# ddrakard/tensorflow-distributed-on-gke

Hardware: AMD Instinct MI355X
Metric: tokens/sec (whole node), Transformer-base en-pt at 1/2/4/8 MI355X (higher is better)
Workload: dtype bf16; 1 GPU; model=transformer-base (6L, d_model=512, heads=8, d_ff=2048, vocab 7765/7010), global_batch=64, local_batch=64, seq_len=128, parallelism=dp1, hip_graph=single, grad_comm=fp32, defer_wgrad=True

## Files before the change

csrc/bindings/embedding.cpp:

```cpp
#include "common.h"

namespace {

bool check_tok(const Tensor& tok) {
  TORCH_CHECK(tok.is_contiguous() && tok.is_cuda(), "tok must be a contiguous GPU tensor");
  const bool t64 = tok.scalar_type() == at::kLong;
  TORCH_CHECK(t64 || tok.scalar_type() == at::kInt, "tok must be int32/int64");
  return t64;
}
void check_grads(const Tensor& dout, const Tensor& dtable, int64_t M) {
  check_bf16(dout, "dout");
  check_contig(dout, "dout");
  check_f32(dtable, "dtable");
  check_contig(dtable, "dtable");
  TORCH_CHECK(dout.numel() == M * dtable.size(1), "dout shape");
}
void check_kbits(const optional<Tensor>& kbits, int64_t M, int64_t D) {
  if (!kbits.has_value()) return;
  TORCH_CHECK(kbits->is_cuda() && kbits->scalar_type() == at::kByte && kbits->is_contiguous() &&
                  kbits->numel() == M * D / 8,
              "kbits: uint8 [M, D / 8]");
  check_aligned(*kbits, 4, "kbits");
}

void embed_fwd(const Tensor& tok, const Tensor& table, const Tensor& pe, const Tensor& out,
               double scale, double p, int64_t seed, const optional<Tensor>& ctr, int64_t site,
               const optional<Tensor>& kbits) {
  TORCH_CHECK(tok.dim() == 2, "tok must be [B,L]");
  const bool t64 = check_tok(tok);
  check_bf16(table, "table");
  check_contig(table, "table");
  check_f32(pe, "pe");
  check_contig(pe, "pe");
  check_bf16(out, "out");
  check_contig(out, "out");
  const int64_t D = table.size(1), L = tok.size(1), M = tok.numel();
  TORCH_CHECK(pe.dim() == 2 && pe.size(1) == D && pe.size(0) >= L, "pe table too short");
  TORCH_CHECK(out.numel() == M * D, "out shape");
  check_kbits(kbits, M, D);
  c10::DeviceGuard g(tok.device());
  const int rc = tdg_embed_fwd(tok.data_ptr(), t64, table.data_ptr(), pe.data_ptr<float>(),
                               out.data_ptr(), (int)M, (int)L, (int)D, (float)scale, (float)p,
                               (uint64_t)seed, ctr_ptr(ctr), (uint64_t)site, opt_ptr(kbits),
                               stream_of(tok));
  check_err(rc, "tdg embed_fwd");
}

void embed_bwd(const Tensor& tok, const Tensor& dout, const Tensor& dtable, double scale,
               double p, int64_t seed, const optional<Tensor>& ctr, int64_t site) {
  const bool t64 = check_tok(tok);
  const int64_t D = dtable.size(1), M = tok.numel();
  check_grads(dout, dtable, M);
  c10::DeviceGuard g(tok.device());
  const int rc = tdg_embed_bwd(tok.data_ptr(), t64, dout.data_ptr(), dtable.data_ptr<float>(),
                               (int)M, (int)D, (float)scale, (float)p, (uint64_t)seed,
                               ctr_ptr(ctr), (uint64_t)site, stream_of(tok));
  check_err(rc, "tdg embed_bwd");
}

void embed_bwd_det(const Tensor& tok, const Tensor& dout, const Tensor& dtable, const Tensor& acc,
                   double scale, double p, int64_t seed, const optional<Tensor>& ctr, int64_t site,
                   bool accumulate) {
  const bool t64 = check_tok(tok);
  const int64_t D = dtable.size(1), M = tok.numel(), V = dtable.size(0);
  check_grads(dout, dtable, M);
  TORCH_CHECK(acc.scalar_type() == at::kLong && acc.is_cuda() && acc.is_contiguous(), "acc int64");
  TORCH_CHECK(acc.numel() >= dtable.numel(), "acc too small");
  c10::DeviceGuard g(tok.device());
  const int rc = tdg_embed_bwd_det(tok.data_ptr(), t64, dout.data_ptr(), dtable.data_ptr<float>(),
                                   reinterpret_cast<long long*>(acc.data_ptr<int64_t>()), (int)M,
                                   (int)D, (long long)V, (float)scale, (float)p, (uint64_t)seed,
                                   ctr_ptr(ctr), (uint64_t)site, accumulate ? 1.f : 0.f,
                                   stream_of(tok));
  check_err(rc, "tdg embed_bwd_det");
}

std::vector<int64_t> embed_csr_ws(int64_t M, int64_t V, int64_t D) {
  long long n32 = 0, n64 = 0;
  tdg_embed_csr_ws((int)M, (int)V, (int)D, &n32, &n64);
  return {n32, n64};
}

bool embed_csr_ok(int64_t M, int64_t V) { return tdg_embed_csr_ok((int)M, (int)V) != 0; }

void check_csr_ws(const Tensor& ws32, int64_t M, int64_t V, int64_t D, const char* n) {
  const int64_t n32 = embed_csr_ws(M, V, D)[0];
  TORCH_CHECK(ws32.scalar_type() == at::kInt && ws32.is_cuda() && ws32.is_contiguous() &&
                  ws32.numel() >= n32,
              n, ": int32 workspace of ", n32, " words");
  check_aligned(ws32, 16, n);
}

void embed_csr_sort(const std::vector<Tensor>& toks, const std::vector<int64_t>& V,
                    const std::vector<Tensor>& ws32, const optional<Tensor>& stamps) {
  const int n = (int)toks.size();
  TORCH_CHECK(n >= 1 && n <= 2 && (int)V.size() == n && (int)ws32.size() == n, "embed_csr_sort: 1-2 tables");
  const void* tp[2];
  int t64[2], M[2], VV[2];
  int* wp[2];
  for (int i = 0; i < n; ++i) {
    const Tensor& t = toks[i];
    t64[i] = check_tok(t);
    TORCH_CHECK(tdg_embed_csr_ok((int)t.numel(), (int)V[i]), "embed_csr_sort: shape past the sort");
    check_csr_ws(ws32[i], t.numel(), V[i], 128, "embed_csr_sort");
    tp[i] = t.data_ptr();
    M[i] = (int)t.numel();
    VV[i] = (int)V[i];
    wp[i] = ws32[i].data_ptr<int>();
  }
  c10::DeviceGuard g(toks[0].device());
  long long* sp = nullptr;
  if (stamps.has_value()) {
    TORCH_CHECK(stamps->scalar_type() == at::kLong && stamps->is_cuda() && stamps->numel() >= 1024,
                "stamps");
    sp = reinterpret_cast<long long*>(stamps->data_ptr<int64_t>());
  }
  check_err(tdg_embed_csr_sort(n, tp, t64, M, VV, wp, sp, stream_of(toks[0])), "tdg embed_csr_sort");
}

void embed_csr_apply(const Tensor& dout, const Tensor& dtable, const Tensor& ws32,
                     const Tensor& ws64, int64_t M, double scale, double p, int64_t seed,
                     const optional<Tensor>& ctr, int64_t site, bool accumulate,
                     const optional<Tensor>& kbits) {
  check_grads(dout, dtable, M);
  check_aligned(dtable, 16, "dtable");
  const int64_t D = dtable.size(1), V = dtable.size(0);
  TORCH_CHECK(tdg_embed_csr_ok((int)M, (int)V), "embed_csr_apply: shape past the sort");
  check_kbits(kbits, M, D);
  check_csr_ws(ws32, M, V, D, "embed_csr_apply");
  const int64_t n64 = embed_csr_ws(M, V, D)[1];
  TORCH_CHECK(ws64.scalar_type() == at::kLong && ws64.is_cuda() && ws64.is_contiguous() &&
                  ws64.numel() >= n64,
              "embed_csr_apply: int64 workspace of ", n64, " words");
  c10::DeviceGuard g(dout.device());
  check_err(tdg_embed_csr_apply(dout.data_ptr(), opt_ptr(kbits), dtable.data_ptr<float>(),
                                ws32.data_ptr<int>(),
                                reinterpret_cast<long long*>(ws64.data_ptr<int64_t>()), (int)M,
                                (int)D, (int)V, (float)scale, (float)p, (uint64_t)seed,
                                ctr_ptr(ctr), (uint64_t)site, accumulate ? 1.f : 0.f,
                                stream_of(dout)),
            "tdg embed_csr_apply");
}

}

void def_embedding(py::module_& m) {
  m.def("embed_fwd", &embed_fwd);
  m.def("embed_bwd", &embed_bwd);
  m.def("embed_bwd_det", &embed_bwd_det);
  m.def("embed_csr_ws", &embed_csr_ws);
  m.def("embed_csr_ok", &embed_csr_ok);
  m.def("embed_csr_sort", &embed_csr_sort);
  m.def("embed_csr_apply", &embed_csr_apply);
}
```

csrc/bindings/gemm.cpp:

```cpp
#include "common.h"

namespace {

void check_operand(const Tensor& t, bool kc, int64_t mn, int64_t K, int64_t ld, const char* n) {
  check_bf16(t, n);
  check_aligned(t, 16, n);
  if (kc) check_extent(t, mn, ld, round8(K), n);
  else check_extent(t, K, ld, round8(mn), n);
}
void check_group_c(const Tensor& C, bool f32, int64_t M, int64_t N, int64_t ldc) {
  TORCH_CHECK(C.is_cuda() && (C.scalar_type() == at::kFloat) == f32 &&
                  (f32 || C.scalar_type() == at::kBFloat16),
              "grouped gemm: C dtypes must match (f32 or bf16)");
  check_extent(C, M, ldc, N, "C");
}

void gemm(const Tensor& A, const Tensor& B, const Tensor& C, const optional<Tensor>& bias,
          const optional<Tensor>& aux, int64_t M, int64_t N, int64_t K, int64_t lda, int64_t ldb,
          int64_t ldc, int64_t ldaux, bool a_kc, bool b_kc, int64_t epi, double alpha,
          double beta, int64_t tile_cfg, int64_t splits, const optional<Tensor>& ws,
          const optional<Tensor>& relu_bits, int64_t ldbits) {
  TORCH_CHECK(C.is_cuda(), "C must be a GPU tensor");
  const bool f32 = C.scalar_type() == at::kFloat;
  TORCH_CHECK(f32 || C.scalar_type() == at::kBFloat16, "C must be f32 or bf16");
  TORCH_CHECK(M > 0 && N > 0 && K > 0, "gemm: empty problem");
  TORCH_CHECK(lda % 8 == 0 && ldb % 8 == 0, "gemm: lda/ldb must be multiples of 8");
  TORCH_CHECK(lda >= round8(a_kc ? K : M), "gemm: lda < round8(", a_kc ? "K)" : "M)");
  TORCH_CHECK(ldb >= round8(b_kc ? K : N), "gemm: ldb < round8(", b_kc ? "K)" : "N)");
  check_operand(A, a_kc, M, K, lda, "A");
  check_operand(B, b_kc, N, K, ldb, "B");
  TORCH_CHECK(ldc >= N, "gemm: ldc < N");
  check_extent(C, M, ldc, N, "C");
  const float* bptr = nullptr;
  if (epi == 1 || epi == 2) {
    TORCH_CHECK(bias.has_value(), "gemm: bias epilogue needs bias");
    check_f32(*bias, "bias");
    TORCH_CHECK(bias->numel() >= N, "gemm: bias too short");
    bptr = bias->data_ptr<float>();
  }
  const void* xptr = nullptr;
  void* bits = nullptr;
  if (relu_bits.has_value()) {
    TORCH_CHECK(epi == 2 || epi == 3, "gemm: relu_bits needs the bias+ReLU or ReLU-backward epilogue");
    TORCH_CHECK(relu_bits->is_cuda() && relu_bits->scalar_type() == at::kByte,
                "relu_bits must be a uint8 GPU tensor");
    TORCH_CHECK(N % 8 == 0, "gemm: relu_bits needs N % 8 == 0");
    TORCH_CHECK(ldbits >= N / 8, "gemm: ldbits < N / 8");
    check_extent(*relu_bits, M, ldbits, N / 8, "relu_bits");
    bits = relu_bits->data_ptr();
  }
  if (epi == 3 && bits == nullptr) {
    TORCH_CHECK(aux.has_value(), "gemm: DRELU epilogue needs aux");
    check_bf16(*aux, "aux");
    check_extent(*aux, M, ldaux, N, "aux");
    xptr = aux->data_ptr();
  }
  float* wptr = nullptr;
  if (splits > 1) {
    TORCH_CHECK(ws.has_value(), "gemm: split-K needs a workspace");
    check_f32(*ws, "ws");
    TORCH_CHECK(ws->numel() >= splits * M * ldc, "gemm: workspace too small");
    wptr = ws->data_ptr<float>();
  }
  c10::DeviceGuard g(A.device());
  const int rc = tdg_gemm(A.data_ptr(), B.data_ptr(), C.data_ptr(), bptr, xptr, (int)M, (int)N,
                          (int)K, (int)lda, (int)ldb, (int)ldc, (int)ldaux, a_kc, b_kc, (int)epi,
                          f32, (float)alpha, (float)beta, (int)tile_cfg, (int)splits, wptr,
                          stream_of(A), bits, (int)ldbits);
  check_err(rc, "tdg gemm");
}

void gemm_grouped(const std::vector<Tensor>& As, const std::vector<Tensor>& Bs,
                  const std::vector<Tensor>& Cs, int64_t M, int64_t N, int64_t K, int64_t lda,
                  int64_t ldb, int64_t ldc, bool a_kc, bool b_kc, double alpha, double beta,
                  int64_t tile_cfg) {
  const size_t G = As.size();
  TORCH_CHECK(G >= 1 && G <= 32 && Bs.size() == G && Cs.size() == G, "gemm_grouped: 1..32 problems");
  TORCH_CHECK(M > 0 && N > 0 && K > 0 && lda % 8 == 0 && ldb % 8 == 0 && ldc >= N, "gemm_grouped: shape");
  const bool f32 = Cs[0].scalar_type() == at::kFloat;
  std::vector<const void*> a(G), b(G);
  std::vector<void*> c(G);
  for (size_t i = 0; i < G; ++i) {
    check_operand(As[i], a_kc, M, K, lda, "A");
    check_operand(Bs[i], b_kc, N, K, ldb, "B");
    check_group_c(Cs[i], f32, M, N, ldc);
    a[i] = As[i].data_ptr();
    b[i] = Bs[i].data_ptr();
    c[i] = Cs[i].data_ptr();
  }
  c10::DeviceGuard g(As[0].device());
  const int rc = tdg_gemm_grouped(a.data(), b.data(), c.data(), (int)G, (int)M, (int)N, (int)K,
                                  (int)lda, (int)ldb, (int)ldc, a_kc, b_kc, f32, (float)alpha,
                                  (float)beta, (int)tile_cfg, stream_of(As[0]));
  check_err(rc, "tdg gemm_grouped");
}

void gemm_ragged(const std::vector<Tensor>& As, const std::vector<Tensor>& Bs,
                 const std::vector<Tensor>& Cs, const std::vector<int64_t>& shapes, int64_t K,
                 bool a_kc, bool b_kc, double alpha, double beta,
                 const std::vector<c10::optional<Tensor>>& bias_out) {
  const size_t P = As.size();
  TORCH_CHECK(P >= 1 && P <= 64 && Bs.size() == P && Cs.size() == P && shapes.size() == 7 * P,
              "gemm_ragged: 1..64 problems, 7 shape values each (M, N, lda, ldb, ldc, t_first, "
              "t_count)");
  TORCH_CHECK(K > 0 && K % 64 == 0, "gemm_ragged: K must be a multiple of 64");
  const bool f32 = Cs[0].scalar_type() == at::kFloat;
  std::vector<const void*> a(P), b(P);
  std::vector<void*> c(P);
  std::vector<int> sh(7 * P);
  for (size_t i = 0; i < P; ++i) {
    const int64_t M = shapes[7 * i], N = shapes[7 * i + 1], lda = shapes[7 * i + 2],
                  ldb = shapes[7 * i + 3], ldc = shapes[7 * i + 4];
    TORCH_CHECK(M > 0 && N > 0 && lda % 8 == 0 && ldb % 8 == 0 && ldc >= N, "gemm_ragged: shape");
    check_operand(As[i], a_kc, M, K, lda, "A");
    check_operand(Bs[i], b_kc, N, K, ldb, "B");
    check_group_c(Cs[i], f32, M, N, ldc);
    a[i] = As[i].data_ptr();
    b[i] = Bs[i].data_ptr();
    c[i] = Cs[i].data_ptr();
    for (int j = 0; j < 7; ++j) sh[7 * i + j] = (int)shapes[7 * i + j];
  }
// ... 12 lines not shown
  }
  c10::DeviceGuard g(As[0].device());
  const int rc = tdg_gemm_ragged(a.data(), b.data(), c.data(), (int)P, sh.data(), (int)K, a_kc,
                                 b_kc, f32, (float)alpha, (float)beta,
                                 any_bias ? bo.data() : nullptr, stream_of(As[0]));
  check_err(rc, "tdg gemm_ragged");
}

void colsum(const Tensor& X, const Tensor& out, const Tensor& part, int64_t M, int64_t N,
            int64_t ld, int64_t rows_per_block, double beta) {
  check_bf16(X, "X");
  check_f32(out, "out");
  check_f32(part, "part");
  check_extent(X, M, ld, N, "X");
  TORCH_CHECK(out.numel() >= N, "colsum: out too short");
  TORCH_CHECK(part.numel() >= ((M + rows_per_block - 1) / rows_per_block) * N,
              "colsum: partial buffer too small");
  c10::DeviceGuard g(X.device());
  tdg_colsum(X.data_ptr(), out.data_ptr<float>(), part.data_ptr<float>(), (int)M, (int)N, (int)ld,
             (int)rows_per_block, (float)beta, stream_of(X));
  check_err(0, "tdg colsum");
}

void colsum_grouped(const std::vector<Tensor>& Xs, const std::vector<Tensor>& outs,
                    const Tensor& part, int64_t M, int64_t N, int64_t ld, int64_t rows_per_block,
                    double beta) {
  const size_t G = Xs.size();
  TORCH_CHECK(G >= 1 && G <= 32 && outs.size() == G, "colsum_grouped: 1..32 problems");
  check_f32(part, "part");
  const int64_t nparts = (M + rows_per_block - 1) / rows_per_block;
  TORCH_CHECK(part.numel() >= (int64_t)G * nparts * N, "colsum_grouped: partials too small");
  std::vector<const void*> x(G);
  std::vector<float*> o(G);
  for (size_t i = 0; i < G; ++i) {
    check_bf16(Xs[i], "X");
    check_extent(Xs[i], M, ld, N, "X");
    check_f32(outs[i], "out");
    TORCH_CHECK(outs[i].numel() >= N, "colsum_grouped: out too short");
    x[i] = Xs[i].data_ptr();
    o[i] = outs[i].data_ptr<float>();
  }
  c10::DeviceGuard g(Xs[0].device());
  check_err(tdg_colsum_grouped(x.data(), o.data(), (int)G, part.data_ptr<float>(), (int)M, (int)N,
                               (int)ld, (int)rows_per_block, (float)beta, stream_of(Xs[0])),
            "tdg colsum_grouped");
}

std::vector<int64_t> gemm_last_plan() {
  int p[5];
  tdg_gemm_last_plan(p);
  return {p[0], p[1], p[2], p[3], p[4]};
}

}

void def_gemm(py::module_& m) {
  m.def("gemm", &gemm, py::arg("A"), py::arg("B"), py::arg("C"), py::arg("bias"), py::arg("aux"),
        py::arg("M"), py::arg("N"), py::arg("K"), py::arg("lda"), py::arg("ldb"), py::arg("ldc"),
        py::arg("ldaux"), py::arg("a_kc"), py::arg("b_kc"), py::arg("epi"), py::arg("alpha"),
        py::arg("beta"), py::arg("tile_cfg"), py::arg("splits"), py::arg("ws"),
        py::arg("relu_bits") = optional<Tensor>(), py::arg("ldbits") = 0);
  m.def("gemm_grouped", &gemm_grouped);
  m.def("gemm_ragged", &gemm_ragged, py::arg("As"), py::arg("Bs"), py::arg("Cs"), py::arg("shapes"),
        py::arg("K"), py::arg("a_kc"), py::arg("b_kc"), py::arg("alpha"), py::arg("beta"),
        py::arg("bias_out") = std::vector<c10::optional<Tensor>>{});
  m.def("gemm_last_plan", &gemm_last_plan);
  m.def("colsum", &colsum);
  m.def("colsum_grouped", &colsum_grouped);
}
```

csrc/bindings/layernorm.cpp:

```cpp
#include "common.h"

namespace {

void check_same_numel(const Tensor& t, const Tensor& like, const char* n) {
  TORCH_CHECK(t.numel() == like.numel() && t.is_contiguous(), "ln: ", n, " shape");
}
void check_ln_kbits(const optional<Tensor>& kbits, int64_t M, int64_t D) {
  if (!kbits.has_value()) return;
  TORCH_CHECK(kbits->is_cuda() && kbits->scalar_type() == at::kByte && kbits->is_contiguous() &&
                  kbits->numel() == M * D / 8 && D >= 512,
              "ln: kbits uint8 [M, D / 8] (D >= 512)");
}

void ln_fwd(const Tensor& x, const optional<Tensor>& s, const Tensor& gamma, const Tensor& beta,
            const Tensor& y, const optional<Tensor>& hsave, const optional<Tensor>& mean,
            const optional<Tensor>& rstd, double p, int64_t seed, const optional<Tensor>& ctr,
            int64_t site, double eps, const optional<Tensor>& y8, const optional<Tensor>& s8,
            const optional<Tensor>& amax8, const optional<Tensor>& kbits) {
  check_bf16(x, "x");
  check_contig(x, "x");
  const int64_t D = x.size(-1), M = x.numel() / D;
  check_bf16(y, "y");
  check_same_numel(y, x, "y");
  if (s.has_value()) {
    check_bf16(*s, "s");
    check_same_numel(*s, x, "s");
  }
  check_f32(gamma, "gamma");
  check_f32(beta, "beta");
  TORCH_CHECK(gamma.numel() == D && beta.numel() == D, "ln: gamma/beta shape");
  if (hsave.has_value()) {
    check_bf16(*hsave, "hsave");
    check_same_numel(*hsave, x, "hsave");
  }
  for (auto* t : {&mean, &rstd})
    if (t->has_value()) {
      check_f32(**t, "mean/rstd");
      TORCH_CHECK((*t)->numel() == M, "ln: mean/rstd shape");
    }
  if (y8.has_value()) {
    check_f8_fmt(*y8, 0, "y8");
    check_same_numel(*y8, x, "y8");
    TORCH_CHECK(s8.has_value(), "ln: y8 needs s8");
    check_f32(*s8, "s8");
  }
  check_ln_kbits(kbits, M, D);
  TORCH_CHECK(!kbits.has_value() || s.has_value(), "ln: kbits are the dropout on s");
  c10::DeviceGuard g(x.device());
  const int rc = tdg_ln_fwd(x.data_ptr(), opt_ptr(s), gamma.data_ptr<float>(),
                            beta.data_ptr<float>(), y.data_ptr(), opt_ptr(hsave), opt_f32(mean),
                            opt_f32(rstd), (int)M, (int)D, (float)p, (uint64_t)seed, ctr_ptr(ctr),
                            (uint64_t)site, (float)eps, opt_ptr(y8), opt_f32(s8), amax_ptr(amax8),
                            opt_ptr(kbits), stream_of(x));
  check_err(rc, "tdg ln_fwd");
}

void ln_bwd(const Tensor& dy, const Tensor& hsave, const Tensor& mean, const Tensor& rstd,
            const Tensor& gamma, const Tensor& dh, const optional<Tensor>& ds,
            const optional<Tensor>& dres, const Tensor& dgamma, const Tensor& dbeta,
            const optional<Tensor>& dbias, const Tensor& ws, double p, int64_t seed,
            const optional<Tensor>& ctr, int64_t site, bool accumulate, bool skip_reduce,
            int64_t rpb, const optional<Tensor>& ds8, const optional<Tensor>& s8,
            const optional<Tensor>& amax8, const optional<Tensor>& kbits) {
  check_bf16(dy, "dy");
  check_contig(dy, "dy");
  const int64_t D = dy.size(-1), M = dy.numel() / D;
  for (auto* t : {&hsave, &dh}) {
    check_bf16(*t, "hsave/dh");
    check_same_numel(*t, dy, "hsave/dh");
  }
  for (auto* t : {&ds, &dres})
    if (t->has_value()) {
      check_bf16(**t, "ds/dres");
      check_same_numel(**t, dy, "ds/dres");
    }
  check_f32(mean, "mean");
  check_f32(rstd, "rstd");
  check_f32(gamma, "gamma");
  check_f32(dgamma, "dgamma");
  check_f32(dbeta, "dbeta");
  TORCH_CHECK(mean.numel() == M && rstd.numel() == M, "ln_bwd: mean/rstd shape");
  TORCH_CHECK(gamma.numel() == D && dgamma.numel() == D && dbeta.numel() == D, "ln_bwd: D");
  if (dbias.has_value()) {
    check_f32(*dbias, "dbias");
    TORCH_CHECK(dbias->numel() == D && (ds.has_value() || ds8.has_value()), "ln_bwd: dbias needs ds");
  }
  if (ds8.has_value()) {
    check_f8_fmt(*ds8, 1, "ds8 (e5m2)");
    check_same_numel(*ds8, dy, "ds8");
    TORCH_CHECK(s8.has_value(), "ln_bwd: ds8 needs s8");
    check_f32(*s8, "s8");
  }
  check_f32(ws, "ws");
  TORCH_CHECK(rpb == 16 || rpb == 32 || rpb == 64, "ln_bwd: rows per block 16 / 32 / 64");
  TORCH_CHECK(ws.numel() >= 3 * ((M + rpb - 1) / rpb) * D, "ln_bwd: workspace too small");
  check_ln_kbits(kbits, M, D);
  c10::DeviceGuard g(dy.device());
  const int rc = tdg_ln_bwd(
      dy.data_ptr(), hsave.data_ptr(), mean.data_ptr<float>(), rstd.data_ptr<float>(),
      gamma.data_ptr<float>(), dh.data_ptr(), opt_ptr(ds), opt_ptr(dres), dgamma.data_ptr<float>(),
      dbeta.data_ptr<float>(), opt_f32(dbias), ws.data_ptr<float>(), (int)M, (int)D, (float)p,
      (uint64_t)seed, ctr_ptr(ctr), (uint64_t)site, accumulate, skip_reduce, (int)rpb,
      opt_ptr(ds8), opt_f32(s8), amax_ptr(amax8), opt_ptr(kbits), stream_of(dy));
  check_err(rc, "tdg ln_bwd");
}

void reduce_partials_multi(const std::vector<Tensor>& parts, const std::vector<Tensor>& outs,
                           const std::vector<int64_t>& nparts, int64_t N, double beta) {
  const size_t G = parts.size();
  TORCH_CHECK(G >= 1 && G <= 96 && outs.size() == G && nparts.size() == G,
              "reduce_partials_multi: 1..96 problems");
  std::vector<const float*> pp(G);
  std::vector<float*> oo(G);
  std::vector<int> np(G);
  for (size_t i = 0; i < G; ++i) {
    check_f32(parts[i], "parts");
    check_f32(outs[i], "outs");
    check_contig(parts[i], "parts");
    TORCH_CHECK(outs[i].numel() == N && outs[i].is_contiguous(), "reduce_partials_multi: out");
    TORCH_CHECK(parts[i].numel() >= nparts[i] * N, "reduce_partials_multi: partials too small");
    TORCH_CHECK(parts[i].device() == parts[0].device() && outs[i].device() == parts[0].device(),
                "reduce_partials_multi: one device");
    pp[i] = parts[i].data_ptr<float>();
    oo[i] = outs[i].data_ptr<float>();
    np[i] = (int)nparts[i];
  }
  c10::DeviceGuard g(parts[0].device());
  check_err(tdg_reduce_partials_multi(pp.data(), oo.data(), np.data(), (int)G, (int)N, (float)beta,
                                      stream_of(parts[0])),
            "tdg reduce_partials_multi");
}

}

void def_layernorm(py::module_& m) {
  m.def("ln_fwd", &ln_fwd);
  m.def("ln_bwd", &ln_bwd);
  m.def("reduce_partials_multi", &reduce_partials_multi);
}
```

csrc/include/tdg_api.h:

```cpp
#pragma once
#include <hip/hip_runtime.h>
#include <stdint.h>

#include "tdg_attn.h"
#include "tdg_decode.h"

extern "C" {

int tdg_gemm(const void* A, const void* B, void* C, const float* bias, const void* aux, int M,
             int N, int K, int lda, int ldb, int ldc, int ldaux, int a_kc, int b_kc, int epi,
             int out_f32, float alpha, float beta, int tile_cfg, int splits, float* ws,
             hipStream_t st, void* relu_bits, int ldbits);
int tdg_gemm_grouped(const void* const* A, const void* const* B, void* const* C, int G, int M,
                     int N, int K, int lda, int ldb, int ldc, int a_kc, int b_kc, int out_f32,
                     float alpha, float beta, int tile_cfg, hipStream_t st);
int tdg_gemm_ragged(const void* const* A, const void* const* B, void* const* C, int P,
                    const int* shapes, int K, int a_kc, int b_kc, int out_f32, float alpha,
                    float beta, float* const* bias_out, hipStream_t st);
void tdg_gemm_last_plan(int out[5]);
void tdg_colsum(const void* X, float* out, float* part, int M, int N, int ld, int rows_per_block,
                float beta, hipStream_t st);
int tdg_colsum_grouped(const void* const* X, float* const* out, int G, float* part, int M, int N,
                       int ld, int rows_per_block, float beta, hipStream_t st);

int tdg_attn_fwd(const tdg::AttnArgs* a, int hd, hipStream_t st);
int tdg_qkv_attn_fwd(const tdg::QkvAttnArgs* qa, hipStream_t st);
int tdg_attn_bwd(const tdg::AttnArgs* a, int hd, hipStream_t st);
int tdg_attn_bwd_fdo(const tdg::AttnArgs* a, hipStream_t st);
int tdg_attn_probs(const tdg::AttnArgs* a, int hd, float* probs, hipStream_t st);
int tdg_attn_fwd_fp8(const tdg::AttnArgs* a, int hd, hipStream_t st);
int tdg_attn_bwd_f8(const tdg::AttnArgs* a, int hd, hipStream_t st);

int tdg_decode_attn(const tdg::DecodeAttnArgs* a, int hd, hipStream_t st);
int tdg_beam_topk(const tdg::BeamTopkArgs* a, hipStream_t st);

int tdg_ln_fwd(const void* x, const void* s, const float* gamma, const float* beta, void* y,
               void* hsave, float* mean, float* rstd, int M, int D, float p, uint64_t seed,
               const long long* ctr, uint64_t site, float eps, void* y8, const float* s8,
               unsigned* amax8, void* kbits, hipStream_t st);
int tdg_ln_bwd(const void* dy, const void* hsave, const float* mean, const float* rstd,
               const float* gamma, void* dh, void* ds, const void* dres, float* dgamma,
               float* dbeta, float* dbias, float* ws, int M, int D, float p, uint64_t seed,
               const long long* ctr, uint64_t site, int accumulate, int skip_reduce, int rpb,
               void* ds8, const float* s8, unsigned* amax8, const void* kbits, hipStream_t st);
int tdg_reduce_partials_multi(const float* const* parts, float* const* outs, const int* nparts,
                              int G, int N, float beta, hipStream_t st);

int tdg_embed_fwd(const void* tok, int tok64, const void* table, const float* pe, void* out, int M,
                  int L, int D, float scale, float p, uint64_t seed, const long long* ctr,
                  uint64_t site, void* kbits, hipStream_t st);
int tdg_embed_bwd(const void* tok, int tok64, const void* dout, float* dtable, int M, int D,
                  float scale, float p, uint64_t seed, const long long* ctr, uint64_t site,
                  hipStream_t st);
int tdg_embed_bwd_det(const void* tok, int tok64, const void* dout, float* dtable, long long* acc,
                      int M, int D, long long V, float scale, float p, uint64_t seed,
                      const long long* ctr, uint64_t site, float beta, hipStream_t st);
void tdg_embed_csr_ws(int M, int V, int D, long long* n32, long long* n64);
int tdg_embed_csr_ok(int M, int V);
int tdg_embed_csr_sort(int ntab, const void* const* tok, const int* tok64, const int* M,
                       const int* V, int* const* ws32, long long* stamps, hipStream_t st);
int tdg_embed_csr_apply(const void* dout, const void* kbits, float* dtable, int* ws32,
                        long long* ws64, int M, int D, int V, float scale, float p, uint64_t seed,
                        const long long* ctr, uint64_t site, float beta, hipStream_t st);

int tdg_count_tokens(const void* labels, int lab64, int M, float* out, hipStream_t st);
int tdg_prep_batch(const void* src, int S, const void* tgt, int T1, int B, int lab64, void* tgt_in,
                   void* labels, int* src_len, int* tgt_len, float* ntok, long long* ctr,
                   int* row_lab, unsigned* ticket, int* bad_rows, hipStream_t st);
int tdg_xent(void* logits, int M, int V, int ldl, const void* labels, int lab64, const float* ntok,
             float workers, float smoothing, float* row_loss, float* row_correct, int write_grad,
             hipStream_t st);
int tdg_xent_stats(const float* row_loss, const float* row_correct, int M, const float* ntok,
                   float workers, float* step_out, float* accum, hipStream_t st);

int tdg_adam(float* p, float* g, float* m, float* v, void* shadow, long long n, long long* step,
             float beta1, float beta2, float eps, float lr_const, float d_model, float warmup,
             float grad_scale, float weight_decay, int sched, int zero_grad, int inc_step,
             const float* gstate, hipStream_t st);
int tdg_adam_chunks(float* p, float* g, float* m, float* v, void* shadow, long long n,
                    const void* chunks, int nchunks, long long* step, float beta1, float beta2,
                    float eps, float lr_const, float d_model, float warmup, float grad_scale,
                    float weight_decay, int sched, int zero_grad, int inc_step,
                    const float* scale8, unsigned* amax8, const float* gstate, hipStream_t st);
int tdg_adam_step_inc(long long* step, const float* gstate, hipStream_t st);
long long tdg_grad_sumsq(const float* g, const void* chunks, long long nchunks, long long n,
                         float* partials, hipStream_t st);
int tdg_grad_norm_finalize(const float* partials, long long nparts, float* state,
                           unsigned* counters, float clip, int skip_on, float grad_scale,
                           hipStream_t st);
int tdg_to_bf16(const float* p, void* o, long long n, hipStream_t st);
int tdg_transpose_grouped(const void* const* src, void* const* dst, int G, int R, int C,
                          hipStream_t st);

int tdg_gemm_fp8(const void* A, const void* B, void* C, const float* bias, const float* sa,
                 const float* sb, void* C8, const float* sc8, unsigned* amax, int M, int N, int K,
                 int lda, int ldb, int ldc, int ldc8, int epi, int cfg, int afmt, int cfmt,
                 const void* aux, int ldaux, float beta, const void* aux8, float* colsum_out,
                 float colsum_beta, float* ws, hipStream_t st);
int tdg_wgrad_fp8(const void* const* A, const void* const* B, float* const* C,
                  const float* const* sa, const float* const* sb, int P, const int* shapes, int T,
                  float beta, hipStream_t st);
int tdg_fp8_set_persist(int on);
int tdg_fp8_quant(const void* x, void* y8, long long n, const float* scale, unsigned* amax,
// ... 17 lines not shown
```

csrc/include/tdg_common.h:

```cpp
#pragma once
#include <hip/hip_runtime.h>
#include <utility>
#include <stdint.h>

namespace tdg {

#ifdef TDG_STAMPS
__device__ unsigned long long* tdg_stamps;
#define TDG_STAMP(i)                                                                      \
  do {                                                                                    \
    if (threadIdx.x < 64)                                                                 \
      tdg_stamps[(((size_t)blockIdx.z * gridDim.y + blockIdx.y) * gridDim.x + blockIdx.x) * 512 + (i) * 64 + threadIdx.x] =                     \
          __builtin_amdgcn_s_memrealtime();                                               \
  } while (0)
#else
#define TDG_STAMP(i) \
  do {               \
  } while (0)
#endif

typedef uint16_t bf16_t;

typedef __bf16 bf16x8 __attribute__((ext_vector_type(8)));
typedef short short4_t __attribute__((ext_vector_type(4)));
typedef short short8_t __attribute__((ext_vector_type(8)));
typedef short short2_t __attribute__((ext_vector_type(2)));
typedef __bf16 bf16x2_t __attribute__((ext_vector_type(2)));
typedef float f32x4 __attribute__((ext_vector_type(4)));
typedef float f32x16 __attribute__((ext_vector_type(16)));

typedef __attribute__((address_space(3))) short4_t lds_short4;

constexpr int WAVE = 64;

__device__ __forceinline__ float bf2f(bf16_t v) {
  return __uint_as_float(((uint32_t)v) << 16);
}

__device__ __forceinline__ bf16_t f2bf(float f) {
  return __builtin_bit_cast(bf16_t, (__bf16)f);
}

__device__ __forceinline__ uint32_t pack2bf(float a, float b) {
  const bf16x2_t v = {(__bf16)a, (__bf16)b};
  return __builtin_bit_cast(uint32_t, v);
}

__host__ __device__ __forceinline__ int cdiv(int a, int b) { return (a + b - 1) / b; }

template <int CTRL, int ROWS = 0xF, bool BC = true>
__device__ __forceinline__ float dpp_f(float v, float old = 0.f) {
  return __builtin_bit_cast(float, __builtin_amdgcn_update_dpp(__builtin_bit_cast(int, old),
                                                               __builtin_bit_cast(int, v), CTRL, ROWS,
                                                               0xF, BC));
}
__device__ __forceinline__ float lane63(float v) {
// ... 169 lines not shown
  short8_t r;
  asm volatile("ds_read_b128 %0, %1 offset:%2" : "=v"(r) : "v"(a), "i"(OFF) : "memory");
  return r;
}
template <int OFF>
__device__ __forceinline__ short4_t lds_read_tr16_at(uint32_t a) {
  static_assert(OFF >= 0 && OFF < 65536, "DS offset field");
  short4_t r;
  asm volatile("ds_read_b64_tr_b16 %0, %1 offset:%2" : "=v"(r) : "v"(a), "i"(OFF) : "memory");
  return r;
}
template <class F, int... I>
__device__ __forceinline__ void static_for_impl(F&& f, std::integer_sequence<int, I...>) {
  (f(std::integral_constant<int, I>{}), ...);
}
template <int N, class F>
__device__ __forceinline__ void static_for(F&& f) {
  static_for_impl(f, std::make_integer_sequence<int, N>{});
}
__device__ __forceinline__ long lds_read_tr8_async(const void* p) {
  long r;
  const uint32_t a = (uint32_t)(uintptr_t)p;
  asm volatile("ds_read_b64_tr_b8 %0, %1" : "=v"(r) : "v"(a) : "memory");
  return r;
}

template <int N>
__device__ __forceinline__ void lgkm_wait() {
  asm volatile("s_waitcnt lgkmcnt(%0)" ::"n"(N < 15 ? N : 15) : "memory");
}

template <typename T>
__device__ __forceinline__ void tie(T& x) {
  asm volatile("" : "+v"(x));
}

__device__ __forceinline__ short8_t cat4(short4_t a, short4_t b) {
  short8_t r;
  r[0] = a[0]; r[1] = a[1]; r[2] = a[2]; r[3] = a[3];
  r[4] = b[0]; r[5] = b[1]; r[6] = b[2]; r[7] = b[3];
  return r;
}

__device__ __forceinline__ short pack_bf(float f) { return (short)f2bf(f); }

__device__ __forceinline__ short8_t pack8(float a0, float a1, float a2, float a3, float a4, float a5,
                                          float a6, float a7) {
  short8_t r;
  r[0] = pack_bf(a0); r[1] = pack_bf(a1); r[2] = pack_bf(a2); r[3] = pack_bf(a3);
  r[4] = pack_bf(a4); r[5] = pack_bf(a5); r[6] = pack_bf(a6); r[7] = pack_bf(a7);
  return r;
}

typedef unsigned int u32x4_t __attribute__((ext_vector_type(4)));
typedef unsigned int u32x2_t __attribute__((ext_vector_type(2)));
struct WtBuf {
  __amdgpu_buffer_rsrc_t r;
  const char* base;
  bool ok;
  __device__ __forceinline__ WtBuf(const void* p, size_t bytes)
      : r(__builtin_amdgcn_make_buffer_rsrc(const_cast<void*>(p), 0,
                                             (int)(bytes < 0x7fffffffull ? bytes : 0x7fffffffull),
                                             0x00020000)),
        base(static_cast<const char*>(p)),
        ok(bytes <= 0x7fffffffull) {}
  template <typename T>
  __device__ __forceinline__ void st16(void* p, const T& v) const {
    static_assert(sizeof(T) == 16, "16-byte value");
    if (ok)
      __builtin_amdgcn_raw_buffer_store_b128(__builtin_bit_cast(u32x4_t, v), r,
                                             (int)(static_cast<const char*>(p) - base), 0, 16);
    else
      *static_cast<T*>(p) = v;
  }
  template <typename T>
  __device__ __forceinline__ void st8(void* p, const T& v) const {
    static_assert(sizeof(T) == 8, "8-byte value");
    if (ok)
      __builtin_amdgcn_raw_buffer_store_b64(__builtin_bit_cast(u32x2_t, v), r,
                                            (int)(static_cast<const char*>(p) - base), 0, 16);
    else
      *static_cast<T*>(p) = v;
  }
  __device__ __forceinline__ void st4(void* p, uint32_t v) const {
    if (ok)
      __builtin_amdgcn_raw_buffer_store_b32(v, r, (int)(static_cast<const char*>(p) - base), 0, 16);
    else
      *static_cast<uint32_t*>(p) = v;
  }
};

constexpr float E4M3_MAX = 448.f;
constexpr int AMAX_SPREAD = 64;
constexpr int AMAX_STRIDE = 32;
constexpr int AMAX_WORDS = AMAX_SPREAD * AMAX_STRIDE;
__device__ __forceinline__ unsigned* amax_word(unsigned* slot, int b) {
  return slot + (b & (AMAX_SPREAD - 1)) * AMAX_STRIDE;
}
template <bool HI>
__device__ __forceinline__ int pack2_e4m3(float a, float b, int old) {
  a = fminf(fmaxf(a, -E4M3_MAX), E4M3_MAX);
  b = fminf(fmaxf(b, -E4M3_MAX), E4M3_MAX);
  return __builtin_amdgcn_cvt_pk_fp8_f32(a, b, old, HI);
}
constexpr float E5M2_MAX_F = 57344.f;
template <bool HI>
__device__ __forceinline__ int pack2_e5m2c(float a, float b, int old) {
  a = fminf(fmaxf(a, -E5M2_MAX_F), E5M2_MAX_F);
  b = fminf(fmaxf(b, -E5M2_MAX_F), E5M2_MAX_F);
  return __builtin_amdgcn_cvt_pk_bf8_f32(a, b, old, HI);
}
__device__ __forceinline__ void atomic_amax(unsigned* p, float v) {
  atomicMax(p, __float_as_uint(fabsf(v)));
}

__device__ __forceinline__ int xcd_remap(int bid, int nwg) {
  constexpr int NX = 8;
  if (nwg <= NX) return bid;
  const int q = nwg / NX, r = nwg % NX;
  const int x = bid % NX, i = bid / NX;
  const int base = (x < r) ? x * (q + 1) : r * (q + 1) + (x - r) * q;
  return base + i;
}

}
```

csrc/include/tdg_gemm.h:

```cpp
#pragma once
#include "tdg_common.h"

#include <type_traits>

namespace tdg {

constexpr int BK = 64;

template <bool KC, int R>
__device__ __forceinline__ int lds_off(int row, int byte) {
  if constexpr (KC) {
    const int seg = (byte >> 5) ^ ((row >> 1) & 3);
    return row * (BK * 2) + (seg << 5) + (byte & 31);
  } else if constexpr (R >= 128) {
    const int seg = (byte >> 5) ^ ((row & 3) | (((row >> 3) & 1) << 2));
    return row * (R * 2) + (seg << 5) + (byte & 31);
  } else {
    static_assert(R == 64, "MN-contiguous tiles must be 64 or 128 wide");
    const int seg = (byte >> 5) ^ (((row >> 1) & 1) | (((row >> 3) & 1) << 1));
    return row * 128 + (seg << 5) + (byte & 31);
  }
}

template <bool KC, int R, int NW>
// ... 225 lines not shown
}

template <int EPI, bool OUT_F32, int TM, int TN, int RPASS>
struct EpiLds {
  static constexpr int ES = OUT_F32 ? 4 : 2;
  static constexpr int SP = TN * 16 * ES + 16;
  static constexpr int CPR = TN * 16 * ES / 16;
  static constexpr int EPC = 16 / ES;
  static constexpr int ITER = RPASS * CPR / 64;
  static constexpr int BYTES = RPASS * SP;
  static_assert(RPASS % 16 == 0 && (TM * 16) % RPASS == 0, "passes of whole 16-row sub-tiles");
  static_assert((RPASS * CPR) % 64 == 0, "whole chunk iterations");
  static constexpr bool BITS = epi_has_bits(EPI);
  static constexpr int PAD = TN * 16 * ES;
  static constexpr int MBW = CPR / 4 > 0 ? CPR / 4 : 1;
  static constexpr int MBR = MBW * ((TM * 16 + 63) / 64);
  static_assert(!BITS || (!OUT_F32 && (CPR == 4 || CPR == 8) && (RPASS == 64 || RPASS == TM * 16)),
                "bitmap epilogues: bf16 out, 32/64-wide wave tiles, rows of a pass held by lanes 0..RPASS-1");

  __device__ static __forceinline__ void mask_load(uint32_t (&mb)[MBR], const unsigned char* bits,
                                                   int ldb, int M, int N, int mw0, int nw0, int lane) {
    const bool wide = nw0 + TN * 16 <= N && (ldb % (4 * MBW)) == 0 &&
                      (reinterpret_cast<uintptr_t>(bits) % (4 * MBW)) == 0;
#pragma unroll
    for (int k = 0; k < MBR / MBW; ++k) {
      int m = mw0 + lane + 64 * k;
      m = m < M ? m : M - 1;
      const unsigned char* p = bits + (size_t)m * ldb + (nw0 >> 3);
      if (wide) {
        if constexpr (MBW == 2) {
          const uint2 v = *reinterpret_cast<const uint2*>(p);
          mb[2 * k] = v.x;
          mb[2 * k + 1] = v.y;
        } else {
          mb[k] = *reinterpret_cast<const uint32_t*>(p);
        }
      } else {
#pragma unroll
        for (int w = 0; w < MBW; ++w) mb[MBW * k + w] = 0u;
#pragma unroll
        for (int c = 0; c < CPR; ++c)
          if (nw0 + 8 * c < N) mb[MBW * k + c / 4] |= (uint32_t)p[c] << (8 * (c % 4));
      }
    }
  }

  __device__ static __forceinline__ int row_of(int lane, int t) { return (lane + 64 * t) / CPR; }
  __device__ static __forceinline__ int col_of(int lane, int t) { return ((lane + 64 * t) % CPR) * EPC; }

  __device__ static __forceinline__ void run(char* wimg, const f32x4 (&acc)[TM][TN], int lane,
                                             void* __restrict__ Cv, int ldc, int M, int N, int mw0,
                                             int nw0, float alpha, float beta,
                                             const float* __restrict__ bias,
                                             const bf16_t* __restrict__ aux, int ldaux, bool vec) {
    int4 none[ITER];
    uint32_t nomask[MBR];
    run_pre<false>(wimg, acc, lane, Cv, ldc, M, N, mw0, nw0, alpha, beta, bias, aux, ldaux, vec,
                   none, false, none, false, nomask);
  }
  __device__ static __forceinline__ void run_mask(char* wimg, const f32x4 (&acc)[TM][TN], int lane,
                                                  void* __restrict__ Cv, int ldc, int M, int N,
                                                  int mw0, int nw0, float alpha, float beta,
                                                  const float* __restrict__ bias,
                                                  const bf16_t* __restrict__ aux, int ldaux, bool vec,
                                                  const uint32_t (&mb)[MBR]) {
    int4 none[ITER];
    run_pre<false>(wimg, acc, lane, Cv, ldc, M, N, mw0, nw0, alpha, beta, bias, aux, ldaux, vec,
                   none, false, none, false, mb);
  }
  template <bool PRE>
  __device__ static __forceinline__ void run_pre(char* wimg, const f32x4 (&acc)[TM][TN], int lane,
                                                 void* __restrict__ Cv, int ldc, int M, int N,
                                                 int mw0, int nw0, float alpha, float beta,
                                                 const float* __restrict__ bias,
                                                 const bf16_t* __restrict__ aux, int ldaux, bool vec,
                                                 const int4 (&pre_aux)[ITER], bool use_aux,
                                                 const int4 (&pre_c)[ITER], bool use_c,
                                                 const uint32_t (&mb)[MBR]) {
    const int g = lane >> 4, r16 = lane & 15;
    bool vok = vec && ((ldc * ES) % 16) == 0 && (reinterpret_cast<uintptr_t>(Cv) & 15) == 0;
    if constexpr (EPI == EPI_DRELU)
      vok = vok && (ldaux % EPC) == 0 && (reinterpret_cast<uintptr_t>(aux) % (2 * EPC)) == 0;
#if TDG_EPI_SC1
    const WtBuf wt(Cv, ((size_t)(M - 1) * ldc + N) * ES);
#endif
    f32x4 bn[TN];
#pragma unroll
    for (int j = 0; j < TN; ++j) bn[j] = load_bias4<EPI>(bias, nw0 + 16 * j + 4 * g, N);
    using VecT = typename std::conditional<OUT_F32, f32x4, short8_t>::type;
    constexpr bool AUX8 = EPI == EPI_DRELU && EPC == 8;
    const bool loc_aux = AUX8 && !(PRE && use_aux) && vok;
    const bool loc_c = !(PRE && use_c) && beta != 0.f && vok;
#pragma unroll
    for (int p = 0; p < TM * 16 / RPASS; ++p) {
      int4 la[ITER], lc[ITER];
      if (loc_aux || loc_c) {
#pragma unroll
        for (int t = 0; t < ITER; ++t) {
          const int id = lane + 64 * t;
          const int m = mw0 + p * RPASS + id / CPR, n = nw0 + (id % CPR) * EPC;
          const bool in = m < M && n + EPC <= N;
          if (loc_aux) {
            const bf16_t* a = in ? aux + (size_t)m * ldaux + n : aux;
            la[t] = *reinterpret_cast<const int4*>(a);
          }
          if (loc_c) {
            const char* c = in ? reinterpret_cast<const char*>(Cv) + ((size_t)m * ldc + n) * ES
                               : reinterpret_cast<const char*>(Cv);
            lc[t] = *reinterpret_cast<const int4*>(c);
          }
        }
      }
      if constexpr (EPI == EPI_DRELU_BITS) {
        if (RPASS == 64 || lane < RPASS) {
          const int k = p * RPASS / 64;
          char* dst = wimg + lane * SP + PAD;
          if constexpr (MBW == 2) *reinterpret_cast<uint2*>(dst) = uint2{mb[2 * k], mb[2 * k + 1]};
          else *reinterpret_cast<uint32_t*>(dst) = mb[k];
        }
      }
#pragma unroll
      for (int ii = 0; ii < RPASS / 16; ++ii) {
        const int i = p * (RPASS / 16) + ii;
#pragma unroll
        for (int j = 0; j < TN; ++j) {
          float v[4];
#pragma unroll
          for (int r = 0; r < 4; ++r) {
            v[r] = alpha * acc[i][j][r];
            if constexpr (EPI == EPI_BIAS) v[r] += bn[j][r];
            if constexpr (epi_has_relu(EPI)) v[r] = fmaxf(v[r] + bn[j][r], 0.f);
          }
          char* dst = wimg + (16 * ii + r16) * SP + (16 * j + 4 * g) * ES;
          if constexpr (OUT_F32) {
            *reinterpret_cast<f32x4*>(dst) = f32x4{v[0], v[1], v[2], v[3]};
          } else {
            short4_t w;
// ... 109 lines not shown
```

csrc/include/tdg_ln.h:

```cpp
#pragma once
#include "tdg_common.h"

namespace tdg {

template <int VEC>
struct RowMap {
  static constexpr int W = VEC < 8 ? VEC : 8;
  static constexpr int CH = VEC / W;
  __device__ static __forceinline__ int col(int lane, int i) {
    return (i / W) * (64 * W) + lane * W + (i % W);
  }
};

template <int VEC>
struct RowVec {
  using Map = RowMap<VEC>;
  float v[VEC];
  __device__ __forceinline__ void load_row(const bf16_t* row, int lane) {
    const bf16_t* p = row + lane * Map::W;
    if constexpr (VEC == 2) {
      const uint32_t w = *reinterpret_cast<const uint32_t*>(p);
      v[0] = bf2f((bf16_t)(w & 0xffff));
      v[1] = bf2f((bf16_t)(w >> 16));
    } else if constexpr (VEC == 4) {
// ... 21 lines not shown
    } else {
#pragma unroll
      for (int c = 0; c < Map::CH; ++c) {
        short8_t w;
#pragma unroll
        for (int i = 0; i < 8; ++i) w[i] = (short)f2bf(v[8 * c + i]);
        wt.st16(p + 512 * c, w);
      }
    }
  }
  __device__ __forceinline__ void store_row(bf16_t* row, int lane) const {
    bf16_t* p = row + lane * Map::W;
    if constexpr (VEC == 2) {
      *reinterpret_cast<uint32_t*>(p) = pack2bf(v[0], v[1]);
    } else if constexpr (VEC == 4) {
      short4_t w;
#pragma unroll
      for (int i = 0; i < 4; ++i) w[i] = (short)f2bf(v[i]);
      *reinterpret_cast<short4_t*>(p) = w;
    } else {
#pragma unroll
      for (int c = 0; c < Map::CH; ++c) {
        short8_t w;
#pragma unroll
        for (int i = 0; i < 8; ++i) w[i] = (short)f2bf(v[8 * c + i]);
        *reinterpret_cast<short8_t*>(p + 512 * c) = w;
      }
    }
  }
};

template <int VEC>
__device__ __forceinline__ uint32_t keep_bits(uint64_t seed, const long long* ctr, uint64_t site,
                                              uint64_t e_row, int lane, uint32_t thresh) {
  using Map = RowMap<VEC>;
  const uint64_t off = rng_offset(ctr, site);
  uint32_t m = 0;
#pragma unroll
  for (int c = 0; c < Map::CH; ++c)
    m |= dropout_keep_run<Map::W>(seed, off, e_row + Map::col(lane, Map::W * c), thresh)
         << (Map::W * c);
  return m;
}

template <int D>
__device__ __forceinline__ void ln_row_fwd(RowVec<D / 64>& h, RowVec<D / 64>& t, bool has_t,
                                           size_t rbase, int row, int lane,
                                           const float* __restrict__ gamma,
                                           const float* __restrict__ beta, bf16_t* __restrict__ y,
                                           bf16_t* __restrict__ hsave, float* __restrict__ mean_out,
                                           float* __restrict__ rstd_out, float p, uint32_t thresh,
                                           uint64_t seed, const long long* ctr, uint64_t site,
                                           float eps, RowVec<D / 64>& o, size_t wt_bytes = 0,
                                           uint8_t* __restrict__ kbits = nullptr) {
  constexpr int VEC = D / 64;
  if (has_t) {
    if (p > 0.f) {
      const uint32_t km = keep_bits<VEC>(seed, ctr, site, rbase, lane, thresh);
      if constexpr (VEC >= 8) {
        if (kbits) {
#pragma unroll
          for (int c = 0; c < RowMap<VEC>::CH; ++c)
            kbits[rbase / 8 + 64 * c + lane] = (uint8_t)(km >> (8 * c));
        }
      }
      const float sc = 1.f / (1.f - p);
#pragma unroll
      for (int i = 0; i < VEC; ++i) t.v[i] = ((km >> i) & 1u) ? t.v[i] * sc : 0.f;
    }
#pragma unroll
    for (int i = 0; i < VEC; ++i) h.v[i] += t.v[i];
  }
  if (hsave) {
    if (wt_bytes) h.store_row(hsave + rbase, lane, WtBuf(hsave, wt_bytes));
    else h.store_row(hsave + rbase, lane);
#pragma unroll
    for (int i = 0; i < VEC; ++i) h.v[i] = bf2f(f2bf(h.v[i]));
  }
  float sum = 0.f;
#pragma unroll
  for (int i = 0; i < VEC; ++i) sum += h.v[i];
  const float mean = wave_sum(sum) * (1.f / D);
  float sq = 0.f;
#pragma unroll
  for (int i = 0; i < VEC; ++i) {
    const float d = h.v[i] - mean;
    sq += d * d;
  }
  const float var = wave_sum(sq) * (1.f / D);
  const float rstd = rsqrtf(var + eps);
#pragma unroll
  for (int i = 0; i < VEC; ++i) {
    const int col = RowMap<VEC>::col(lane, i);
    o.v[i] = (h.v[i] - mean) * rstd * gamma[col] + beta[col];
  }
  if (wt_bytes) o.store_row(y + rbase, lane, WtBuf(y, wt_bytes));
  else o.store_row(y + rbase, lane);
  if (lane == 0) {
    if (mean_out) mean_out[row] = mean;
    if (rstd_out) rstd_out[row] = rstd;
  }
}

}
```

csrc/kernels/attn_bwd.h:

```cpp
#pragma once
#include "attn_impl.h"

namespace tdg {

#define TDG_ATTENDS(key, q, klim, Lq, causal) \
  (((key) < (klim)) & ((q) < (Lq)) & (!(causal) | ((key) <= (q))))
#define TDG_PDS_KEY_LANE(U_, full, sv, dpv, lse, del, c, key, q4, klim, Lq, causal, p, ds)   \
  if (full) {                                                                                \
    _Pragma("unroll") for (int r_ = 0; r_ < 4; ++r_)                                         \
    _Pragma("unroll") for (int u_ = 0; u_ < U_; ++u_) {                                      \
      const float pv_ = fast_exp2((sv)[u_][r_] * (c) - (lse)[r_]);                           \
      (p)[u_][r_] = pv_;                                                                     \
      (ds)[u_][r_] = pv_ * ((dpv)[u_][r_] - (del)[r_]);                                      \
    }                                                                                        \
  } else {                                                                                   \
    _Pragma("unroll") for (int r_ = 0; r_ < 4; ++r_) {                                       \
      const int q_ = (q4) + r_;                                                              \
      _Pragma("unroll") for (int u_ = 0; u_ < U_; ++u_) {                                    \
        const bool ok_ = TDG_ATTENDS((key)[u_], q_, klim, Lq, causal);                       \
        const float pv_ = masked_exp2((sv)[u_][r_] * (c) - (lse)[r_], ok_);                  \
        (p)[u_][r_] = pv_;                                                                   \
        (ds)[u_][r_] = pv_ * ((dpv)[u_][r_] - (del)[r_]);                                    \
      }                                                                                      \
    }                                                                                        \
// ... 721 lines not shown
      if constexpr (MODE >= 2) wait_vmcnt<(STAGES - 2) * PT>();
      else wait_vmcnt<0>();
      lds_barrier();
      const char* nx = smem + ((kt + 1) % STAGES) * SB;
      if constexpr (MODE == 3) {
        char* ns = smem + (kt % STAGES) * SB;
        ga.issue(Y, a.fdo_ldy, a.Lq, K, 0, (kt + STAGES) * BK, ns, wid);
        gb.issue(W, a.fdo_ldw, BN, K, 0, (kt + STAGES) * BK, ns + A_BYTES, wid);
      }
#pragma unroll
      for (int i = 0; i < TM; ++i) fa0[i] = frag<true, BM>(nx, abase + 16 * i, 0, lane);
#pragma unroll
      for (int j = 0; j < TN; ++j) fb0[j] = frag<false, BN>(nx + A_BYTES, bbase + 16 * j, 0, lane);
    } else {
      lgkm_wait<0>();
    }
    tie_all(fa1);
    tie_all(fb1);
    prio_hi();
#pragma unroll
    for (int i = 0; i < TM; ++i)
#pragma unroll
      for (int j = 0; j < TN; ++j) acc[i][j] = mfma16(fb1[j], fa1[i], acc[i][j]);
    prio_lo();
  };
  int kt = 0;
  for (; kt + STAGES < nk; ++kt) kstep(kt, std::integral_constant<int, 3>{});
  if (kt + STAGES - 1 < nk && kt + 1 < nk) kstep(kt++, std::integral_constant<int, 2>{});
  for (; kt + 1 < nk; ++kt) kstep(kt, std::integral_constant<int, 1>{});
  if (kt < nk) kstep(kt, std::integral_constant<int, 0>{});
  lds_barrier();
}

template <int HD, int U, bool FDO = false>
__global__ __launch_bounds__(512 / U) __attribute__((amdgpu_waves_per_eu(U == 1 ? (HD <= 64 ? 4 : 2) : 2))) void attn_bwd_fused_kernel(AttnArgs a) {
  static_assert(!FDO || (HD == 64 && U == 1), "in-kernel dO: hd 64, 8 waves");
  using T = ATile<HD>;
  using TS = DsImg;
  constexpr int R = 128;
  constexpr int NT = 512 / U;
  constexpr int TB = R * T::RB;
  constexpr int SB = R * TS::RB;
  constexpr int ALIAS = 2 * TB >= SB;
  extern __shared__ __attribute__((aligned(16))) char smem[];
  char* ldsQ = smem;
  char* ldsO = smem + TB;
  char* ldsK = smem + 2 * TB;
  char* ldsS = ALIAS ? smem : smem + 3 * TB;
  float* ldsL = reinterpret_cast<float*>(smem + (ALIAS ? 3 * TB : 3 * TB + SB));
  float* ldsD = ldsL + R;
  const int tid = threadIdx.x, lane = tid & 63, g = lane >> 4, cl = lane & 15;
  const int w = __builtin_amdgcn_readfirstlane(tid >> 6);
  const int bh = a.xcd ? xcd_remap(blockIdx.x, gridDim.x) : blockIdx.x;
  const int b = bh / a.H, h = bh % a.H;
  int klim;
  float scl;
  bool causal;
  key_window(a, b, klim, scl, causal);
  const float c = scl * LOG2E;

  TDG_STAMP(0);
  const bf16_t* qb = a.q + b * a.q_sb + h * a.q_sh;
  const bf16_t* ob = a.dout + b * a.do_sb + h * a.do_sh;
  const bf16_t* kbp = a.k + b * a.k_sb + h * a.k_sh;
  const bf16_t* obo = a.o + b * a.o_sb + h * a.o_sh;
  int key[U];
#pragma unroll
  for (int u = 0; u < U; ++u) key[u] = 16 * (U * w + u) + cl;
  short8_t kf[U][T::KS], vf[U][T::KS];
#pragma unroll
  for (int u = 0; u < U; ++u) {
    const int krow = min(key[u], a.Lk - 1);
    const bf16_t* kp = kbp + (long long)krow * a.k_sl;
    const bf16_t* vp = a.v + b * a.v_sb + (long long)krow * a.v_sl + h * a.v_sh;
    TDG_LOAD_ROW_FRAGS2(HD, lane, key[u] < a.Lk, kf[u], kp, vf[u], vp)
  }
  {
    constexpr int CPR = HD / 8;
    constexpr int TOTAL = R * CPR;
    constexpr int NI = (TOTAL + NT - 1) / NT;
    short8_t vq[NI], vo[NI], vk[NI], vx[NI];
    const short8_t z = {0, 0, 0, 0, 0, 0, 0, 0};
#pragma unroll
    for (int i = 0; i < NI; ++i) {
      const int id = tid + i * NT;
      const int row = id / CPR, cc = id % CPR;
      vq[i] = vo[i] = vk[i] = vx[i] = z;
      if constexpr (TOTAL % NT == 0) {
        const int rq = min(row, a.Lq - 1), rk = min(row, a.Lk - 1);
        vq[i] = ld8_or0(qb + (long long)rq * a.q_sl + cc * 8, row < a.Lq);
        if constexpr (!FDO) vo[i] = ld8_or0(ob + (long long)rq * a.do_sl + cc * 8, row < a.Lq);
        vx[i] = ld8_or0(obo + (long long)rq * a.o_sl + cc * 8, row < a.Lq);
        vk[i] = ld8_or0(kbp + (long long)rk * a.k_sl + cc * 8, row < a.Lk);
      } else {
        if (id < TOTAL && row < a.Lq) {
          vq[i] = *reinterpret_cast<const short8_t*>(qb + (long long)row * a.q_sl + cc * 8);
          if constexpr (!FDO) vo[i] = *reinterpret_cast<const short8_t*>(ob + (long long)row * a.do_sl + cc * 8);
          vx[i] = *reinterpret_cast<const short8_t*>(obo + (long long)row * a.o_sl + cc * 8);
        }
        if (id < TOTAL && row < a.Lk)
          vk[i] = *reinterpret_cast<const short8_t*>(kbp + (long long)row * a.k_sl + cc * 8);
      }
    }
    const float lse_v = (tid < R && tid < a.Lq) ? a.lse[((long long)b * a.H + h) * a.Lq + tid] : INFINITY;
    if constexpr (FDO) {
      f32x4 acc[2][2];
      fdo_tile(a, b, h, smem, w, lane, acc);
// ... 230 lines not shown
```

csrc/kernels/attn_qkv.h:

```cpp
#pragma once
#include "attn_impl.h"

namespace tdg {

template <int STAGES, bool CROSS, bool SB1 = false>
__global__ __launch_bounds__(512) __attribute__((amdgpu_waves_per_eu(SB1 ? 4 : 2))) void qkv_attn_fwd_kernel(
    const QkvAttnArgs qa) {
  constexpr int NW = 8, WM = CROSS ? 4 : 2, WN = CROSS ? 2 : 4, BM = 128, BN = CROSS ? 64 : 192;
  constexpr int NPART = BN / 64;
  constexpr int TM = BM / WM / 16, TN = BN / WN / 16;
  constexpr int A_BYTES = BM * BK * 2, B_BYTES = BN * BK * 2, SB = A_BYTES + B_BYTES;
  using GA = Glds<true, BM, NW>;
  using GB = Glds<true, BN, NW>;
  constexpr int PT = GA::P + GB::P;
  using T = ATile<64>;
  extern __shared__ __attribute__((aligned(16))) char smem[];
  const AttnArgs& a = qa.a;
  const int tid = threadIdx.x, lane = tid & 63;
  const int wid = __builtin_amdgcn_readfirstlane(tid >> 6);
  const int wm = wid / WN, wn = wid % WN;
  const int t = xcd_remap(blockIdx.x, gridDim.x);
  const int h = t % a.H, b = t / a.H;
  const int L = qa.L, d = qa.d, K = d;
  const bf16_t* X = reinterpret_cast<const bf16_t*>(qa.x) + (size_t)b * L * qa.ldx;
  using Ch = typename ATile<64>::template Chunks<512>;
  Ch ck[2], cv[2];
  if constexpr (CROSS) {
    const bf16_t* kb = a.k + b * a.k_sb + h * a.k_sh;
    const bf16_t* vb = a.v + b * a.v_sb + h * a.v_sh;
#pragma unroll
    for (int h64 = 0; h64 < 2; ++h64) {
      ATile<64>::template fetch<512>(ck[h64], kb, a.k_sl, 64 * h64, a.Lk, tid);
      ATile<64>::template fetch<512>(cv[h64], vb, a.v_sl, 64 * h64, a.Lk, tid);
    }
  }

  GA ga;
  GB gb;
  ga.init(wid, lane);
  gb.init(wid, lane);
  int wrow[GB::P];
#pragma unroll
  for (int i = 0; i < GB::P; ++i) wrow[i] = (gb.row[i] >> 6) * d + 64 * h + (gb.row[i] & 63);
  auto issue_b = [&](int k0, char* lds) {
#pragma unroll
    for (int i = 0; i < GB::P; ++i) {
      const long long off = (long long)wrow[i] * qa.ldw + k0 + gb.col[i];
      __builtin_amdgcn_global_load_lds((const void*)(reinterpret_cast<const bf16_t*>(qa.w) + off),
                                       (__attribute__((address_space(3))) void*)(lds + (wid * GB::P + i) * 1024),
                                       16, 0, 0);
    }
  };
  const int nk = K / BK;
  f32x4 acc[TM][TN];
  TDG_ZERO(TM, TN, acc)
#pragma unroll
  for (int st = 0; st < STAGES; ++st) {
    if (st < nk) {
      ga.issue(X, qa.ldx, L, K, 0, st * BK, smem + st * SB, wid);
      issue_b(st * BK, smem + st * SB + A_BYTES);
    }
  }
  const int abase = wm * (BM / WM), bbase = wn * (BN / WN);
  if constexpr (SB1) {
    short8_t fa[TM], fb[TN];
    for (int kt = 0; kt < nk; ++kt) {
      if (kt + 1 < nk) wait_vmcnt<PT>();
      else wait_vmcnt<0>();
      lds_barrier();
      const char* st = smem + (kt % STAGES) * SB;
#pragma unroll
      for (int s2 = 0; s2 < 2; ++s2) {
#pragma unroll
        for (int i = 0; i < TM; ++i) fa[i] = frag<true, BM>(st, abase + 16 * i, s2, lane);
#pragma unroll
// ... 184 lines not shown
```

csrc/kernels/embed.hip:

```cpp
#include "tdg_api.h"
#include "tdg_common.h"
#include "tdg_ln.h"

#include <algorithm>

namespace tdg {

template <int D, typename TokT>
__global__ __launch_bounds__(256) void embed_fwd_kernel(
    const TokT* __restrict__ tok, const bf16_t* __restrict__ table, const float* __restrict__ pe,
    bf16_t* __restrict__ out, int M, int L, float scale, float p, uint32_t thresh, uint64_t seed,
    const long long* __restrict__ ctr, uint64_t site, uint8_t* __restrict__ kbits) {
  constexpr int VEC = D / 64;
  const int lane = threadIdx.x & 63;
  const int row = blockIdx.x * 4 + (threadIdx.x >> 6);
  if (row >= M) return;
  const int pos = row % L;
  const long long t = (long long)tok[row];
  const float* pr = pe + (size_t)pos * D;
  RowVec<VEC> v;
  v.load_row(table + t * D, lane);
#pragma unroll
  for (int i = 0; i < VEC; ++i) v.v[i] = v.v[i] * scale + pr[RowMap<VEC>::col(lane, i)];
  if (p > 0.f) {
    const float sc = 1.f / (1.f - p);
    const uint32_t km = keep_bits<VEC>(seed, ctr, site, (size_t)row * D, lane, thresh);
#pragma unroll
    for (int i = 0; i < VEC; ++i) v.v[i] = ((km >> i) & 1u) ? v.v[i] * sc : 0.f;
    if constexpr (VEC >= 8) {
      if (kbits) {
#pragma unroll
        for (int c = 0; c < RowMap<VEC>::CH; ++c)
          kbits[(size_t)row * (D / 8) + 64 * c + lane] = (uint8_t)(km >> (8 * c));
      }
    }
  }
  v.store_row(out + (size_t)row * D, lane);
}

template <int D>
struct RowKeep {
  static constexpr int NS = (D + 511) / 512;
  uint32_t m[NS];
  __device__ __forceinline__ void draw(uint64_t seed, const long long* ctr, uint64_t site,
                                       size_t rbase, int lane, uint32_t thresh) {
    const uint64_t off = rng_offset(ctr, site);
#pragma unroll
    for (int s = 0; s < NS; ++s)
      m[s] = dropout_keep_run<8>(seed, off, rbase + 512 * s + 8 * lane, thresh);
  }
  __device__ __forceinline__ bool keep(int c, int lane) const {
    const int col = c * 64 + lane;
    const uint32_t mm = (uint32_t)__shfl((int)m[c >> 3], (col >> 3) & 63, 64);
    return (mm >> (col & 7)) & 1u;
  }
};

template <int D, typename TokT>
__global__ __launch_bounds__(256) void embed_bwd_kernel(
    const TokT* __restrict__ tok, const bf16_t* __restrict__ dout, float* __restrict__ dtable,
    int M, float scale, float p, uint32_t thresh, uint64_t seed, const long long* ctr, uint64_t site) {
  constexpr int VEC = D / 64;
  const int lane = threadIdx.x & 63;
  const int row = blockIdx.x * 4 + (threadIdx.x >> 6);
  if (row >= M) return;
  const long long t = (long long)tok[row];
  const size_t rbase = (size_t)row * D;
  const float sc = p > 0.f ? scale / (1.f - p) : scale;
// ... 378 lines not shown
      acc[i] += (long long)rintf(x * FX_SCALE);
    }
  }
  if (w.y < 0) {
    emb_store_row<VEC>(dtable + (size_t)w.x * D, acc, lane, beta,
                       WtBuf(dtable, (size_t)V * D * sizeof(float)));
  } else {
    long long* sl = cs.slab + (size_t)w.y * D;
#pragma unroll
    for (int i = 0; i < VEC; ++i) sl[Map::col(lane, i)] = acc[i];
  }
}

template <int D>
__global__ __launch_bounds__(1024) void embed_combine_kernel(float* __restrict__ dtable, EmbCsr cs,
                                                             int V, int nub, float beta) {
  constexpr int VEC = D / 64;
  using Map = RowMap<VEC>;
  __shared__ long long red[16][D];
  const int lane = threadIdx.x & 63, wid = threadIdx.x >> 6;
  const int hb = blockIdx.x;
  if (hb >= nub || hb >= cs.counts[1]) return;
  const int4 h = cs.heavy[hb];
  long long acc[VEC];
#pragma unroll
  for (int i = 0; i < VEC; ++i) acc[i] = 0;
  for (int k = wid; k < h.z; k += 16) {
    const long long* sl = cs.slab + (size_t)(h.y + k) * D;
#pragma unroll
    for (int i = 0; i < VEC; ++i) acc[i] += sl[Map::col(lane, i)];
  }
#pragma unroll
  for (int i = 0; i < VEC; ++i) red[wid][Map::col(lane, i)] = acc[i];
  __syncthreads();
  float* row = dtable + (size_t)h.x * D;
  for (int c = threadIdx.x; c < D; c += 1024) {
    long long t = 0;
#pragma unroll
    for (int q = 0; q < 16; ++q) t += red[q][c];
    float o = (float)t * (1.f / FX_SCALE);
    if (beta != 0.f) o += beta * row[c];
    row[c] = o;
  }
}

}

using namespace tdg;

namespace {
template <int D, typename TT>
void fwd_d(const void* tok, const void* table, const float* pe, void* out, int M, int L,
           float scale, float p, uint64_t seed, const long long* ctr, uint64_t site,
           void* kbits, hipStream_t st) {
  const uint32_t thresh = dropout_thresh(p);
  hipLaunchKernelGGL((embed_fwd_kernel<D, TT>), dim3(cdiv(M, 4)), dim3(256), 0, st,
                     (const TT*)tok, (const bf16_t*)table, pe, (bf16_t*)out, M, L, scale, p,
                     thresh, seed, ctr, site, (uint8_t*)kbits);
}
template <int D, typename TT>
void bwd_d(const void* tok, const void* dout, float* dtable, int M, float scale, float p,
           uint64_t seed, const long long* ctr, uint64_t site, hipStream_t st) {
  const uint32_t thresh = dropout_thresh(p);
  hipLaunchKernelGGL((embed_bwd_kernel<D, TT>), dim3(cdiv(M, 4)), dim3(256), 0, st,
                     (const TT*)tok, (const bf16_t*)dout, dtable, M, scale, p, thresh, seed, ctr, site);
}
template <int D, typename TT>
void bwd_fx_d(const void* tok, const void* dout, unsigned long long* acc, int M, float scale, float p,
              uint64_t seed, const long long* ctr, uint64_t site, hipStream_t st) {
  const uint32_t thresh = dropout_thresh(p);
  hipLaunchKernelGGL((embed_bwd_fx_kernel<D, TT>), dim3(cdiv(M, 4)), dim3(256), 0, st,
                     (const TT*)tok, (const bf16_t*)dout, acc, M, scale, p, thresh, seed, ctr, site);
}
}

#define TDG_D_SWITCH(F, TT, ...)                  \
  switch (D) {                                    \
    case 128: F<128, TT>(__VA_ARGS__); return 0;  \
    case 256: F<256, TT>(__VA_ARGS__); return 0;  \
    case 512: F<512, TT>(__VA_ARGS__); return 0;  \
    case 1024: F<1024, TT>(__VA_ARGS__); return 0; \
    default: return -1;                           \
  }

extern "C" int tdg_embed_fwd(const void* tok, int tok64, const void* table, const float* pe,
                             void* out, int M, int L, int D, float scale, float p, uint64_t seed,
                             const long long* ctr, uint64_t site, void* kbits, hipStream_t st) {
  if (kbits && D < 512) return -3;
  if (tok64) {
    TDG_D_SWITCH(fwd_d, long long, tok, table, pe, out, M, L, scale, p, seed, ctr, site, kbits, st)
  } else {
    TDG_D_SWITCH(fwd_d, int, tok, table, pe, out, M, L, scale, p, seed, ctr, site, kbits, st)
  }
}

extern "C" int tdg_embed_bwd(const void* tok, int tok64, const void* dout, float* dtable, int M,
                             int D, float scale, float p, uint64_t seed, const long long* ctr, uint64_t site,
                             hipStream_t st) {
  if (tok64) {
    TDG_D_SWITCH(bwd_d, long long, tok, dout, dtable, M, scale, p, seed, ctr, site, st)
  } else {
    TDG_D_SWITCH(bwd_d, int, tok, dout, dtable, M, scale, p, seed, ctr, site, st)
  }
}

extern "C" int tdg_embed_bwd_det(const void* tok, int tok64, const void* dout, float* dtable,
                                 long long* acc, int M, int D, long long V, float scale, float p,
                                 uint64_t seed, const long long* ctr, uint64_t site, float beta,
                                 hipStream_t st) {
  unsigned long long* a = reinterpret_cast<unsigned long long*>(acc);
  int rc = -1;
  if (tok64) {
    switch (D) {
      case 128: bwd_fx_d<128, long long>(tok, dout, a, M, scale, p, seed, ctr, site, st); rc = 0; break;
      case 256: bwd_fx_d<256, long long>(tok, dout, a, M, scale, p, seed, ctr, site, st); rc = 0; break;
      case 512: bwd_fx_d<512, long long>(tok, dout, a, M, scale, p, seed, ctr, site, st); rc = 0; break;
      case 1024: bwd_fx_d<1024, long long>(tok, dout, a, M, scale, p, seed, ctr, site, st); rc = 0; break;
    }
  } else {
    switch (D) {
      case 128: bwd_fx_d<128, int>(tok, dout, a, M, scale, p, seed, ctr, site, st); rc = 0; break;
      case 256: bwd_fx_d<256, int>(tok, dout, a, M, scale, p, seed, ctr, site, st); rc = 0; break;
      case 512: bwd_fx_d<512, int>(tok, dout, a, M, scale, p, seed, ctr, site, st); rc = 0; break;
      case 1024: bwd_fx_d<1024, int>(tok, dout, a, M, scale, p, seed, ctr, site, st); rc = 0; break;
    }
  }
  if (rc) return rc;
  const long long n = V * D;
  if (n % 4 == 0 && reinterpret_cast<uintptr_t>(dtable) % 16 == 0 &&
      reinterpret_cast<uintptr_t>(acc) % 16 == 0 && (size_t)n * sizeof(float) <= 0x7fffffffull) {
    const int blocks = (int)std::min<long long>(4096, (n / 4 + 255) / 256);
    hipLaunchKernelGGL(embed_acc_convert4_kernel, dim3(blocks > 0 ? blocks : 1), dim3(256), 0, st, acc,
                       dtable, n, beta);
    return 0;
  }
  const int blocks = (int)std::min<long long>(4096, (n / 2 + 255) / 256 + 1);
  hipLaunchKernelGGL(embed_acc_convert_kernel, dim3(blocks), dim3(256), 0, st, acc, dtable, n, beta);
  return 0;
}

extern "C" void tdg_embed_csr_ws(int M, int V, int D, long long* n32, long long* n64) {
  *n32 = (long long)(sizeof(EmbItem) / 4) * csr_ub_items(M, V) + 4LL * csr_ub_heavy(M) + 4;
  *n64 = (long long)csr_ub_slots(M) * D;
}

// ... 62 lines not shown
```

csrc/kernels/gemm.hip:

```cpp
#include "tdg_api.h"
#include "gemm_impl.h"

namespace tdg {

__global__ __launch_bounds__(256) void colsum_partial_kernel(const bf16_t* __restrict__ X,
                                                             float* __restrict__ part, int M, int N,
                                                             int ld, int rows_per_block) {
  __shared__ float red[32][65];
  const int cg = threadIdx.x & 7, rl = threadIdx.x >> 3;
  const int col0 = blockIdx.x * 64 + cg * 8;
  const int r0 = blockIdx.y * rows_per_block;
  const int r1 = min(M, r0 + rows_per_block);
  float acc[8];
#pragma unroll
  for (int i = 0; i < 8; ++i) acc[i] = 0.f;
  const bool vec = (col0 + 8 <= N) && (ld % 8 == 0);
  for (int r = r0 + rl; r < r1; r += 32) {
    const bf16_t* p = X + (size_t)r * ld + col0;
    if (vec) {
      const short8_t v = *reinterpret_cast<const short8_t*>(p);
#pragma unroll
      for (int i = 0; i < 8; ++i) acc[i] += bf2f((bf16_t)v[i]);
    } else {
#pragma unroll
// ... 43 lines not shown
#pragma unroll
      for (int i = 0; i < 8; ++i)
        if (col0 + i < N) acc[i] += bf2f(p[i]);
    }
  }
#pragma unroll
  for (int i = 0; i < 8; ++i) red[rl][cg * 8 + i] = acc[i];
  __syncthreads();
  if (threadIdx.x < 64) {
    float s = 0.f;
#pragma unroll 8
    for (int k = 0; k < 32; ++k) s += red[k][threadIdx.x];
    const int col = blockIdx.x * 64 + threadIdx.x;
    if (col < N) pz[(size_t)blockIdx.y * N + col] = s;
  }
}

__global__ __launch_bounds__(256) void reduce_partials_grouped_kernel(ColsumGroup grp,
                                                                      const float* __restrict__ part,
                                                                      int N, int P, float beta) {
  __shared__ float red[4][64];
  const float* pz = part + (size_t)blockIdx.y * P * N;
  float* out = grp.out[blockIdx.y];
  const int c = threadIdx.x & 63, g = threadIdx.x >> 6;
  const int col = blockIdx.x * 64 + c;
  float s = 0.f;
  if (col < N) {
#pragma unroll 8
    for (int p = g; p < P; p += 4) s += pz[(size_t)p * N + col];
  }
  red[g][c] = s;
  __syncthreads();
  if (g == 0 && col < N) {
    const float t = red[0][c] + red[1][c] + red[2][c] + red[3][c];
    out[col] = (beta != 0.f ? beta * out[col] : 0.f) + t;
  }
}

int* gemm_plan_slot() {
  static thread_local int plan[5] = {-1, 0, 0, 0, 0};
  return plan;
}

}

extern "C" void tdg_gemm_last_plan(int out[5]) {
  const int* p = gemm_plan_slot();
  for (int i = 0; i < 5; ++i) out[i] = p[i];
}

extern "C" int tdg_gemm(const void* A, const void* B, void* C, const float* bias, const void* aux,
                        int M, int N, int K, int lda, int ldb, int ldc, int ldaux, int a_kc,
                        int b_kc, int epi, int out_f32, float alpha, float beta, int tile_cfg,
                        int splits, float* ws, hipStream_t st, void* relu_bits, int ldbits) {
  const bf16_t* a = (const bf16_t*)A;
  const bf16_t* b = (const bf16_t*)B;
  const bf16_t* x = (const bf16_t*)aux;
  if (relu_bits) {
    if (epi != EPI_BIAS_RELU && epi != EPI_DRELU) return -11;
    if (out_f32 || N % 8 != 0 || ldc % 8 != 0 || (reinterpret_cast<uintptr_t>(C) & 15) != 0 ||
        ldbits < N / 8)
      return -11;
    epi = epi == EPI_BIAS_RELU ? EPI_BIAS_RELU_BITS : EPI_DRELU_BITS;
    x = (const bf16_t*)relu_bits;
    ldaux = ldbits;
  } else if (epi > EPI_DRELU) {
    return -1;
  }
  auto fn = a_kc ? (b_kc ? gemm_nt : gemm_nn) : (b_kc ? gemm_tt : gemm_tn);
  return fn(epi, out_f32 != 0, tile_cfg, a, b, C, bias, x, M, N, K, lda, ldb, ldc, ldaux, alpha,
            beta, splits, ws, st);
}

extern "C" int tdg_gemm_grouped(const void* const* A, const void* const* B, void* const* C, int G,
                                int M, int N, int K, int lda, int ldb, int ldc, int a_kc, int b_kc,
                                int out_f32, float alpha, float beta, int tile_cfg, hipStream_t st) {
  if (G < 1 || G > MAXG) return -2;
  GemmGroup g{};
  for (int i = 0; i < G; ++i) {
    g.A[i] = (const bf16_t*)A[i];
    g.B[i] = (const bf16_t*)B[i];
    g.C[i] = C[i];
  }
  auto fn = a_kc ? (b_kc ? gemm_grouped_nt : gemm_grouped_nn)
                 : (b_kc ? gemm_grouped_tt : gemm_grouped_tn);
  return fn(g, G, M, N, K, lda, ldb, ldc, out_f32 != 0, alpha, beta, tile_cfg, st);
}

extern "C" int tdg_gemm_ragged(const void* const* A, const void* const* B, void* const* C, int P,
                               const int* shapes, int K, int a_kc, int b_kc, int out_f32,
                               float alpha, float beta, float* const* bias_out,
                               hipStream_t st) {
  if (P < 1 || P > R256_MAXP) return -2;
  R256Args args{};
  int ncls = 0, tiles = 0;
  bool prev_partial = false;
  for (int i = 0; i < P; ++i) {
    const int* s = shapes + 7 * i;
    const int tpp = cdiv(s[0], 256) * cdiv(s[1], 256);
    const int first = s[5], count = s[6] < 0 ? tpp - s[5] : s[6];
    if (first < 0 || count <= 0 || first + count > tpp) return -8;
    const bool partial = count != tpp;
    const bool same = ncls > 0 && !partial && !prev_partial && args.cls[ncls - 1].M == s[0] &&
                      args.cls[ncls - 1].N == s[1] && args.cls[ncls - 1].lda == s[2] &&
                      args.cls[ncls - 1].ldb == s[3] && args.cls[ncls - 1].ldc == s[4];
    if (!same) {
      if (ncls == R256_MAXC) return -5;
      R256Class& c = args.cls[ncls++];
      c.M = s[0]; c.N = s[1]; c.lda = s[2]; c.ldb = s[3]; c.ldc = s[4];
      c.tiles_m = cdiv(s[0], 256); c.tiles_n = cdiv(s[1], 256);
      c.tile_start = tiles; c.prob_start = i; c.t_first = first;
      if ((!a_kc && s[2] % 8) || (!b_kc && s[3] % 8)) return -6;
    }
    prev_partial = partial;
    tiles += count;
    args.A[i] = (const bf16_t*)A[i];
    args.B[i] = (const bf16_t*)B[i];
    args.C[i] = C[i];
    args.bias_out[i] = bias_out ? bias_out[i] : nullptr;
    if (args.bias_out[i] && a_kc) return -7;
  }
  args.ncls = ncls;
  if (a_kc && b_kc) return gemm_ragged_nt(args, tiles, K, out_f32 != 0, alpha, beta, st);
  if (a_kc && !b_kc) return out_f32 ? -4 : gemm_ragged_nn(args, tiles, K, false, alpha, beta, st);
// ... 30 lines not shown
```

csrc/kernels/gemm_impl.h:

```cpp
#pragma once
#include "tdg_common.h"
#include "tdg_gemm.h"
#include "tdg_reduce.h"
#include "gemm_pipe.h"

#include <cstdlib>
#include <type_traits>

namespace tdg {



constexpr int MAXG = 32;
struct GemmGroup {
  const bf16_t* A[MAXG];
  const bf16_t* B[MAXG];
  void* C[MAXG];
};

template <int BM, int BN, int WM, int WN, int STAGES, bool A_KC, bool B_KC, int EPI,
          bool OUT_F32>
__global__ __launch_bounds__(WM* WN * 64) void gemm_kernel(
    const bf16_t* __restrict__ A, const bf16_t* __restrict__ B, void* __restrict__ Cv,
    const float* __restrict__ bias, const bf16_t* __restrict__ aux, int M, int N, int K, int lda,
    int ldb, int ldc, int ldaux, float alpha, float beta, int k_per_split, long long split_stride,
    const GemmGroup grp) {
  if (gridDim.y > 1) {
    A = grp.A[blockIdx.y];
    B = grp.B[blockIdx.y];
    Cv = grp.C[blockIdx.y];
  }
  constexpr int NW = WM * WN;
  constexpr int NT = NW * 64;
  constexpr int TM = BM / WM / 16;
  constexpr int TN = BN / WN / 16;
  constexpr int A_BYTES = BM * BK * 2, B_BYTES = BN * BK * 2;
  constexpr int SB = A_BYTES + B_BYTES;
  using GA = Glds<A_KC, BM, NW>;
  using GB = Glds<B_KC, BN, NW>;
  constexpr int PT = GA::P + GB::P;
  extern __shared__ __attribute__((aligned(16))) char smem[];

  const int tid = threadIdx.x, lane = tid & 63;
  const int wid = __builtin_amdgcn_readfirstlane(tid >> 6);
  const int wm = wid / WN, wn = wid % WN;
  const int tiles_m = cdiv(M, BM), tiles_n = cdiv(N, BN);
  const int nwg = tiles_m * tiles_n;
  const int t = xcd_remap(blockIdx.x, nwg);
  int tm, tn;
  if (tiles_n <= tiles_m) {
    tn = t % tiles_n;
    tm = t / tiles_n;
  } else {
    tm = t % tiles_m;
    tn = t / tiles_m;
  }
  const int m0 = tm * BM, n0 = tn * BN;
  TDG_STAMP(0);

  const int kb = blockIdx.z * k_per_split;
  const int ke = min(K, kb + k_per_split);
  const int nk = cdiv(ke - kb, BK);
  const bool ktail = ((ke - kb) % BK) != 0;

  GA ga;
  GB gb;
  ga.init(wid, lane);
  gb.init(wid, lane);

  using OutT = typename std::conditional<OUT_F32, float, bf16_t>::type;
  constexpr int WTM = BM / WM, WTN = BN / WN;
  constexpr int RPASS = OUT_F32 ? (WTM < 32 ? WTM : 32) : WTM;
  using Epi = EpiLds<EPI, OUT_F32, TM, TN, RPASS>;
  using EpiF = EpiLds<EPI_NONE, true, TM, TN, (WTM < 32 ? WTM : 32)>;
  static_assert(NW * Epi::BYTES <= STAGES * (BM + BN) * BK * 2 &&
                    NW * EpiF::BYTES <= STAGES * (BM + BN) * BK * 2,
                "epilogue images must fit in the pipeline LDS");
  const bool split = gridDim.z > 1;
  const bool vec = epi_vec_ok<EPI, OUT_F32>(Cv, ldc, aux, ldaux);
  constexpr bool SINGLE = RPASS == WTM;
  const bool pre_aux = SINGLE && EPI == EPI_DRELU && !split && vec && (ldaux % 8) == 0 &&
                       (reinterpret_cast<uintptr_t>(aux) & 15) == 0;
  const bool pre_c = SINGLE && beta != 0.f && !split && vec && ((ldc * (int)sizeof(OutT)) % 16) == 0;
  int4 aux_r[Epi::ITER], c_r[Epi::ITER];
#pragma unroll
  for (int t = 0; t < Epi::ITER; ++t) {
    const int m = m0 + wm * WTM + Epi::row_of(lane, t);
    const int n = n0 + wn * WTN + Epi::col_of(lane, t);
    const bool in = m < M && n + Epi::EPC <= N;
    if (pre_aux && in) aux_r[t] = *reinterpret_cast<const int4*>(aux + (size_t)m * ldaux + n);
    if (pre_c && in)
      c_r[t] = *reinterpret_cast<const int4*>(reinterpret_cast<const OutT*>(Cv) + (size_t)m * ldc + n);
  }
  uint32_t mask_r[Epi::MBR];
  if constexpr (EPI == EPI_DRELU_BITS)
    Epi::mask_load(mask_r, reinterpret_cast<const unsigned char*>(aux), ldaux, M, N, m0 + wm * WTM,
                   n0 + wn * WTN, lane);

  f32x4 acc[TM][TN];
#pragma unroll
  for (int i = 0; i < TM; ++i)
#pragma unroll
    for (int j = 0; j < TN; ++j) acc[i][j] = f32x4{0.f, 0.f, 0.f, 0.f};

  static_assert(BK == 64, "two 32-deep k-steps per tile");
  const int abase = wm * (BM / WM), bbase = wn * (BN / WN);
#pragma unroll
  for (int s = 0; s < STAGES; ++s) {
    if (s < nk) {
// ... 37 lines not shown
#pragma unroll
      for (int j = 0; j < TN; ++j) acc[i][j] = mfma16(fb0[j], fa0[i], acc[i][j]);
    prio_lo();
    if constexpr (MODE >= 1) {
      if constexpr (MODE >= 2) wait_vmcnt<(STAGES - 2) * PT>();
      else wait_vmcnt<0>();
      lds_barrier();
      const char* nx = smem + ((kt + 1) % STAGES) * SB;
      if constexpr (MODE <= 2) {
        if (ktail && kt + 1 == nk - 1) {
          GA::zero_ktail(const_cast<char*>(nx), kb + (kt + 1) * BK, ke, tid, NT);
          GB::zero_ktail(const_cast<char*>(nx) + A_BYTES, kb + (kt + 1) * BK, ke, tid, NT);
          lds_barrier();
        }
      }
      if constexpr (MODE == 3) {
        char* ns = smem + (kt % STAGES) * SB;
        ga.issue(A, lda, M, ke, m0, kb + (kt + STAGES) * BK, ns, wid);
        gb.issue(B, ldb, N, ke, n0, kb + (kt + STAGES) * BK, ns + A_BYTES, wid);
      }
#pragma unroll
      for (int i = 0; i < TM; ++i) fa0[i] = frag<A_KC, BM>(nx, abase + 16 * i, 0, lane);
#pragma unroll
      for (int j = 0; j < TN; ++j) fb0[j] = frag<B_KC, BN>(nx + A_BYTES, bbase + 16 * j, 0, lane);
    } else {
      lgkm_wait<0>();
    }
    tie_all(fa1);
    tie_all(fb1);
    prio_hi();
#pragma unroll
    for (int i = 0; i < TM; ++i)
#pragma unroll
      for (int j = 0; j < TN; ++j) acc[i][j] = mfma16(fb1[j], fa1[i], acc[i][j]);
    prio_lo();
  };
  {
    int kt = 0;
    for (; kt + STAGES < nk; ++kt) kstep(kt, std::integral_constant<int, 3>{});
    if (kt + STAGES - 1 < nk && kt + 1 < nk) kstep(kt++, std::integral_constant<int, 2>{});
    for (; kt + 1 < nk; ++kt) kstep(kt, std::integral_constant<int, 1>{});
    if (kt < nk) kstep(kt, std::integral_constant<int, 0>{});
  }

  TDG_STAMP(2);
  lds_barrier();
  const int mw0 = m0 + wm * WTM, nw0 = n0 + wn * WTN;
  if (split) {
    float* Cs = reinterpret_cast<float*>(Cv) + (size_t)blockIdx.z * split_stride;
    EpiF::run(smem + wid * EpiF::BYTES, acc, lane, Cs, ldc, M, N, mw0, nw0, 1.f, 0.f, nullptr,
              nullptr, 0, epi_vec_ok<EPI_NONE, true>(Cs, ldc, nullptr, 0));
  } else {
    Epi::template run_pre<true>(smem + wid * Epi::BYTES, acc, lane, Cv, ldc, M, N, mw0, nw0, alpha,
                                beta, bias, aux, ldaux, vec, aux_r, pre_aux, c_r, pre_c, mask_r);
  }
#ifdef TDG_STAMPS
  TDG_STAMP(3);
  asm volatile("s_waitcnt vmcnt(0)" ::: "memory");
  TDG_STAMP(4);
#endif
}

constexpr int R256_MAXP = 64, R256_MAXC = 8;
struct R256Class {
  int M, N, lda, ldb, ldc, tiles_m, tiles_n, tile_start, prob_start, t_first;
};
struct R256Args {
  const bf16_t* A[R256_MAXP];
  const bf16_t* B[R256_MAXP];
  void* C[R256_MAXP];
  float* bias_out[R256_MAXP];
  R256Class cls[R256_MAXC];
  int ncls;
};

template <bool A_KC, bool B_KC, int EPI, bool OUT_F32>
__global__ __launch_bounds__(512) void gemm256_kernel(const R256Args args,
                                                      const float* __restrict__ bias,
                                                      const bf16_t* __restrict__ aux, int K,
                                                      int ldaux, float alpha, float beta) {
  constexpr int NW = 8;
  constexpr int HB = 128 * BK * 2;
  constexpr int SB = 4 * HB;
  using GA = Glds<A_KC, 128, NW>;
  using GB = Glds<B_KC, 128, NW>;
  static_assert(GA::P == 2 && GB::P == 2, "half-tile = 2 pieces per wave");
  extern __shared__ __attribute__((aligned(16))) char smem[];

  const int tid = threadIdx.x, lane = tid & 63;
  const int wid = __builtin_amdgcn_readfirstlane(tid >> 6);
  const int wm = wid >> 2, wn = wid & 3;

  const int t0 = xcd_remap(blockIdx.x, gridDim.x);
  R256Class cl = args.cls[0];
#pragma unroll
  for (int i = 1; i < R256_MAXC; ++i)
    if (i < args.ncls && t0 >= args.cls[i].tile_start) cl = args.cls[i];
  const int M = cl.M, N = cl.N, lda = cl.lda, ldb = cl.ldb, ldc = cl.ldc;
  const int tpp = cl.tiles_m * cl.tiles_n;
  const int lt = t0 - cl.tile_start + cl.t_first;
  const int p = cl.prob_start + lt / tpp;
  const int t = lt % tpp;
  const bf16_t* __restrict__ A = args.A[p];
  const bf16_t* __restrict__ B = args.B[p];
  void* __restrict__ Cv = args.C[p];
  int tm, tn;
  if (cl.tiles_n <= cl.tiles_m) {
    tn = t % cl.tiles_n;
    tm = t / cl.tiles_n;
  } else {
    tm = t % cl.tiles_m;
    tn = t / cl.tiles_m;
  }
  float* __restrict__ bias_out = A_KC ? nullptr : args.bias_out[p];
  const bool do_bsum = bias_out != nullptr && tn == 0;
  float bsum0 = 0.f, bsum1 = 0.f;
  const int m0 = tm * 256, n0 = tn * 256;
  const int nk = K / BK;
  TDG_STAMP(0);

  GA ga;
  GB gb;
  ga.init(wid, lane);
  gb.init(wid, lane);
  uint32_t a_off[2][2], b_off[2][2];
#pragma unroll
  for (int i = 0; i < 2; ++i) {
    const int xa = A_KC ? ga.row[i] : ga.col[i];
    const int xb = B_KC ? gb.row[i] : gb.col[i];
    const int ka = A_KC ? ga.col[i] : ga.row[i];
    const int kb = B_KC ? gb.col[i] : gb.row[i];
#pragma unroll
    for (int hh = 0; hh < 2; ++hh) {
      int ma = m0 + (xa >> 6) * 128 + hh * 64 + (xa & 63);
      int nb = n0 + (xb >> 5) * 64 + hh * 32 + (xb & 31);
      if (A_KC) {
        ma = ma < M ? ma : M - 1;
        a_off[hh][i] = 2u * (uint32_t)(ma * lda + ka);
      } else {
        ma = ma < M ? ma : 0;
        a_off[hh][i] = 2u * (uint32_t)(ka * lda + ma);
      }
      if (B_KC) {
        nb = nb < N ? nb : N - 1;
        b_off[hh][i] = 2u * (uint32_t)(nb * ldb + kb);
      } else {
        nb = nb < N ? nb : 0;
        b_off[hh][i] = 2u * (uint32_t)(kb * ldb + nb);
      }
    }
  }
  const int nrec_a = 2 * (A_KC ? (M - 1) * lda + K : (K - 1) * lda + ((M + 7) & ~7));
  const int nrec_b = 2 * (B_KC ? (N - 1) * ldb + K : (K - 1) * ldb + ((N + 7) & ~7));
  const uint32_t kstep_a = A_KC ? BK * 2u : (uint32_t)BK * (uint32_t)lda * 2u;
  const uint32_t kstep_b = B_KC ? BK * 2u : (uint32_t)BK * (uint32_t)ldb * 2u;
  auto issue = [&](const bf16_t* X, int nrec, const uint32_t* offs, uint32_t soff, char* dst) {
#pragma unroll
    for (int i = 0; i < 2; ++i)
      __builtin_amdgcn_raw_ptr_buffer_load_lds(
          __builtin_amdgcn_make_buffer_rsrc(const_cast<bf16_t*>(X), (short)0, nrec, 0x00020000),
          (__attribute__((address_space(3))) void*)(dst + (wid * 2 + i) * 1024), 16, offs[i],
          (int)soff, 0, 0);
  };
  auto issue_half = [&](int kt, int h) {
    char* st = smem + (kt & 1) * SB;
    if (h == 0) issue(A, nrec_a, a_off[0], kstep_a * (uint32_t)kt, st + 0 * HB);
// ... 120 lines not shown
          lgkm_wait<0>();
          if (ph == 0) {
#pragma unroll
            for (int i = 0; i < 4; ++i) tie_all(fa[i]);
#pragma unroll
            for (int j = 0; j < 2; ++j) tie_all(fb[j]);
          } else if (ph == 1) {
#pragma unroll
            for (int j = 2; j < 4; ++j) tie_all(fb[j]);
          } else {
#pragma unroll
            for (int i = 4; i < 8; ++i) tie_all(fa[i]);
          }
        }
        const int i0 = (ph < 2) ? 0 : 4;
        const int j0 = (ph == 0 || ph == 3) ? 0 : 2;
        __builtin_amdgcn_s_setprio(1);
#pragma unroll
        for (int s2 = 0; s2 < 2; ++s2)
#pragma unroll
          for (int i = 0; i < 4; ++i)
#pragma unroll
            for (int j = 0; j < 2; ++j)
              acc[i0 + i][j0 + j] = mfma16(fb[j0 + j][s2], fa[i0 + i][s2], acc[i0 + i][j0 + j]);
        __builtin_amdgcn_s_setprio(0);
        if (do_bsum && (ph == 0 || ph == 2)) bias_sum(ph);
      }
    };
    int kt = 0;
    for (; kt + 2 < nk; ++kt) kstep_deep(kt, std::integral_constant<int, 3>{});
    if (kt + 1 < nk) kstep_deep(kt++, std::integral_constant<int, 2>{});
    kstep_deep(kt, std::integral_constant<int, 1>{});
  }
  if (do_bsum) {
    bsum0 += __shfl_xor(bsum0, 16, 64);
    bsum0 += __shfl_xor(bsum0, 32, 64);
    bsum1 += __shfl_xor(bsum1, 16, 64);
    bsum1 += __shfl_xor(bsum1, 32, 64);
    if (lane < 16) {
      const int mA = m0 + wm * 128 + 16 * wn + lane, mB = mA + 64;
      if (mA < M) bias_out[mA] = alpha * bsum0 + (beta != 0.f ? beta * bias_out[mA] : 0.f);
      if (mB < M) bias_out[mB] = alpha * bsum1 + (beta != 0.f ? beta * bias_out[mB] : 0.f);
    }
  }

  TDG_STAMP(2);
  wait_vmcnt<0>();
  lds_barrier();
  {
    static_assert(8 * Epi::BYTES <= 2 * 4 * 128 * BK * 2, "epilogue images fit in the stages");
    if constexpr (EPI == EPI_DRELU_BITS)
      Epi::run_mask(smem + wid * Epi::BYTES, acc, lane, Cv, ldc, M, N, m0 + wm * 128, n0 + wn * 64,
                    alpha, beta, bias, aux, ldaux, epi_vec_ok<EPI, OUT_F32>(Cv, ldc, aux, ldaux),
                    mask_r);
    else
      Epi::run(smem + wid * Epi::BYTES, acc, lane, Cv, ldc, M, N, m0 + wm * 128, n0 + wn * 64, alpha,
               beta, bias, aux, ldaux, epi_vec_ok<EPI, OUT_F32>(Cv, ldc, aux, ldaux));
  }
#ifdef TDG_STAMPS
  TDG_STAMP(3);
  asm volatile("s_waitcnt vmcnt(0)" ::: "memory");
  TDG_STAMP(4);
#endif
}

template <int EPI, bool OUT_F32>
__global__ void splitk_reduce_kernel(const float* __restrict__ ws, void* __restrict__ Cv,
                                     const float* __restrict__ bias, const bf16_t* __restrict__ aux,
                                     int M, int N, int ldc, int ldaux, int splits,
                                     long long split_stride, float alpha, float beta) {
  const long long total = (long long)M * N;
  for (long long idx = (long long)blockIdx.x * blockDim.x + threadIdx.x; idx < total;
       idx += (long long)gridDim.x * blockDim.x) {
    const int m = (int)(idx / N), n = (int)(idx % N);
    const size_t o = (size_t)m * ldc + n;
    float v = 0.f;
    for (int z = 0; z < splits; ++z) v += ws[(size_t)z * split_stride + o];
    v *= alpha;
    if constexpr (EPI == EPI_BIAS) v += bias[n];
    if constexpr (EPI == EPI_BIAS_RELU) v = fmaxf(v + bias[n], 0.f);
    if constexpr (EPI == EPI_DRELU) {
      if (!(bf2f(aux[(size_t)m * ldaux + n]) > 0.f)) v = 0.f;
    }
    if constexpr (OUT_F32) {
      float* C = reinterpret_cast<float*>(Cv);
      if (beta != 0.f) v += beta * C[o];
      C[o] = v;
    } else {
      bf16_t* C = reinterpret_cast<bf16_t*>(Cv);
      if (beta != 0.f) v += beta * bf2f(C[o]);
      C[o] = f2bf(v);
    }
  }
}

}

using namespace tdg;

namespace tdg {
enum PlanFamily : int { PLAN_LOCK = 0, PLAN_R256 = 1, PLAN_PIPE = 2 };
int* gemm_plan_slot();
inline void plan_record(int family, int bm, int bn, int depth, int splits) {
  int* p = gemm_plan_slot();
  p[0] = family; p[1] = bm; p[2] = bn; p[3] = depth; p[4] = splits;
}
}

namespace {

template <int BM, int BN, int WM, int WN, int ST, bool AK, bool BKc, int EPI, bool F32>
void launch_cfg(const bf16_t* A, const bf16_t* B, void* C, const float* bias, const bf16_t* aux,
                int M, int N, int K, int lda, int ldb, int ldc, int ldaux, float alpha, float beta,
                int splits, float* ws, hipStream_t st, const GemmGroup* grp = nullptr, int G = 1) {
  static const GemmGroup kNoGroup{};
  const GemmGroup& gr = grp ? *grp : kNoGroup;
  const int tiles = cdiv(M, BM) * cdiv(N, BN);
  const int lds = ST * (BM + BN) * BK * 2;
  static bool attr_set = false;
  if (!attr_set) {
    (void)hipFuncSetAttribute((const void*)gemm_kernel<BM, BN, WM, WN, ST, AK, BKc, EPI, F32>,
                              hipFuncAttributeMaxDynamicSharedMemorySize, 160 * 1024);
    (void)hipFuncSetAttribute((const void*)gemm_kernel<BM, BN, WM, WN, ST, AK, BKc, EPI_NONE, true>,
                              hipFuncAttributeMaxDynamicSharedMemorySize, 160 * 1024);
    attr_set = true;
  }
  if (splits <= 1 || G > 1) {
    plan_record(PLAN_LOCK, BM, BN, ST, 1);
    hipLaunchKernelGGL((gemm_kernel<BM, BN, WM, WN, ST, AK, BKc, EPI, F32>), dim3(tiles, G, 1),
                       dim3(WM * WN * 64), lds, st, A, B, C, bias, aux, M, N, K, lda, ldb, ldc,
                       ldaux, alpha, beta, K, 0LL, gr);
  } else {
    int kps = cdiv(cdiv(K, splits), BK) * BK;
    splits = cdiv(K, kps);
    const long long stride = (long long)M * ldc;
    plan_record(PLAN_LOCK, BM, BN, ST, splits);
    hipLaunchKernelGGL((gemm_kernel<BM, BN, WM, WN, ST, AK, BKc, EPI_NONE, true>),
                       dim3(tiles, 1, splits), dim3(WM * WN * 64), lds, st, A, B, (void*)ws, bias,
                       aux, M, N, K, lda, ldb, ldc, ldaux, 1.f, 0.f, kps, stride, gr);
    const long long total = (long long)M * N;
    const int blocks = (int)std::min<long long>(4096, (total + 255) / 256);
    hipLaunchKernelGGL((splitk_reduce_kernel<EPI, F32>), dim3(blocks), dim3(256), 0, st, ws, C,
                       bias, aux, M, N, ldc, ldaux, splits, stride, alpha, beta);
  }
}

template <bool AK, bool BKc, int EPI, bool F32>
constexpr bool has_256() {
  if (AK && BKc) return !F32 || EPI == EPI_NONE;
  if (AK && !BKc) return !F32 && (EPI == EPI_NONE || EPI == EPI_DRELU || EPI == EPI_DRELU_BITS);
  if (!AK && !BKc) return EPI == EPI_NONE;
  return false;
}

inline bool r256_offsets_ok(const R256Args& a, bool akc, bool bkc, int K) {
  for (int c = 0; c < a.ncls; ++c) {
    const R256Class& k = a.cls[c];
    const long long ea = akc ? (long long)(k.M - 1) * k.lda + K : (long long)(K - 1) * k.lda + ((k.M + 7) & ~7);
    const long long eb = bkc ? (long long)(k.N - 1) * k.ldb + K : (long long)(K - 1) * k.ldb + ((k.N + 7) & ~7);
    if (ea * 2 >= 0x7fffffffLL || eb * 2 >= 0x7fffffffLL) return false;
  }
  return true;
}

template <bool AK, bool BKc, int EPI, bool F32>
int launch_256(const R256Args& args, int tiles, const float* bias, const bf16_t* aux, int K,
               int ldaux, float alpha, float beta, hipStream_t st) {
  if constexpr (!has_256<AK, BKc, EPI, F32>()) {
    return -4;
  } else {
    if (K % BK != 0 || tiles <= 0) return -3;
    if (!r256_offsets_ok(args, AK, BKc, K)) return -9;
    constexpr int lds = 2 * 4 * 128 * BK * 2;
    static bool attr = false;
    if (!attr) {
      (void)hipFuncSetAttribute((const void*)gemm256_kernel<AK, BKc, EPI, F32>,
                                hipFuncAttributeMaxDynamicSharedMemorySize, 160 * 1024);
      attr = true;
    }
    plan_record(PLAN_R256, 256, 256, 2, 1);
    hipLaunchKernelGGL((gemm256_kernel<AK, BKc, EPI, F32>), dim3(tiles), dim3(512), lds, st, args,
                       bias, aux, K, ldaux, alpha, beta);
    return 0;
  }
}

inline int r256_single(R256Args& a, const bf16_t* const* A, const bf16_t* const* B,
                       void* const* C, int G, int M, int N, int lda, int ldb, int ldc) {
  a.ncls = 1;
  for (int i = 0; i < G; ++i) {
    a.A[i] = A[i];
    a.B[i] = B[i];
    a.C[i] = C[i];
  }
  R256Class& c = a.cls[0];
  c.M = M; c.N = N; c.lda = lda; c.ldb = ldb; c.ldc = ldc;
  c.tiles_m = cdiv(M, 256); c.tiles_n = cdiv(N, 256);
  c.tile_start = 0; c.prob_start = 0; c.t_first = 0;
  return G * c.tiles_m * c.tiles_n;
}

template <int BM, int BN, int WM, int WN, int NS, bool AK, bool BKc, int EPI, bool F32>
bool launch_pipe(const bf16_t* A, const bf16_t* B, void* C, const float* bias, const bf16_t* aux,
                 int M, int N, int K, int lda, int ldb, int ldc, int ldaux, float alpha, float beta,
                 hipStream_t st) {
  if constexpr (epi_has_bits(EPI) && BN / WN > 64) return false;
  else {
  if (K % PK != 0 || K <= 0) return false;
  const long long ab = AK ? (long long)(M - 1) * lda + K : (long long)(K - 1) * lda + ((M + 7) & ~7);
  const long long bb = BKc ? (long long)(N - 1) * ldb + K : (long long)(K - 1) * ldb + ((N + 7) & ~7);
  if (ab * 2 >= 0x7fffffffLL || bb * 2 >= 0x7fffffffLL) return false;
  if ((!AK && lda % 8) || (!BKc && ldb % 8)) return false;
  constexpr int lds = NS * (BM + BN) * PK * 2;
  static bool attr = false;
  if (!attr) {
    (void)hipFuncSetAttribute((const void*)gemm_pipe_kernel<BM, BN, WM, WN, NS, AK, BKc, EPI, F32>,
                              hipFuncAttributeMaxDynamicSharedMemorySize, 160 * 1024);
    attr = true;
  }
  const int tiles = cdiv(M, BM) * cdiv(N, BN);
  plan_record(PLAN_PIPE, BM, BN, NS, 1);
  hipLaunchKernelGGL((gemm_pipe_kernel<BM, BN, WM, WN, NS, AK, BKc, EPI, F32>), dim3(tiles),
                     dim3(WM * WN * 64), lds,
                     st, A, B, C, bias, aux, M, N, K, lda, ldb, ldc, ldaux, alpha, beta,
                     (int)(ab * 2), (int)(bb * 2));
  return true;
  }
}

template <bool AK, bool BKc, int EPI, bool F32>
void launch_tiles(int tile_cfg, const bf16_t* A, const bf16_t* B, void* C, const float* bias,
                  const bf16_t* aux, int M, int N, int K, int lda, int ldb, int ldc, int ldaux,
                  float alpha, float beta, int splits, float* ws, hipStream_t st,
                  const GemmGroup* grp = nullptr, int G = 1) {
  if (tile_cfg >= 20 && tile_cfg <= 26) {
    if (!grp && splits <= 1) {
      bool ok = false;
#define TDG_PIPE(ID, BM_, BN_, WM_, WN_, NS_)                                                      \
  case ID:                                                                                    \
    ok = launch_pipe<BM_, BN_, WM_, WN_, NS_, AK, BKc, EPI, F32>(A, B, C, bias, aux, M, N, K, lda, \
                                                                 ldb, ldc, ldaux, alpha, beta, st); \
    break;
      switch (tile_cfg) {
        TDG_PIPE(20, 256, 256, 2, 4, 4)
        TDG_PIPE(21, 256, 128, 2, 4, 6)
        TDG_PIPE(22, 128, 256, 2, 4, 6)
        TDG_PIPE(23, 256, 256, 2, 2, 4)
        TDG_PIPE(24, 256, 256, 2, 2, 5)
        TDG_PIPE(25, 256, 128, 2, 2, 6)
        TDG_PIPE(26, 128, 256, 2, 2, 6)
        default: break;
      }
#undef TDG_PIPE
      if (ok) return;
    }
    tile_cfg = 13;
  }
  if (tile_cfg == 12) {
    if (splits <= 1 && (AK || lda % 8 == 0) && (BKc || ldb % 8 == 0)) {
      R256Args args{};
      const bf16_t* a1 = A;
      const bf16_t* b1 = B;
      void* c1 = C;
      const int tiles = grp ? r256_single(args, grp->A, grp->B, grp->C, G, M, N, lda, ldb, ldc)
                            : r256_single(args, &a1, &b1, &c1, 1, M, N, lda, ldb, ldc);
      if (launch_256<AK, BKc, EPI, F32>(args, tiles, bias, aux, K, ldaux, alpha, beta, st) == 0)
        return;
    }
    tile_cfg = 13;
  }
#define TDG_CFG(ID, BM_, BN_, WM_, WN_, ST_)                                                  \
  case ID:                                                                                    \
    launch_cfg<BM_, BN_, WM_, WN_, ST_, AK, BKc, EPI, F32>(A, B, C, bias, aux, M, N, K, lda, ldb, \
                                                          ldc, ldaux, alpha, beta, splits, ws,   \
                                                          st, grp, G);                           \
    break;
  switch (tile_cfg) {
    TDG_CFG(0, 128, 128, 2, 2, 2)
// ... 99 lines not shown
```

csrc/kernels/gemm_pipe.h:

```cpp
#pragma once
#include "tdg_common.h"
#include "tdg_gemm.h"

namespace tdg {

constexpr int PK = 32;

template <bool KC, int R>
__device__ __forceinline__ int plds_off(int row, int byte) {
  if constexpr (KC) {
    const int ch = (byte >> 4) ^ (((row >> 3) & 1) << 1);
    return row * 64 + (ch << 4) + (byte & 15);
  } else {
    return lds_off<false, R>(row, byte);
  }
}

template <bool KC, int R, int NW>
struct PStage {
  static constexpr int BYTES = R * PK * 2;
  static constexpr int P = BYTES / (NW * 1024);
  static_assert(BYTES % (NW * 1024) == 0, "tile must split into 1 KiB pieces per wave");
  uint32_t voff[P];
  const bf16_t* base;
// ... 120 lines not shown
                                                  int abase, int bbase, float (&bs)[TM],
                                                  bool do_bs) {
    if (STEADY || kt + 1 < nk) {
      if constexpr (STEADY) wait_vmcnt<(NS - 3) * PT>();
      else wait_tiles<PT, NS - 2>(kt == 0 ? min(NS - 2, nk - 2) : min(NS - 3, nk - 2 - kt));
      __builtin_amdgcn_s_barrier();
    }
    const char* nx = smem + ((kt + 1) % NS) * SB;
    const int rt = kt - 1 + NS;
    const bool refill = STEADY || (rt < nk && kt >= 1);
#pragma unroll
    for (int j = 0; j < TN; ++j) {
      throttle<FBt>();
      FN[j].read(nx + A_BYTES, bbase + 16 * j, lane);
    }
#pragma unroll
    for (int i = 0; i < TM; ++i) {
      lgkm_wait<LGKM>();
      fa[i].tie_();
      if (i == 0) {
#pragma unroll
        for (int j = 0; j < TN; ++j) FB[j].tie_();
      }
      const short8_t a = fa[i].get();
      __builtin_amdgcn_s_setprio(1);
#pragma unroll
      for (int j = 0; j < TN; ++j) acc[i][j] = mfma16(FB[j].get(), a, acc[i][j]);
      __builtin_amdgcn_s_setprio(0);
      if constexpr (BS) {
        if (do_bs) {
          const bf16x2_t one = __builtin_bit_cast(bf16x2_t, 0x3f803f80);
          float b = bs[i];
#pragma unroll
          for (int e = 0; e < 4; ++e)
            b = __builtin_amdgcn_fdot2_f32_bf16(
                __builtin_bit_cast(bf16x2_t, (short2_t){a[2 * e], a[2 * e + 1]}), one, b, false);
          bs[i] = b;
        }
      }
      throttle<FA>();
      fa[i].read(nx, abase + 16 * i, lane);
#pragma unroll
      for (int q = 0; q < PT; ++q)
        if (q * TM / PT == i && refill) stage_piece(sa, sb, smem, q, rt, wid);
      __builtin_amdgcn_sched_barrier(0);
    }
  }
};

template <int BM, int BN, int WM, int WN, int NS, bool A_KC, bool B_KC, int EPI, bool OUT_F32>
__global__ __launch_bounds__(WM * WN * 64) void gemm_pipe_kernel(
    const bf16_t* __restrict__ A, const bf16_t* __restrict__ B, void* __restrict__ Cv,
    const float* __restrict__ bias, const bf16_t* __restrict__ aux, int M, int N, int K, int lda,
    int ldb, int ldc, int ldaux, float alpha, float beta, int a_bytes, int b_bytes) {
  using P = Pipe<BM, BN, WM, WN, NS, A_KC, B_KC>;
  constexpr int NW = P::NW, TM = P::TM, TN = P::TN, A_BYTES = P::A_BYTES, SB = P::SB, PT = P::PT;
  constexpr int WTM = BM / WM, WTN = BN / WN;
  static_assert(NS >= 3, "ring: refilled, being read, landed");
  extern __shared__ __attribute__((aligned(16))) char smem[];

  const int tid = threadIdx.x, lane = tid & 63;
  const int wid = __builtin_amdgcn_readfirstlane(tid >> 6);
  const int wm = wid / WN, wn = wid % WN;
  const int tiles_m = cdiv(M, BM), tiles_n = cdiv(N, BN);
  const int t = xcd_remap(blockIdx.x, tiles_m * tiles_n);
  int tm, tn;
  if (tiles_n <= tiles_m) {
    tn = t % tiles_n;
    tm = t / tiles_n;
  } else {
    tm = t % tiles_m;
    tn = t / tiles_m;
  }
  const int m0 = tm * BM, n0 = tn * BN;
  const int nk = K / PK;

  typename P::SA sa;
  typename P::SBt sb;
  sa.init(A, lda, M, m0, a_bytes, wid, lane);
  sb.init(B, ldb, N, n0, b_bytes, wid, lane);
  f32x4 acc[TM][TN];
#pragma unroll
  for (int i = 0; i < TM; ++i)
#pragma unroll
    for (int j = 0; j < TN; ++j) acc[i][j] = f32x4{0.f, 0.f, 0.f, 0.f};

  const int abase = wm * WTM, bbase = wn * WTN;
  constexpr int RPASS = OUT_F32 ? (WTM < 32 ? WTM : 32) : (WTM > 64 ? 64 : WTM);
  using Epi = EpiLds<EPI, OUT_F32, TM, TN, RPASS>;
  uint32_t mask_r[Epi::MBR];
  if constexpr (EPI == EPI_DRELU_BITS)
    Epi::mask_load(mask_r, reinterpret_cast<const unsigned char*>(aux), ldaux, M, N, m0 + abase,
                   n0 + bbase, lane);
#pragma unroll
  for (int s = 0; s < NS - 1; ++s)
    if (s < nk) P::stage(sa, sb, smem, s, wid);
  wait_tiles<PT, NS - 2>(min(NS - 1, nk) - 1);
  __builtin_amdgcn_s_barrier();
  typename P::FA fa[TM];
  typename P::FBt fb[TN], fbn[TN];
#pragma unroll
  for (int j = 0; j < TN; ++j) {
    lgkm_wait<15 - P::FBt::NI>();
    fb[j].read(smem + A_BYTES, bbase + 16 * j, lane);
  }
#pragma unroll
  for (int i = 0; i < TM; ++i) {
    lgkm_wait<15 - P::FA::NI>();
    fa[i].read(smem, abase + 16 * i, lane);
  }

  if (NS - 1 < nk) P::stage(sa, sb, smem, NS - 1, wid);
  int kt = 0;
  if (nk > 0) P::ktile(kt++, nk, fb, fbn, fa, acc, sa, sb, smem, lane, wid, abase, bbase);
  for (; kt + 1 <= nk - NS; kt += 2) {
    P::ktile_s(kt, nk, fbn, fb, fa, acc, sa, sb, smem, lane, wid, abase, bbase);
    P::ktile_s(kt + 1, nk, fb, fbn, fa, acc, sa, sb, smem, lane, wid, abase, bbase);
  }
  for (; kt + 1 < nk; kt += 2) {
    P::ktile(kt, nk, fbn, fb, fa, acc, sa, sb, smem, lane, wid, abase, bbase);
    P::ktile(kt + 1, nk, fb, fbn, fa, acc, sa, sb, smem, lane, wid, abase, bbase);
  }
  if (kt < nk) P::ktile(kt, nk, fbn, fb, fa, acc, sa, sb, smem, lane, wid, abase, bbase);

  lgkm_wait<0>();
  wait_vmcnt<0>();
  lds_barrier();
  {
    using OutT = typename std::conditional<OUT_F32, float, bf16_t>::type;
    (void)sizeof(OutT);
    static_assert(NW * Epi::BYTES <= NS * SB, "epilogue images fit in the stages");
    if constexpr (EPI == EPI_DRELU_BITS)
      Epi::run_mask(smem + wid * Epi::BYTES, acc, lane, Cv, ldc, M, N, m0 + wm * WTM, n0 + wn * WTN,
                    alpha, beta, bias, aux, ldaux, epi_vec_ok<EPI, OUT_F32>(Cv, ldc, aux, ldaux),
                    mask_r);
    else
      Epi::run(smem + wid * Epi::BYTES, acc, lane, Cv, ldc, M, N, m0 + wm * WTM, n0 + wn * WTN, alpha,
               beta, bias, aux, ldaux, epi_vec_ok<EPI, OUT_F32>(Cv, ldc, aux, ldaux));
  }
}

}
```

csrc/kernels/norm.hip:

```cpp
#include "tdg_api.h"
#include "tdg_common.h"
#include "tdg_ln.h"
#include "tdg_reduce.h"

namespace tdg {

template <int D, int FMT = 0>
__device__ __forceinline__ void ln_row_y8(const RowVec<D / 64>& o, float s8, uint8_t* __restrict__ y8,
                                          size_t rbase, int lane, float& am, const WtBuf& wt) {
  constexpr int VEC = D / 64;
  int w[(VEC + 3) / 4];
#pragma unroll
  for (int i = 0; i < (VEC + 3) / 4; ++i) w[i] = 0;
#pragma unroll
  for (int i = 0; i < VEC; i += 2) {
    const float a = bf2f(f2bf(o.v[i])), b = bf2f(f2bf(o.v[i + 1]));
    am = fmaxf(am, fmaxf(fabsf(a), fabsf(b)));
    if constexpr (FMT == 0) {
      if ((i & 2) == 0) w[i / 4] = pack2_e4m3<false>(a * s8, b * s8, w[i / 4]);
      else w[i / 4] = pack2_e4m3<true>(a * s8, b * s8, w[i / 4]);
    } else {
      if ((i & 2) == 0) w[i / 4] = pack2_e5m2c<false>(a * s8, b * s8, w[i / 4]);
      else w[i / 4] = pack2_e5m2c<true>(a * s8, b * s8, w[i / 4]);
    }
  }
  uint8_t* dst = y8 + rbase + lane * RowMap<VEC>::W;
  if constexpr (VEC == 2) {
    *reinterpret_cast<uint16_t*>(dst) = (uint16_t)(w[0] & 0xffff);
  } else if constexpr (VEC == 4) {
    wt.st4(dst, (uint32_t)w[0]);
  } else {
#pragma unroll
    for (int i = 0; i < VEC / 8; ++i) wt.st8(dst + 512 * i, make_int2(w[2 * i], w[2 * i + 1]));
  }
}

__device__ __forceinline__ void ln_amax_flush(float am, float* red8, unsigned* amax8) {
  am = wave_max(am);
  if ((threadIdx.x & 63) == 0) red8[threadIdx.x >> 6] = am;
  __syncthreads();
  if (threadIdx.x == 0 && amax8)
    atomic_amax(amax_word(amax8, blockIdx.x), fmaxf(fmaxf(red8[0], red8[1]), fmaxf(red8[2], red8[3])));
}

template <int D, int RPW>
__global__ __launch_bounds__(256) void ln_fwd_kernel(
    const bf16_t* __restrict__ x, const bf16_t* __restrict__ s, const float* __restrict__ gamma,
    const float* __restrict__ beta, bf16_t* __restrict__ y, bf16_t* __restrict__ hsave,
    float* __restrict__ mean_out, float* __restrict__ rstd_out, int M, float p, uint32_t thresh,
    uint64_t seed, const long long* ctr, uint64_t site, float eps, uint8_t* __restrict__ y8,
    const float* __restrict__ s8p, unsigned* __restrict__ amax8, uint8_t* __restrict__ kbits) {
  constexpr int VEC = D / 64;
  const int lane = threadIdx.x & 63;
  const int r0 = (blockIdx.x * 4 + (threadIdx.x >> 6)) * RPW;
  __shared__ float red8[4];
  RowVec<VEC> h[RPW], t[RPW];
#pragma unroll
  for (int k = 0; k < RPW; ++k) {
    const size_t rbase = (size_t)min(r0 + k, M - 1) * D;
    h[k].load_row(x + rbase, lane);
    if (s) t[k].load_row(s + rbase, lane);
  }
  float am = 0.f;
#pragma unroll
  for (int k = 0; k < RPW; ++k) {
    const int row = r0 + k;
    if (row >= M) break;
    const size_t rbase = (size_t)row * D;
    RowVec<VEC> o;
    ln_row_fwd<D>(h[k], t[k], s != nullptr, rbase, row, lane, gamma, beta, y, hsave, mean_out,
                  rstd_out, p, thresh, seed, ctr, site, eps, o, (size_t)M * D * sizeof(bf16_t), kbits);
    if (y8) ln_row_y8<D>(o, s8p[0], y8, rbase, lane, am, WtBuf(y8, (size_t)M * D));
  }
  if (y8) ln_amax_flush(am, red8, amax8);
}

template <int D, int RPW, int NWV>
__global__ __launch_bounds__(NWV * 64) void ln_bwd_kernel(
    const bf16_t* __restrict__ dy, const bf16_t* __restrict__ hsave,
    const float* __restrict__ mean_in, const float* __restrict__ rstd_in,
    const float* __restrict__ gamma, bf16_t* __restrict__ dh_out, bf16_t* __restrict__ ds_out,
    const bf16_t* __restrict__ dres_in, float* __restrict__ part_g, float* __restrict__ part_b,
    float* __restrict__ part_s, int M, float p, uint32_t thresh, uint64_t seed,
    const long long* ctr, uint64_t site, int iters, uint8_t* __restrict__ ds8,
    const float* __restrict__ s8p, unsigned* __restrict__ amax8,
    const uint8_t* __restrict__ kbits) {
  constexpr int VEC = D / 64;
  __shared__ float red[NWV][D];
  float am8 = 0.f;
  const int lane = threadIdx.x & 63, w = threadIdx.x >> 6;
  float ag[VEC], ab[VEC], as[VEC];
#pragma unroll
  for (int i = 0; i < VEC; ++i) ag[i] = ab[i] = as[i] = 0.f;
  float gm[VEC];
#pragma unroll
  for (int i = 0; i < VEC; ++i) gm[i] = gamma[RowMap<VEC>::col(lane, i)];
  const float sc = p > 0.f ? 1.f / (1.f - p) : 1.f;
  const WtBuf wdh(dh_out, (size_t)M * D * sizeof(bf16_t));
  const WtBuf wds(ds_out ? ds_out : dh_out, (size_t)M * D * sizeof(bf16_t));
#pragma unroll 1
  for (int it = 0; it < iters; ++it) {
  const int r0 = (blockIdx.x * iters + it) * (NWV * RPW) + w * RPW;
  if (r0 >= M) break;
  RowVec<VEC> g[RPW], h[RPW], e[RPW];
  float mean[RPW], rstd[RPW];
  uint32_t kb[RPW];
#pragma unroll
  for (int k = 0; k < RPW; ++k) {
    const int row = min(r0 + k, M - 1);
    const size_t rbase = (size_t)row * D;
    g[k].load_row(dy + rbase, lane);
    h[k].load_row(hsave + rbase, lane);
    if (dres_in) e[k].load_row(dres_in + rbase, lane);
    mean[k] = mean_in[row];
    rstd[k] = rstd_in[row];
    kb[k] = 0u;
    if constexpr (VEC >= 8) {
      if (kbits) {
#pragma unroll
        for (int c = 0; c < RowMap<VEC>::CH; ++c) kb[k] |= (uint32_t)kbits[rbase / 8 + 64 * c + lane] << (8 * c);
      }
    }
  }
#pragma unroll
  for (int k = 0; k < RPW; ++k) {
    const int row = r0 + k;
    if (row >= M) break;
    const size_t rbase = (size_t)row * D;
    float sg = 0.f, sgx = 0.f;
    float xh[VEC];
#pragma unroll
    for (int i = 0; i < VEC; ++i) {
      xh[i] = (h[k].v[i] - mean[k]) * rstd[k];
      ag[i] += g[k].v[i] * xh[i];
      ab[i] += g[k].v[i];
      const float gg = g[k].v[i] * gm[i];
      sg += gg;
      sgx += gg * xh[i];
    }
    sg = wave_sum(sg) * (1.f / D);
    sgx = wave_sum(sgx) * (1.f / D);
    RowVec<VEC> dh;
#pragma unroll
    for (int i = 0; i < VEC; ++i) dh.v[i] = rstd[k] * (g[k].v[i] * gm[i] - sg - xh[i] * sgx);
    RowVec<VEC> ds = dh;
    if (p > 0.f) {
      const uint32_t km = (VEC >= 8 && kbits) ? kb[k] : keep_bits<VEC>(seed, ctr, site, rbase, lane, thresh);
#pragma unroll
      for (int i = 0; i < VEC; ++i) ds.v[i] = ((km >> i) & 1u) ? dh.v[i] * sc : 0.f;
    }
    if (ds_out || ds8) {
      if (ds_out) ds.store_row(ds_out + rbase, lane, wds);
      if (ds8) ln_row_y8<D, 1>(ds, s8p[0], ds8, rbase, lane, am8, WtBuf(ds8, (size_t)M * D));
#pragma unroll
      for (int i = 0; i < VEC; ++i) as[i] += ds.v[i];
    }
    if (dres_in) {
#pragma unroll
      for (int i = 0; i < VEC; ++i) dh.v[i] += e[k].v[i];
    }
    dh.store_row(dh_out + rbase, lane, wdh);
  }
  }
  float* const parts[3] = {part_g, part_b, part_s};
#pragma unroll
  for (int q = 0; q < 3; ++q) {
    if (q == 2 && !part_s) break;
#pragma unroll
    for (int i = 0; i < VEC; ++i) red[w][RowMap<VEC>::col(lane, i)] = q == 0 ? ag[i] : q == 1 ? ab[i] : as[i];
    __syncthreads();
    for (int col = threadIdx.x; col < D; col += NWV * 64) {
      float a = 0.f;
#pragma unroll
      for (int k = 0; k < NWV; ++k) a += red[k][col];
      parts[q][(size_t)blockIdx.x * D + col] = a;
    }
    __syncthreads();
  }
  if (ds8) {
    am8 = wave_max(am8);
    if (lane == 0) red[0][w] = am8;
    __syncthreads();
    if (threadIdx.x == 0 && amax8) {
      float m = 0.f;
#pragma unroll
      for (int k = 0; k < NWV; ++k) m = fmaxf(m, red[0][k]);
      atomic_amax(amax_word(amax8, blockIdx.x), m);
    }
  }
}

}

using namespace tdg;

namespace {
template <int D>
void ln_fwd_d(const void* x, const void* s, const float* gamma, const float* beta, void* y,
              void* hsave, float* mean, float* rstd, int M, float p, uint64_t seed,
              const long long* ctr, uint64_t site, float eps, void* y8, const float* s8,
              unsigned* amax8, void* kbits, hipStream_t st) {
  const uint32_t thresh = dropout_thresh(p);
  hipLaunchKernelGGL((ln_fwd_kernel<D, 1>), dim3(cdiv(M, 4)), dim3(256), 0, st, (const bf16_t*)x,
                     (const bf16_t*)s, gamma, beta, (bf16_t*)y, (bf16_t*)hsave, mean, rstd, M, p,
                     thresh, seed, ctr, site, eps, (uint8_t*)y8, s8, amax8, (uint8_t*)kbits);
}
template <int D>
void ln_bwd_d(const void* dy, const void* hsave, const float* mean, const float* rstd,
              const float* gamma, void* dh, void* ds, const void* dres, float* dgamma,
              float* dbeta, float* dbias, float* ws, int M, float p, uint64_t seed, const long long* ctr, uint64_t site,
              int accumulate, int skip_reduce, int rpb, void* ds8, const float* s8, unsigned* amax8,
              const void* kbits, hipStream_t st) {
  const uint32_t thresh = dropout_thresh(p);
  constexpr int RPW = D >= 1024 ? 2 : 4;
  const int nb = cdiv(M, rpb);
  float* pg = ws;
  float* pb = ws + (size_t)nb * D;
  float* ps = dbias ? ws + 2 * (size_t)nb * D : nullptr;
  if (rpb <= 16)
    hipLaunchKernelGGL((ln_bwd_kernel<D, RPW, 4>), dim3(nb), dim3(256), 0, st, (const bf16_t*)dy,
                       (const bf16_t*)hsave, mean, rstd, gamma, (bf16_t*)dh, (bf16_t*)ds,
                       (const bf16_t*)dres, pg, pb, ps, M, p, thresh, seed, ctr, site,
                       max(1, rpb / (RPW * 4)), (uint8_t*)ds8, s8, amax8, (const uint8_t*)kbits);
  else
    hipLaunchKernelGGL((ln_bwd_kernel<D, RPW, 8>), dim3(nb), dim3(512), 0, st, (const bf16_t*)dy,
                       (const bf16_t*)hsave, mean, rstd, gamma, (bf16_t*)dh, (bf16_t*)ds,
                       (const bf16_t*)dres, pg, pb, ps, M, p, thresh, seed, ctr, site,
                       max(1, rpb / (RPW * 8)), (uint8_t*)ds8, s8, amax8, (const uint8_t*)kbits);
  if (skip_reduce) return;
  const float beta = accumulate ? 1.f : 0.f;
  ReduceSet rs{{pg, pb, ps}, {dgamma, dbeta, dbias}};
  hipLaunchKernelGGL(reduce_partials3_kernel, dim3(cdiv(D, 16), dbias ? 3 : 2), dim3(256), 0, st,
                     rs, D, nb, beta);
}
}

extern "C" int tdg_ln_fwd(const void* x, const void* s, const float* gamma, const float* beta,
                          void* y, void* hsave, float* mean, float* rstd, int M, int D, float p,
                          uint64_t seed, const long long* ctr, uint64_t site, float eps, void* y8,
                          const float* s8, unsigned* amax8, void* kbits, hipStream_t st) {
  if (kbits && D < 512) return -3;
#define TDG_LN_F(DD) \
  ln_fwd_d<DD>(x, s, gamma, beta, y, hsave, mean, rstd, M, p, seed, ctr, site, eps, y8, s8, amax8, kbits, st); \
  return 0;
  switch (D) {
    case 128: TDG_LN_F(128)
    case 256: TDG_LN_F(256)
    case 512: TDG_LN_F(512)
    case 1024: TDG_LN_F(1024)
    default: return -1;
  }
#undef TDG_LN_F
}

extern "C" int tdg_ln_bwd(const void* dy, const void* hsave, const float* mean, const float* rstd,
                          const float* gamma, void* dh, void* ds, const void* dres, float* dgamma,
                          float* dbeta, float* dbias, float* ws, int M, int D, float p,
                          uint64_t seed, const long long* ctr, uint64_t site, int accumulate,
                          int skip_reduce, int rpb, void* ds8, const float* s8, unsigned* amax8,
                          const void* kbits, hipStream_t st) {
  if (rpb != 16 && rpb != 32 && rpb != 64) return -2;
  if (ds8 && !s8) return -2;
  if (kbits && D < 512) return -3;
#define TDG_LN_B(DD)                                                                              \
  ln_bwd_d<DD>(dy, hsave, mean, rstd, gamma, dh, ds, dres, dgamma, dbeta, dbias, ws, M, p, seed, \
               ctr, site, accumulate, skip_reduce, rpb, ds8, s8, amax8, kbits, st);              \
  return 0;
  switch (D) {
    case 128: TDG_LN_B(128)
    case 256: TDG_LN_B(256)
    case 512: TDG_LN_B(512)
    case 1024: TDG_LN_B(1024)
    default: return -1;
  }
#undef TDG_LN_B
}

namespace tdg {
constexpr int MAXR = 96;
struct MultiReduce {
  const float* part[MAXR];
  float* out[MAXR];
  int nparts[MAXR];
};
__global__ __launch_bounds__(256) void reduce_partials_multi_kernel(MultiReduce mr, int N,
                                                                    float beta) {
  __shared__ float red[16][17];
  const float* part = mr.part[blockIdx.y];
  float* out = mr.out[blockIdx.y];
  const int P = mr.nparts[blockIdx.y];
  const int c = threadIdx.x & 15, g = threadIdx.x >> 4;
  const int col = blockIdx.x * 16 + c;
  float s = 0.f;
  if (col < N) {
#pragma unroll 8
    for (int q = g; q < P; q += 16) s += part[(size_t)q * N + col];
  }
  red[g][c] = s;
  __syncthreads();
  if (g == 0 && col < N) {
    float t = 0.f;
#pragma unroll
    for (int k = 0; k < 16; ++k) t += red[k][c];
    out[col] = (beta != 0.f ? beta * out[col] : 0.f) + t;
  }
}
__global__ __launch_bounds__(256) void reduce_partials_multi4_kernel(MultiReduce mr, int N,
                                                                     float beta) {
  __shared__ float4 red[16][17];
  const float* part = mr.part[blockIdx.y];
  float* out = mr.out[blockIdx.y];
  const int P = mr.nparts[blockIdx.y];
  const int c = threadIdx.x & 15, g = threadIdx.x >> 4;
  const int col = blockIdx.x * 64 + c * 4;
  float4 s = make_float4(0.f, 0.f, 0.f, 0.f);
  if (col < N) {
#pragma unroll 8
    for (int q = g; q < P; q += 16) {
      const float4 v = *reinterpret_cast<const float4*>(part + (size_t)q * N + col);
      s.x += v.x;
      s.y += v.y;
      s.z += v.z;
      s.w += v.w;
    }
  }
  red[g][c] = s;
  __syncthreads();
  if (g == 0 && col < N) {
// ... 44 lines not shown
```

tensorflow_distributed_on_gke_amd/ops/kernels.py:

```python
from __future__ import annotations

import math
import os
from typing import Dict, List, Optional, Tuple

import torch

from tensorflow_distributed_on_gke_amd.ops._ext import C

EPI_NONE, EPI_BIAS, EPI_BIAS_RELU, EPI_DRELU = 0, 1, 2, 3
NUM_CU = 256

_WS: Dict[Tuple[int, int, str], torch.Tensor] = {}
_WS_RETIRED: List[torch.Tensor] = []


def workspace(name: str, numel: int, device, dtype=torch.float32, zero: bool = False) -> torch.Tensor:
    dev = torch.device(device)
    sid = torch.cuda.current_stream(dev).stream_id if dev.type == "cuda" else 0
    key = (dev.index or 0, sid, name)
    t = _WS.get(key)
    if t is None or t.numel() < numel or t.dtype != dtype:
        if t is not None:
            _WS_RETIRED.append(t)
        t = (torch.zeros if zero else torch.empty)(max(numel, 1), dtype=dtype, device=dev)
        _WS[key] = t
    return t


def reset_workspace() -> None:
    _WS.clear()
    _WS_RETIRED.clear()


_TILES = {0: (128, 128), 1: (128, 64), 2: (64, 128), 3: (64, 64), 4: (128, 128), 5: (256, 128),
          6: (128, 256), 7: (64, 128), 8: (64, 64), 9: (256, 128), 10: (128, 256), 11: (128, 128),
          12: (256, 256), 13: (128, 128), 14: (128, 128),
          20: (256, 256), 21: (256, 128), 22: (128, 256)}
_CFG_OVERRIDE: Dict[Tuple[int, int, int, bool, bool], Tuple[int, int]] = {}


def set_gemm_config(M: int, N: int, K: int, a_kc: bool, b_kc: bool, cfg: int, splits: int) -> None:
    _CFG_OVERRIDE[(M, N, K, a_kc, b_kc)] = (cfg, splits)


def choose_gemm(M: int, N: int, K: int, a_kc: bool = True, b_kc: bool = True) -> Tuple[int, int]:
    o = _CFG_OVERRIDE.get((M, N, K, a_kc, b_kc))
    if o is not None:
        return o
    if not a_kc and not b_kc:
        t128 = math.ceil(M / 128) * math.ceil(N / 128)
        splits = 1
        while t128 * splits < NUM_CU and K // (splits * 2) >= 512:
            splits *= 2
        return 0, splits
    if K % 64 == 0 and math.ceil(M / 256) * math.ceil(N / 256) >= 192:
        return 12, 1
    if a_kc and not b_kc and N >= 1024 and math.ceil(M / 128) * math.ceil(N / 256) >= NUM_CU:
        return 6, 1
    return (13, 1) if not b_kc else (4, 1)


_TUNED: Dict[tuple, Tuple[int, int]] = {}
AUTOTUNE = os.environ.get("TDG_GEMM_AUTOTUNE", "0") == "1"
# ... 23 lines not shown
            except RuntimeError:
                continue
            times[cfg] = min(t, times.get(cfg, float("inf")))
    return min(times, key=times.get)


def _key_str(k: tuple) -> str:
    M, N, K, a_kc, b_kc, epi, dt, ld8, beta = k
    return f"{M},{N},{K},{int(a_kc)},{int(b_kc)},{epi},{str(dt).replace('torch.', '')},{int(ld8)},{int(beta)}"


def save_tuned(path: str) -> None:
    import json

    with open(path, "w") as f:
        json.dump({_key_str(k): list(v[0]) for k, v in sorted(_TUNED.items(), key=lambda kv: str(kv[0]))},
                  f, indent=0)


def load_tuned(path: str) -> int:
    import json

    if not os.path.exists(path):
        return 0
    with open(path) as f:
        data = json.load(f)
    for ks, v in data.items():
        M, N, K, a, b, epi, dt, ld8, beta = ks.split(",")
        key = (int(M), int(N), int(K), bool(int(a)), bool(int(b)), int(epi), getattr(torch, dt),
               bool(int(ld8)), bool(int(beta)))
        cfg = (int(v[0]), int(v[1]))
        _TUNED[key] = (cfg, cfg)
    return len(data)


TUNED_FILE = os.environ.get("TDG_GEMM_TUNED_FILE") or os.path.join(
    os.path.dirname(os.path.abspath(__file__)), "gemm_tuned_gfx950.json")
load_tuned(TUNED_FILE)


def _tok_bucket(v: int) -> int:
    return -(-v // 1024) * 1024


def gemm(A, B, Cout, M, N, K, lda, ldb, ldc, a_kc, b_kc, epi=EPI_NONE, bias=None, aux=None,
         ldaux=0, alpha=1.0, beta=0.0, cfg: Optional[Tuple[int, int]] = None,
         relu_bits: Optional[torch.Tensor] = None) -> torch.Tensor:

    def run(c, out=Cout):
        tile, splits = c
        ws = workspace("splitk", splits * M * ldc, A.device) if splits > 1 else None
        if relu_bits is None:
            C().gemm(A, B, out, bias, aux, M, N, K, lda, ldb, ldc, ldaux, a_kc, b_kc, epi, alpha,
                     beta, tile, splits, ws)
        else:
            C().gemm(A, B, out, bias, aux, M, N, K, lda, ldb, ldc, ldaux, a_kc, b_kc, epi, alpha,
                     beta, tile, splits, ws, relu_bits=relu_bits, ldbits=relu_bits.stride(0))

    if cfg is None:
        Mk, Kk = (M, _tok_bucket(K)) if (not a_kc and not b_kc) else (_tok_bucket(M), K)
        key = (Mk, N, Kk, a_kc, b_kc, epi, Cout.dtype, ldc % 8 == 0, beta != 0.0)
        ent = _TUNED.get(key)
        if ent is None:
            o = _CFG_OVERRIDE.get((M, N, K, a_kc, b_kc))
            if o is not None:
                ent = (o, o)
        if ent is None and AUTOTUNE and A.is_cuda and not torch.cuda.is_current_stream_capturing():
            if beta != 0.0:
                scratch = workspace("tune_c", Cout.numel(), A.device, Cout.dtype)[: Cout.numel()]
                scratch = scratch.view_as(Cout)
                best = _autotune(key, lambda c: run(c, scratch))
            else:
                best = _autotune(key, run)
            ent = (best, best)
            _TUNED[key] = ent
        if ent is None:
            cfg = choose_gemm(M, N, K, a_kc, b_kc)
        else:
            cfg = ent[0]
    run(cfg)
    return Cout


def tuned_table() -> Dict[str, str]:
    return {f"{k[0]}x{k[1]}x{k[2]} a_kc={k[3]} b_kc={k[4]} epi={k[5]}": f"cfg{v[0]} split{v[1]}"
            for k, v in _TUNED.items()}


def pack_relu_bits(h: torch.Tensor) -> torch.Tensor:
    M, N = h.shape
    w = (1 << torch.arange(8, device=h.device, dtype=torch.int32))
    return ((h > 0).view(M, N // 8, 8).to(torch.int32) * w).sum(-1).to(torch.uint8)


def linear_fwd(x2: torch.Tensor, w: torch.Tensor, bias: Optional[torch.Tensor], relu: bool = False,
               out: Optional[torch.Tensor] = None, ldc: Optional[int] = None,
               relu_bits: Optional[torch.Tensor] = None) -> torch.Tensor:
    M, K = x2.shape
    N = w.shape[0]
    ldc = ldc or N
    if out is None:
        out = torch.empty(M, ldc, dtype=torch.bfloat16, device=x2.device)
    epi = EPI_BIAS_RELU if relu else (EPI_BIAS if bias is not None else EPI_NONE)
    if relu_bits is not None and not relu:
        raise ValueError("linear_fwd: relu_bits needs relu=True")
    return gemm(x2, w, out, M, N, K, x2.stride(0), w.stride(0), ldc, True, True, epi, bias=bias,
                relu_bits=relu_bits)


def linear_dgrad(dy2: torch.Tensor, w: torch.Tensor, N: int, relu_aux: Optional[torch.Tensor] = None,
# ... 239 lines not shown


def beam_topk(logits, V: int, score, fin, beam: int, end_id: int, pad_id: int, anc=None, t: int = 0,
              anc_out=None):
    R = logits.shape[0]
    if not 1 <= beam <= 8 or not 1 <= V <= 65536:
        raise RuntimeError(f"beam_topk: beam {beam} outside [1, 8] or V {V} outside [1, 65536]")
    dev = logits.device
    if logits.is_cuda:
        score_out = torch.empty(R, dtype=torch.float32, device=dev)
        parent, token, fin_out = (torch.empty(R, dtype=torch.int32, device=dev) for _ in range(3))
        if anc is not None and anc_out is None:
            anc_out = torch.zeros_like(anc)
        C().beam_topk(logits, V, score, fin, beam, end_id, pad_id, score_out, parent, token, fin_out,
                      anc, anc_out, t)
        return score_out, parent, token, fin_out, anc_out
    B = R // beam
    x = logits[:, :V].float()
    logp = x - torch.logsumexp(x, dim=-1, keepdim=True)
    cand = score.float().view(R, 1) + logp
    ended = fin.view(R, 1) != 0
    only_pad = torch.full_like(cand, float("-inf"))
    only_pad[:, pad_id] = score.float()
    cand = torch.where(ended, only_pad, cand)
    cand = torch.where(torch.isnan(cand) | ~(score.float() > float("-inf")).view(R, 1),
                       torch.full_like(cand, float("-inf")), cand)
    flat = cand.view(B, beam * V)
    order = torch.sort(-flat, dim=-1, stable=True).indices[:, :beam]
    val = torch.gather(flat, 1, order)
    dead = ~(val > float("-inf"))
    base = (torch.arange(B) * beam).view(B, 1)
    parent = torch.where(dead, base.expand(B, beam), base + order // V)
    token = torch.where(dead, torch.full_like(order, pad_id), order % V)
    fin_out = dead | (fin.view(R)[parent.view(R)].view(B, beam) != 0) | (token == end_id)
    score_out = torch.where(dead, torch.full_like(val, float("-inf")), val)
    parent = parent.reshape(R).to(torch.int32)
    if anc is not None:
        if anc_out is None:
            anc_out = torch.zeros_like(anc)
        anc_out[:, : t + 1] = anc[parent.long(), : t + 1]
        anc_out[:, t + 1] = torch.arange(R, dtype=anc.dtype)
    return (score_out.reshape(R), parent, token.reshape(R).to(torch.int32),
            fin_out.reshape(R).to(torch.int32), anc_out)


def ln_fwd(x, s, gamma, beta, p, seed, ctr, site, eps=1e-6, save=True, y8=None, s8=None,
           amax8=None, kbits=None):
    D = x.shape[-1]
    M = x.numel() // D
    y = torch.empty_like(x)
    h = torch.empty_like(x) if save else None
    mean = torch.empty(M, dtype=torch.float32, device=x.device) if save else None
    rstd = torch.empty(M, dtype=torch.float32, device=x.device) if save else None
    C().ln_fwd(x, s, gamma, beta, y, h, mean, rstd, p, seed, ctr, site, eps, y8, s8, amax8, kbits)
    return y, h, mean, rstd


LN_BWD_RPB = int(os.environ.get("TDG_LN_BWD_RPB", "0") or 0)


def ln_bwd_rpb(D: int) -> int:
    return LN_BWD_RPB or (32 if D <= 512 else 16)


def ln_bwd_nparts(M: int, D: int) -> int:
    return math.ceil(M / ln_bwd_rpb(D))


def ln_bwd(dy, h, mean, rstd, gamma, dgamma, dbeta, dbias, p, seed, ctr, site, want_ds=True,
           dres=None, accumulate=False, defer=None, ds8=None, s8=None, amax8=None, kbits=None):
    D = dy.shape[-1]
    M = dy.numel() // D
    dh = torch.empty_like(dy)
    need_ds = (want_ds and (p > 0 or dres is not None)) or (dbias is not None and ds8 is None)
    ds = torch.empty_like(dy) if need_ds else None
    if defer is None:
        ws = workspace("ln_bwd", 3 * ln_bwd_nparts(M, D) * D, dy.device)
    else:
        ws = workspace(f"ln_bwd_part_{site}", 3 * ln_bwd_nparts(M, D) * D, dy.device)
    C().ln_bwd(dy, h, mean, rstd, gamma, dh, ds, dres, dgamma, dbeta, dbias, ws, p, seed, ctr, site,
               accumulate, defer is not None, ln_bwd_rpb(D), ds8, s8, amax8, kbits)
    if defer is not None:
        nb = ln_bwd_nparts(M, D)
        outs = [dgamma, dbeta] + ([dbias] if dbias is not None else [])
        for i, o in enumerate(outs):
            defer.append((ws[i * nb * D:(i + 1) * nb * D], o, nb, D, 1.0 if accumulate else 0.0))
    if ds is None:
        ds = dh
    return dh, ds


def reduce_partials_multi(items) -> None:
    groups = {}
    for part, out, nparts, N, beta in items:
        groups.setdefault((N, beta), []).append((part, out, nparts))
    for (N, beta), its in groups.items():
        for c0 in range(0, len(its), 96):
            ch = its[c0:c0 + 96]
            C().reduce_partials_multi([i[0] for i in ch], [i[1] for i in ch], [i[2] for i in ch],
                                      N, beta)


def embed_fwd(tok, table, pe, scale, p, seed, ctr, site, kbits=None):
    B, L = tok.shape
    D = table.shape[1]
    out = torch.empty(B, L, D, dtype=torch.bfloat16, device=tok.device)
    C().embed_fwd(tok, table, pe, out, scale, p, seed, ctr, site, kbits)
    return out


DETERMINISTIC_EMBED = os.environ.get("TDG_DETERMINISTIC", "1") != "0"


EMBED_CSR = os.environ.get("TDG_EMBED_CSR", "1") != "0"


class EmbCsr:

    def __init__(self, tok: torch.Tensor, V: int, name: str):
        self.tok, self.V, self.M = tok, int(V), tok.numel()
        n32, _ = C().embed_csr_ws(self.M, self.V, 128)
        self.w32 = workspace("embed_csr32_" + name, n32, tok.device, torch.int32)


def embed_csr_ok(M: int, V: int) -> bool:
    return DETERMINISTIC_EMBED and EMBED_CSR and C().embed_csr_ok(M, V)


def embed_csr_sort(tables, stamps=None) -> list:
    cs = [EmbCsr(t.contiguous(), V, name) for t, V, name in tables]
    C().embed_csr_sort([c.tok for c in cs], [c.V for c in cs], [c.w32 for c in cs], stamps)
    return cs


def embed_csr_apply(cs: EmbCsr, dout, dtable, scale, p, seed, ctr, site, accumulate=False,
                    kbits=None) -> None:
    _, n64 = C().embed_csr_ws(cs.M, cs.V, dtable.shape[1])
    w64 = workspace("embed_csr64", n64, dtable.device, torch.int64)
    C().embed_csr_apply(dout, dtable, cs.w32, w64, cs.M, scale, p, seed, ctr, site, accumulate, kbits)


def embed_bwd(tok, dout, dtable, scale, p, seed, ctr, site, accumulate=False, kbits=None,
              csr: Optional[EmbCsr] = None):
    if csr is not None or embed_csr_ok(tok.numel(), dtable.shape[0]):
        if csr is None:
            csr = embed_csr_sort([(tok, dtable.shape[0], "bwd")])[0]
        embed_csr_apply(csr, dout.contiguous(), dtable, scale, p, seed, ctr, site, accumulate, kbits)
        return
    if DETERMINISTIC_EMBED:
        acc = workspace("embed_fx", dtable.numel(), dtable.device, torch.int64, zero=True)
        C().embed_bwd_det(tok, dout, dtable, acc, scale, p, seed, ctr, site, accumulate)
    else:
        C().embed_bwd(tok, dout, dtable, scale, p, seed, ctr, site)


def count_tokens(labels, out):
    C().count_tokens(labels, out)


_PREP_SCRATCH: Dict[tuple, torch.Tensor] = {}
# ... 88 lines not shown
```

Before: 3.563 million tokens/s.

## Add XCD-aware block remapping for LayerNorm/embedding and selectable store cache flavour

```diff
diff --git a/csrc/bindings/embedding.cpp b/csrc/bindings/embedding.cpp
--- a/csrc/bindings/embedding.cpp
+++ b/csrc/bindings/embedding.cpp
@@ -25,7 +25,7 @@
 
 void embed_fwd(const Tensor& tok, const Tensor& table, const Tensor& pe, const Tensor& out,
                double scale, double p, int64_t seed, const optional<Tensor>& ctr, int64_t site,
-               const optional<Tensor>& kbits) {
+               const optional<Tensor>& kbits, bool band_order) {
   TORCH_CHECK(tok.dim() == 2, "tok must be [B,L]");
   const bool t64 = check_tok(tok);
   check_bf16(table, "table");
@@ -42,7 +42,7 @@
   const int rc = tdg_embed_fwd(tok.data_ptr(), t64, table.data_ptr(), pe.data_ptr<float>(),
                                out.data_ptr(), (int)M, (int)L, (int)D, (float)scale, (float)p,
                                (uint64_t)seed, ctr_ptr(ctr), (uint64_t)site, opt_ptr(kbits),
-                               stream_of(tok));
+                               band_order, stream_of(tok));
   check_err(rc, "tdg embed_fwd");
 }
 
@@ -145,7 +145,9 @@
 }
 
 void def_embedding(py::module_& m) {
-  m.def("embed_fwd", &embed_fwd);
+  m.def("embed_fwd", &embed_fwd, py::arg("tok"), py::arg("table"), py::arg("pe"), py::arg("out"),
+        py::arg("scale"), py::arg("p"), py::arg("seed"), py::arg("ctr"), py::arg("site"),
+        py::arg("kbits"), py::arg("band_order") = false);
   m.def("embed_bwd", &embed_bwd);
   m.def("embed_bwd_det", &embed_bwd_det);
   m.def("embed_csr_ws", &embed_csr_ws);
diff --git a/csrc/bindings/gemm.cpp b/csrc/bindings/gemm.cpp
--- a/csrc/bindings/gemm.cpp
+++ b/csrc/bindings/gemm.cpp
@@ -19,7 +19,7 @@
           const optional<Tensor>& aux, int64_t M, int64_t N, int64_t K, int64_t lda, int64_t ldb,
           int64_t ldc, int64_t ldaux, bool a_kc, bool b_kc, int64_t epi, double alpha,
           double beta, int64_t tile_cfg, int64_t splits, const optional<Tensor>& ws,
-          const optional<Tensor>& relu_bits, int64_t ldbits) {
+          const optional<Tensor>& relu_bits, int64_t ldbits, int64_t band_store) {
   TORCH_CHECK(C.is_cuda(), "C must be a GPU tensor");
   const bool f32 = C.scalar_type() == at::kFloat;
   TORCH_CHECK(f32 || C.scalar_type() == at::kBFloat16, "C must be f32 or bf16");
@@ -66,7 +66,7 @@
   const int rc = tdg_gemm(A.data_ptr(), B.data_ptr(), C.data_ptr(), bptr, xptr, (int)M, (int)N,
                           (int)K, (int)lda, (int)ldb, (int)ldc, (int)ldaux, a_kc, b_kc, (int)epi,
                           f32, (float)alpha, (float)beta, (int)tile_cfg, (int)splits, wptr,
-                          stream_of(A), bits, (int)ldbits);
+                          stream_of(A), bits, (int)ldbits, (int)band_store);
   check_err(rc, "tdg gemm");
 }
 
@@ -185,6 +185,19 @@
   return {p[0], p[1], p[2], p[3], p[4]};
 }
 
+std::vector<int64_t> band_of(const std::string& kind, int64_t M, int64_t N, int64_t K,
+                             int64_t block) {
+  static const char* const kinds[] = {"gemm128", "gemm256", "ln_fwd", "ln_bwd", "attn", "embed_fwd", "blocks"};
+  int k = -1;
+  for (int i = 0; i < 7; ++i)
+    if (kind == kinds[i]) k = i;
+  TORCH_CHECK(k >= 0, "band_of: kind is one of gemm128, gemm256, ln_fwd, ln_bwd, attn, embed_fwd, blocks");
+  int out[4];
+  TORCH_CHECK(tdg_band_of(k, (int)M, (int)N, (int)K, (int)block, out) == 0,
+              "band_of: block out of range or bad shape");
+  return {out[0], out[1], out[2], out[3]};
+}
+
 }
 
 void def_gemm(py::module_& m) {
@@ -192,12 +205,15 @@
         py::arg("M"), py::arg("N"), py::arg("K"), py::arg("lda"), py::arg("ldb"), py::arg("ldc"),
         py::arg("ldaux"), py::arg("a_kc"), py::arg("b_kc"), py::arg("epi"), py::arg("alpha"),
         py::arg("beta"), py::arg("tile_cfg"), py::arg("splits"), py::arg("ws"),
-        py::arg("relu_bits") = optional<Tensor>(), py::arg("ldbits") = 0);
+        py::arg("relu_bits") = optional<Tensor>(), py::arg("ldbits") = 0,
+        py::arg("band_store") = 0);
   m.def("gemm_grouped", &gemm_grouped);
   m.def("gemm_ragged", &gemm_ragged, py::arg("As"), py::arg("Bs"), py::arg("Cs"), py::arg("shapes"),
         py::arg("K"), py::arg("a_kc"), py::arg("b_kc"), py::arg("alpha"), py::arg("beta"),
         py::arg("bias_out") = std::vector<c10::optional<Tensor>>{});
   m.def("gemm_last_plan", &gemm_last_plan);
+  m.def("band_of", &band_of, py::arg("kind"), py::arg("M"), py::arg("N") = 0, py::arg("K") = 0,
+        py::arg("block") = 0);
   m.def("colsum", &colsum);
   m.def("colsum_grouped", &colsum_grouped);
 }
diff --git a/csrc/bindings/layernorm.cpp b/csrc/bindings/layernorm.cpp
--- a/csrc/bindings/layernorm.cpp
+++ b/csrc/bindings/layernorm.cpp
@@ -16,7 +16,8 @@
             const Tensor& y, const optional<Tensor>& hsave, const optional<Tensor>& mean,
             const optional<Tensor>& rstd, double p, int64_t seed, const optional<Tensor>& ctr,
             int64_t site, double eps, const optional<Tensor>& y8, const optional<Tensor>& s8,
-            const optional<Tensor>& amax8, const optional<Tensor>& kbits) {
+            const optional<Tensor>& amax8, const optional<Tensor>& kbits, bool band_order,
+            int64_t band_store) {
   check_bf16(x, "x");
   check_contig(x, "x");
   const int64_t D = x.size(-1), M = x.numel() / D;
@@ -51,7 +52,7 @@
                             beta.data_ptr<float>(), y.data_ptr(), opt_ptr(hsave), opt_f32(mean),
                             opt_f32(rstd), (int)M, (int)D, (float)p, (uint64_t)seed, ctr_ptr(ctr),
                             (uint64_t)site, (float)eps, opt_ptr(y8), opt_f32(s8), amax_ptr(amax8),
-                            opt_ptr(kbits), stream_of(x));
+                            opt_ptr(kbits), band_order, (int)band_store, stream_of(x));
   check_err(rc, "tdg ln_fwd");
 }
 
@@ -61,7 +62,8 @@
             const optional<Tensor>& dbias, const Tensor& ws, double p, int64_t seed,
             const optional<Tensor>& ctr, int64_t site, bool accumulate, bool skip_reduce,
             int64_t rpb, const optional<Tensor>& ds8, const optional<Tensor>& s8,
-            const optional<Tensor>& amax8, const optional<Tensor>& kbits) {
+            const optional<Tensor>& amax8, const optional<Tensor>& kbits, bool band_order,
+            int64_t band_store) {
   check_bf16(dy, "dy");
   check_contig(dy, "dy");
   const int64_t D = dy.size(-1), M = dy.numel() / D;
@@ -101,7 +103,8 @@
       gamma.data_ptr<float>(), dh.data_ptr(), opt_ptr(ds), opt_ptr(dres), dgamma.data_ptr<float>(),
       dbeta.data_ptr<float>(), opt_f32(dbias), ws.data_ptr<float>(), (int)M, (int)D, (float)p,
       (uint64_t)seed, ctr_ptr(ctr), (uint64_t)site, accumulate, skip_reduce, (int)rpb,
-      opt_ptr(ds8), opt_f32(s8), amax_ptr(amax8), opt_ptr(kbits), stream_of(dy));
+      opt_ptr(ds8), opt_f32(s8), amax_ptr(amax8), opt_ptr(kbits), band_order, (int)band_store,
+      stream_of(dy));
   check_err(rc, "tdg ln_bwd");
 }
 
@@ -134,7 +137,16 @@
 }
 
 void def_layernorm(py::module_& m) {
-  m.def("ln_fwd", &ln_fwd);
-  m.def("ln_bwd", &ln_bwd);
+  m.def("ln_fwd", &ln_fwd, py::arg("x"), py::arg("s"), py::arg("gamma"), py::arg("beta"),
+        py::arg("y"), py::arg("hsave"), py::arg("mean"), py::arg("rstd"), py::arg("p"),
+        py::arg("seed"), py::arg("ctr"), py::arg("site"), py::arg("eps"), py::arg("y8"),
+        py::arg("s8"), py::arg("amax8"), py::arg("kbits"), py::arg("band_order") = false,
+        py::arg("band_store") = 0);
+  m.def("ln_bwd", &ln_bwd, py::arg("dy"), py::arg("hsave"), py::arg("mean"), py::arg("rstd"),
+        py::arg("gamma"), py::arg("dh"), py::arg("ds"), py::arg("dres"), py::arg("dgamma"),
+        py::arg("dbeta"), py::arg("dbias"), py::arg("ws"), py::arg("p"), py::arg("seed"),
+        py::arg("ctr"), py::arg("site"), py::arg("accumulate"), py::arg("skip_reduce"),
+        py::arg("rpb"), py::arg("ds8"), py::arg("s8"), py::arg("amax8"), py::arg("kbits"),
+        py::arg("band_order") = false, py::arg("band_store") = 0);
   m.def("reduce_partials_multi", &reduce_partials_multi);
 }
diff --git a/csrc/include/tdg_api.h b/csrc/include/tdg_api.h
--- a/csrc/include/tdg_api.h
+++ b/csrc/include/tdg_api.h
@@ -10,7 +10,7 @@
 int tdg_gemm(const void* A, const void* B, void* C, const float* bias, const void* aux, int M,
              int N, int K, int lda, int ldb, int ldc, int ldaux, int a_kc, int b_kc, int epi,
              int out_f32, float alpha, float beta, int tile_cfg, int splits, float* ws,
-             hipStream_t st, void* relu_bits, int ldbits);
+             hipStream_t st, void* relu_bits, int ldbits, int band_store);
 int tdg_gemm_grouped(const void* const* A, const void* const* B, void* const* C, int G, int M,
                      int N, int K, int lda, int ldb, int ldc, int a_kc, int b_kc, int out_f32,
                      float alpha, float beta, int tile_cfg, hipStream_t st);
@@ -18,6 +18,8 @@
                     const int* shapes, int K, int a_kc, int b_kc, int out_f32, float alpha,
                     float beta, float* const* bias_out, hipStream_t st);
 void tdg_gemm_last_plan(int out[5]);
+
+int tdg_band_of(int kind, int M, int N, int K, int block, int out[4]);
 void tdg_colsum(const void* X, float* out, float* part, int M, int N, int ld, int rows_per_block,
                 float beta, hipStream_t st);
 int tdg_colsum_grouped(const void* const* X, float* const* out, int G, float* part, int M, int N,
@@ -37,18 +39,19 @@
 int tdg_ln_fwd(const void* x, const void* s, const float* gamma, const float* beta, void* y,
                void* hsave, float* mean, float* rstd, int M, int D, float p, uint64_t seed,
                const long long* ctr, uint64_t site, float eps, void* y8, const float* s8,
-               unsigned* amax8, void* kbits, hipStream_t st);
+               unsigned* amax8, void* kbits, int band_order, int band_store, hipStream_t st);
 int tdg_ln_bwd(const void* dy, const void* hsave, const float* mean, const float* rstd,
                const float* gamma, void* dh, void* ds, const void* dres, float* dgamma,
                float* dbeta, float* dbias, float* ws, int M, int D, float p, uint64_t seed,
                const long long* ctr, uint64_t site, int accumulate, int skip_reduce, int rpb,
-               void* ds8, const float* s8, unsigned* amax8, const void* kbits, hipStream_t st);
+               void* ds8, const float* s8, unsigned* amax8, const void* kbits, int band_order,
+               int band_store, hipStream_t st);
 int tdg_reduce_partials_multi(const float* const* parts, float* const* outs, const int* nparts,
                               int G, int N, float beta, hipStream_t st);
 
 int tdg_embed_fwd(const void* tok, int tok64, const void* table, const float* pe, void* out, int M,
                   int L, int D, float scale, float p, uint64_t seed, const long long* ctr,
-                  uint64_t site, void* kbits, hipStream_t st);
+                  uint64_t site, void* kbits, int band_order, hipStream_t st);
 int tdg_embed_bwd(const void* tok, int tok64, const void* dout, float* dtable, int M, int D,
                   float scale, float p, uint64_t seed, const long long* ctr, uint64_t site,
                   hipStream_t st);
diff --git a/csrc/include/tdg_bands.h b/csrc/include/tdg_bands.h
--- /dev/null
+++ b/csrc/include/tdg_bands.h
@@ -0,0 +1,46 @@
+#pragma once
+
+#ifndef __host__
+#define __host__
+#define __device__
+#endif
+
+namespace tdg {
+
+constexpr int NUM_XCD = 8;
+constexpr int BAND_EDGE_BYTES = 1 << 20;
+
+__host__ __device__ inline int xcd_remap(int bid, int nwg) {
+  constexpr int NX = NUM_XCD;
+  if (nwg <= NX) return bid;
+  const int q = nwg / NX, r = nwg % NX;
+  const int x = bid % NX, i = bid / NX;
+  const int base = (x < r) ? x * (q + 1) : r * (q + 1) + (x - r) * q;
+  return base + i;
+}
+__host__ __device__ inline int xcd_of_block(int bid) { return bid % NUM_XCD; }
+
+__host__ __device__ inline void tile_raster(int t, int tiles_m, int tiles_n, int& tm, int& tn) {
+  if (tiles_n <= tiles_m) {
+    tn = t % tiles_n;
+    tm = t / tiles_n;
+  } else {
+    tm = t % tiles_m;
+    tn = t / tiles_m;
+  }
+}
+
+__host__ __device__ inline int ln_block(int bid, int nblocks, int band_order) {
+  return band_order ? xcd_remap(bid, nblocks) : bid;
+}
+__host__ __device__ inline int ln_fwd_row0(int t, int wave, int rpw) { return (t * 4 + wave) * rpw; }
+__host__ __device__ inline int ln_bwd_row0(int t, int iters, int it, int rows_per_pass) {
+  return (t * iters + it) * rows_per_pass;
+}
+
+__host__ __device__ inline void attn_head_batch(int t, int H, int& h, int& b) {
+  h = t % H;
+  b = t / H;
+}
+
+}
diff --git a/csrc/include/tdg_common.h b/csrc/include/tdg_common.h
--- a/csrc/include/tdg_common.h
+++ b/csrc/include/tdg_common.h
@@ -2,6 +2,8 @@
 #include <hip/hip_runtime.h>
 #include <utility>
 #include <stdint.h>
+
+#include "tdg_bands.h"
 
 namespace tdg {
 
@@ -277,39 +279,47 @@
   return r;
 }
 
+enum StoreFlavour : int { ST_SC1 = 0, ST_NT = 1, ST_PLAIN = 2 };
 typedef unsigned int u32x4_t __attribute__((ext_vector_type(4)));
 typedef unsigned int u32x2_t __attribute__((ext_vector_type(2)));
 struct WtBuf {
   __amdgpu_buffer_rsrc_t r;
   const char* base;
-  bool ok;
-  __device__ __forceinline__ WtBuf(const void* p, size_t bytes)
+  int mode;
+  __device__ __forceinline__ WtBuf(const void* p, size_t bytes, int flavour = ST_SC1)
       : r(__builtin_amdgcn_make_buffer_rsrc(const_cast<void*>(p), 0,
                                              (int)(bytes < 0x7fffffffull ? bytes : 0x7fffffffull),
                                              0x00020000)),
         base(static_cast<const char*>(p)),
-        ok(bytes <= 0x7fffffffull) {}
+        mode(bytes <= 0x7fffffffull ? flavour : (int)ST_PLAIN) {}
   template <typename T>
   __device__ __forceinline__ void st16(void* p, const T& v) const {
     static_assert(sizeof(T) == 16, "16-byte value");
-    if (ok)
-      __builtin_amdgcn_raw_buffer_store_b128(__builtin_bit_cast(u32x4_t, v), r,
-                                             (int)(static_cast<const char*>(p) - base), 0, 16);
+    const int off = (int)(static_cast<const char*>(p) - base);
+    if (mode == ST_SC1)
+      __builtin_amdgcn_raw_buffer_store_b128(__builtin_bit_cast(u32x4_t, v), r, off, 0, 16);
+    else if (mode == ST_NT)
+      __builtin_amdgcn_raw_buffer_store_b128(__builtin_bit_cast(u32x4_t, v), r, off, 0, 2);
     else
       *static_cast<T*>(p) = v;
   }
   template <typename T>
   __device__ __forceinline__ void st8(void* p, const T& v) const {
     static_assert(sizeof(T) == 8, "8-byte value");
-    if (ok)
-      __builtin_amdgcn_raw_buffer_store_b64(__builtin_bit_cast(u32x2_t, v), r,
-                                            (int)(static_cast<const char*>(p) - base), 0, 16);
+    const int off = (int)(static_cast<const char*>(p) - base);
+    if (mode == ST_SC1)
+      __builtin_amdgcn_raw_buffer_store_b64(__builtin_bit_cast(u32x2_t, v), r, off, 0, 16);
+    else if (mode == ST_NT)
+      __builtin_amdgcn_raw_buffer_store_b64(__builtin_bit_cast(u32x2_t, v), r, off, 0, 2);
     else
       *static_cast<T*>(p) = v;
   }
   __device__ __forceinline__ void st4(void* p, uint32_t v) const {
-    if (ok)
-      __builtin_amdgcn_raw_buffer_store_b32(v, r, (int)(static_cast<const char*>(p) - base), 0, 16);
+    const int off = (int)(static_cast<const char*>(p) - base);
+    if (mode == ST_SC1)
+      __builtin_amdgcn_raw_buffer_store_b32(v, r, off, 0, 16);
+    else if (mode == ST_NT)
+      __builtin_amdgcn_raw_buffer_store_b32(v, r, off, 0, 2);
     else
       *static_cast<uint32_t*>(p) = v;
   }
@@ -339,13 +349,4 @@
   atomicMax(p, __float_as_uint(fabsf(v)));
 }
 
-__device__ __forceinline__ int xcd_remap(int bid, int nwg) {
-  constexpr int NX = 8;
-  if (nwg <= NX) return bid;
-  const int q = nwg / NX, r = nwg % NX;
-  const int x = bid % NX, i = bid / NX;
-  const int base = (x < r) ? x * (q + 1) : r * (q + 1) + (x - r) * q;
-  return base + i;
-}
-
-}
+}
diff --git a/csrc/include/tdg_gemm.h b/csrc/include/tdg_gemm.h
--- a/csrc/include/tdg_gemm.h
+++ b/csrc/include/tdg_gemm.h
@@ -301,21 +301,22 @@
                                              void* __restrict__ Cv, int ldc, int M, int N, int mw0,
                                              int nw0, float alpha, float beta,
                                              const float* __restrict__ bias,
-                                             const bf16_t* __restrict__ aux, int ldaux, bool vec) {
+                                             const bf16_t* __restrict__ aux, int ldaux, bool vec,
+                                             int store = ST_SC1) {
     int4 none[ITER];
     uint32_t nomask[MBR];
     run_pre<false>(wimg, acc, lane, Cv, ldc, M, N, mw0, nw0, alpha, beta, bias, aux, ldaux, vec,
-                   none, false, none, false, nomask);
+                   none, false, none, false, nomask, store);
   }
   __device__ static __forceinline__ void run_mask(char* wimg, const f32x4 (&acc)[TM][TN], int lane,
                                                   void* __restrict__ Cv, int ldc, int M, int N,
                                                   int mw0, int nw0, float alpha, float beta,
                                                   const float* __restrict__ bias,
                                                   const bf16_t* __restrict__ aux, int ldaux, bool vec,
-                                                  const uint32_t (&mb)[MBR]) {
+                                                  const uint32_t (&mb)[MBR], int store = ST_SC1) {
     int4 none[ITER];
     run_pre<false>(wimg, acc, lane, Cv, ldc, M, N, mw0, nw0, alpha, beta, bias, aux, ldaux, vec,
-                   none, false, none, false, mb);
+                   none, false, none, false, mb, store);
   }
   template <bool PRE>
   __device__ static __forceinline__ void run_pre(char* wimg, const f32x4 (&acc)[TM][TN], int lane,
@@ -325,13 +326,13 @@
                                                  const bf16_t* __restrict__ aux, int ldaux, bool vec,
                                                  const int4 (&pre_aux)[ITER], bool use_aux,
                                                  const int4 (&pre_c)[ITER], bool use_c,
-                                                 const uint32_t (&mb)[MBR]) {
+                                                 const uint32_t (&mb)[MBR], int store = ST_SC1) {
     const int g = lane >> 4, r16 = lane & 15;
     bool vok = vec && ((ldc * ES) % 16) == 0 && (reinterpret_cast<uintptr_t>(Cv) & 15) == 0;
     if constexpr (EPI == EPI_DRELU)
       vok = vok && (ldaux % EPC) == 0 && (reinterpret_cast<uintptr_t>(aux) % (2 * EPC)) == 0;
 #if TDG_EPI_SC1
-    const WtBuf wt(Cv, ((size_t)(M - 1) * ldc + N) * ES);
+    const WtBuf wt(Cv, ((size_t)(M - 1) * ldc + N) * ES, store);
 #endif
     f32x4 bn[TN];
 #pragma unroll
diff --git a/csrc/include/tdg_ln.h b/csrc/include/tdg_ln.h
--- a/csrc/include/tdg_ln.h
+++ b/csrc/include/tdg_ln.h
@@ -97,7 +97,8 @@
                                            float* __restrict__ rstd_out, float p, uint32_t thresh,
                                            uint64_t seed, const long long* ctr, uint64_t site,
                                            float eps, RowVec<D / 64>& o, size_t wt_bytes = 0,
-                                           uint8_t* __restrict__ kbits = nullptr) {
+                                           uint8_t* __restrict__ kbits = nullptr,
+                                           int store = ST_SC1) {
   constexpr int VEC = D / 64;
   if (has_t) {
     if (p > 0.f) {
@@ -117,7 +118,7 @@
     for (int i = 0; i < VEC; ++i) h.v[i] += t.v[i];
   }
   if (hsave) {
-    if (wt_bytes) h.store_row(hsave + rbase, lane, WtBuf(hsave, wt_bytes));
+    if (wt_bytes) h.store_row(hsave + rbase, lane, WtBuf(hsave, wt_bytes, store));
     else h.store_row(hsave + rbase, lane);
 #pragma unroll
     for (int i = 0; i < VEC; ++i) h.v[i] = bf2f(f2bf(h.v[i]));
@@ -139,7 +140,7 @@
     const int col = RowMap<VEC>::col(lane, i);
     o.v[i] = (h.v[i] - mean) * rstd * gamma[col] + beta[col];
   }
-  if (wt_bytes) o.store_row(y + rbase, lane, WtBuf(y, wt_bytes));
+  if (wt_bytes) o.store_row(y + rbase, lane, WtBuf(y, wt_bytes, store));
   else o.store_row(y + rbase, lane);
   if (lane == 0) {
     if (mean_out) mean_out[row] = mean;
diff --git a/csrc/kernels/attn_bwd.h b/csrc/kernels/attn_bwd.h
--- a/csrc/kernels/attn_bwd.h
+++ b/csrc/kernels/attn_bwd.h
@@ -797,7 +797,8 @@
   const int tid = threadIdx.x, lane = tid & 63, g = lane >> 4, cl = lane & 15;
   const int w = __builtin_amdgcn_readfirstlane(tid >> 6);
   const int bh = a.xcd ? xcd_remap(blockIdx.x, gridDim.x) : blockIdx.x;
-  const int b = bh / a.H, h = bh % a.H;
+  int h, b;
+  attn_head_batch(bh, a.H, h, b);
   int klim;
   float scl;
   bool causal;
diff --git a/csrc/kernels/attn_qkv.h b/csrc/kernels/attn_qkv.h
--- a/csrc/kernels/attn_qkv.h
+++ b/csrc/kernels/attn_qkv.h
@@ -20,7 +20,8 @@
   const int wid = __builtin_amdgcn_readfirstlane(tid >> 6);
   const int wm = wid / WN, wn = wid % WN;
   const int t = xcd_remap(blockIdx.x, gridDim.x);
-  const int h = t % a.H, b = t / a.H;
+  int h, b;
+  attn_head_batch(t, a.H, h, b);
   const int L = qa.L, d = qa.d, K = d;
   const bf16_t* X = reinterpret_cast<const bf16_t*>(qa.x) + (size_t)b * L * qa.ldx;
   using Ch = typename ATile<64>::template Chunks<512>;
diff --git a/csrc/kernels/bands.hip b/csrc/kernels/bands.hip
--- /dev/null
+++ b/csrc/kernels/bands.hip
@@ -0,0 +1,66 @@
+#include "tdg_api.h"
+#include "tdg_common.h"
+
+using namespace tdg;
+
+extern "C" int tdg_band_of(int kind, int M, int N, int K, int block, int out[4]) {
+  if (M <= 0 || block < 0) return -1;
+  int nblocks, r0, r1;
+  switch (kind) {
+    case 0:
+    case 1: {
+      if (N <= 0) return -1;
+      const int B = kind == 0 ? 128 : 256;
+      const int tiles_m = cdiv(M, B), tiles_n = cdiv(N, B);
+      nblocks = tiles_m * tiles_n;
+      if (block >= nblocks) return -1;
+      int tm, tn;
+      tile_raster(xcd_remap(block, nblocks), tiles_m, tiles_n, tm, tn);
+      r0 = tm * B;
+      r1 = r0 + B - 1;
+      break;
+    }
+    case 2:
+    case 5: {
+      nblocks = cdiv(M, 4);
+      if (block >= nblocks) return -1;
+      const int t = ln_block(block, nblocks, 1);
+      r0 = ln_fwd_row0(t, 0, 1);
+      r1 = ln_fwd_row0(t, 3, 1);
+      break;
+    }
+    case 3: {
+      if (N != 16 && N != 32 && N != 64) return -1;
+      nblocks = cdiv(M, N);
+      if (block >= nblocks) return -1;
+      const int t = ln_block(block, nblocks, 1);
+      r0 = ln_bwd_row0(t, 1, 0, N);
+      r1 = r0 + N - 1;
+      break;
+    }
+    case 4: {
+      if (N <= 0 || K <= 0) return -1;
+      nblocks = M * N;
+      if (block >= nblocks) return -1;
+      int h, b;
+      attn_head_batch(xcd_remap(block, nblocks), N, h, b);
+      r0 = b * K;
+      r1 = r0 + K - 1;
+      M = M * K;
+      break;
+    }
+    case 6: {
+      nblocks = M;
+      if (block >= nblocks) return -1;
+      r0 = r1 = xcd_remap(block, nblocks);
+      break;
+    }
+    default:
+      return -1;
+  }
+  out[0] = xcd_of_block(block);
+  out[1] = r0;
+  out[2] = r1 < M ? r1 : M - 1;
+  out[3] = nblocks;
+  return 0;
+}
diff --git a/csrc/kernels/embed.hip b/csrc/kernels/embed.hip
--- a/csrc/kernels/embed.hip
+++ b/csrc/kernels/embed.hip
@@ -10,10 +10,10 @@
 __global__ __launch_bounds__(256) void embed_fwd_kernel(
     const TokT* __restrict__ tok, const bf16_t* __restrict__ table, const float* __restrict__ pe,
     bf16_t* __restrict__ out, int M, int L, float scale, float p, uint32_t thresh, uint64_t seed,
-    const long long* __restrict__ ctr, uint64_t site, uint8_t* __restrict__ kbits) {
+    const long long* __restrict__ ctr, uint64_t site, uint8_t* __restrict__ kbits, int band) {
   constexpr int VEC = D / 64;
   const int lane = threadIdx.x & 63;
-  const int row = blockIdx.x * 4 + (threadIdx.x >> 6);
+  const int row = ln_fwd_row0(ln_block(blockIdx.x, gridDim.x, band), threadIdx.x >> 6, 1);
   if (row >= M) return;
   const int pos = row % L;
   const long long t = (long long)tok[row];
@@ -498,11 +498,11 @@
 template <int D, typename TT>
 void fwd_d(const void* tok, const void* table, const float* pe, void* out, int M, int L,
            float scale, float p, uint64_t seed, const long long* ctr, uint64_t site,
-           void* kbits, hipStream_t st) {
+           void* kbits, int band, hipStream_t st) {
   const uint32_t thresh = dropout_thresh(p);
   hipLaunchKernelGGL((embed_fwd_kernel<D, TT>), dim3(cdiv(M, 4)), dim3(256), 0, st,
                      (const TT*)tok, (const bf16_t*)table, pe, (bf16_t*)out, M, L, scale, p,
-                     thresh, seed, ctr, site, (uint8_t*)kbits);
+                     thresh, seed, ctr, site, (uint8_t*)kbits, band);
 }
 template <int D, typename TT>
 void bwd_d(const void* tok, const void* dout, float* dtable, int M, float scale, float p,
@@ -531,12 +531,15 @@
 
 extern "C" int tdg_embed_fwd(const void* tok, int tok64, const void* table, const float* pe,
                              void* out, int M, int L, int D, float scale, float p, uint64_t seed,
-                             const long long* ctr, uint64_t site, void* kbits, hipStream_t st) {
+                             const long long* ctr, uint64_t site, void* kbits, int band_order,
+                             hipStream_t st) {
   if (kbits && D < 512) return -3;
   if (tok64) {
-    TDG_D_SWITCH(fwd_d, long long, tok, table, pe, out, M, L, scale, p, seed, ctr, site, kbits, st)
+    TDG_D_SWITCH(fwd_d, long long, tok, table, pe, out, M, L, scale, p, seed, ctr, site, kbits,
+                 band_order, st)
   } else {
-    TDG_D_SWITCH(fwd_d, int, tok, table, pe, out, M, L, scale, p, seed, ctr, site, kbits, st)
+    TDG_D_SWITCH(fwd_d, int, tok, table, pe, out, M, L, scale, p, seed, ctr, site, kbits,
+                 band_order, st)
   }
 }
 
diff --git a/csrc/kernels/gemm.hip b/csrc/kernels/gemm.hip
--- a/csrc/kernels/gemm.hip
+++ b/csrc/kernels/gemm.hip
@@ -119,7 +119,9 @@
 extern "C" int tdg_gemm(const void* A, const void* B, void* C, const float* bias, const void* aux,
                         int M, int N, int K, int lda, int ldb, int ldc, int ldaux, int a_kc,
                         int b_kc, int epi, int out_f32, float alpha, float beta, int tile_cfg,
-                        int splits, float* ws, hipStream_t st, void* relu_bits, int ldbits) {
+                        int splits, float* ws, hipStream_t st, void* relu_bits, int ldbits,
+                        int band_store) {
+  if (band_store < ST_SC1 || band_store > ST_PLAIN) return -13;
   const bf16_t* a = (const bf16_t*)A;
   const bf16_t* b = (const bf16_t*)B;
   const bf16_t* x = (const bf16_t*)aux;
@@ -135,8 +137,13 @@
     return -1;
   }
   auto fn = a_kc ? (b_kc ? gemm_nt : gemm_nn) : (b_kc ? gemm_tt : gemm_tn);
-  return fn(epi, out_f32 != 0, tile_cfg, a, b, C, bias, x, M, N, K, lda, ldb, ldc, ldaux, alpha,
-            beta, splits, ws, st);
+  const bool band = !out_f32 && splits <= 1 &&
+                    (size_t)M * ldc * sizeof(bf16_t) <= (size_t)NUM_XCD * BAND_EDGE_BYTES;
+  *gemm_store_slot() = band ? band_store : (int)ST_SC1;
+  const int rc = fn(epi, out_f32 != 0, tile_cfg, a, b, C, bias, x, M, N, K, lda, ldb, ldc, ldaux,
+                    alpha, beta, splits, ws, st);
+  *gemm_store_slot() = ST_SC1;
+  return rc;
 }
 
 extern "C" int tdg_gemm_grouped(const void* const* A, const void* const* B, void* const* C, int G,
diff --git a/csrc/kernels/gemm_impl.h b/csrc/kernels/gemm_impl.h
--- a/csrc/kernels/gemm_impl.h
+++ b/csrc/kernels/gemm_impl.h
@@ -24,7 +24,7 @@
     const bf16_t* __restrict__ A, const bf16_t* __restrict__ B, void* __restrict__ Cv,
     const float* __restrict__ bias, const bf16_t* __restrict__ aux, int M, int N, int K, int lda,
     int ldb, int ldc, int ldaux, float alpha, float beta, int k_per_split, long long split_stride,
-    const GemmGroup grp) {
+    const GemmGroup grp, int store) {
   if (gridDim.y > 1) {
     A = grp.A[blockIdx.y];
     B = grp.B[blockIdx.y];
@@ -48,13 +48,7 @@
   const int nwg = tiles_m * tiles_n;
   const int t = xcd_remap(blockIdx.x, nwg);
   int tm, tn;
-  if (tiles_n <= tiles_m) {
-    tn = t % tiles_n;
-    tm = t / tiles_n;
-  } else {
-    tm = t % tiles_m;
-    tn = t / tiles_m;
-  }
+  tile_raster(t, tiles_m, tiles_n, tm, tn);
   const int m0 = tm * BM, n0 = tn * BN;
   TDG_STAMP(0);
 
@@ -198,7 +192,8 @@
               nullptr, 0, epi_vec_ok<EPI_NONE, true>(Cs, ldc, nullptr, 0));
   } else {
     Epi::template run_pre<true>(smem + wid * Epi::BYTES, acc, lane, Cv, ldc, M, N, mw0, nw0, alpha,
-                                beta, bias, aux, ldaux, vec, aux_r, pre_aux, c_r, pre_c, mask_r);
+                                beta, bias, aux, ldaux, vec, aux_r, pre_aux, c_r, pre_c, mask_r,
+                                store);
   }
 #ifdef TDG_STAMPS
   TDG_STAMP(3);
@@ -224,7 +219,8 @@
 __global__ __launch_bounds__(512) void gemm256_kernel(const R256Args args,
                                                       const float* __restrict__ bias,
                                                       const bf16_t* __restrict__ aux, int K,
-                                                      int ldaux, float alpha, float beta) {
+                                                      int ldaux, float alpha, float beta,
+                                                      int store) {
   constexpr int NW = 8;
   constexpr int HB = 128 * BK * 2;
   constexpr int SB = 4 * HB;
@@ -251,13 +247,7 @@
   const bf16_t* __restrict__ B = args.B[p];
   void* __restrict__ Cv = args.C[p];
   int tm, tn;
-  if (cl.tiles_n <= cl.tiles_m) {
-    tn = t % cl.tiles_n;
-    tm = t / cl.tiles_n;
-  } else {
-    tm = t % cl.tiles_m;
-    tn = t / cl.tiles_m;
-  }
+  tile_raster(t, cl.tiles_m, cl.tiles_n, tm, tn);
   float* __restrict__ bias_out = A_KC ? nullptr : args.bias_out[p];
   const bool do_bsum = bias_out != nullptr && tn == 0;
   float bsum0 = 0.f, bsum1 = 0.f;
@@ -484,10 +474,10 @@
     if constexpr (EPI == EPI_DRELU_BITS)
       Epi::run_mask(smem + wid * Epi::BYTES, acc, lane, Cv, ldc, M, N, m0 + wm * 128, n0 + wn * 64,
                     alpha, beta, bias, aux, ldaux, epi_vec_ok<EPI, OUT_F32>(Cv, ldc, aux, ldaux),
-                    mask_r);
+                    mask_r, store);
     else
       Epi::run(smem + wid * Epi::BYTES, acc, lane, Cv, ldc, M, N, m0 + wm * 128, n0 + wn * 64, alpha,
-               beta, bias, aux, ldaux, epi_vec_ok<EPI, OUT_F32>(Cv, ldc, aux, ldaux));
+               beta, bias, aux, ldaux, epi_vec_ok<EPI, OUT_F32>(Cv, ldc, aux, ldaux), store);
   }
 #ifdef TDG_STAMPS
   TDG_STAMP(3);
@@ -533,6 +523,11 @@
 namespace tdg {
 enum PlanFamily : int { PLAN_LOCK = 0, PLAN_R256 = 1, PLAN_PIPE = 2 };
 int* gemm_plan_slot();
+inline int* gemm_store_slot() {
+  static thread_local int flavour = ST_SC1;
+  return &flavour;
+}
+inline int gemm_store_flavour() { return *gemm_store_slot(); }
 inline void plan_record(int family, int bm, int bn, int depth, int splits) {
   int* p = gemm_plan_slot();
   p[0] = family; p[1] = bm; p[2] = bn; p[3] = depth; p[4] = splits;
@@ -561,7 +556,7 @@
     plan_record(PLAN_LOCK, BM, BN, ST, 1);
     hipLaunchKernelGGL((gemm_kernel<BM, BN, WM, WN, ST, AK, BKc, EPI, F32>), dim3(tiles, G, 1),
                        dim3(WM * WN * 64), lds, st, A, B, C, bias, aux, M, N, K, lda, ldb, ldc,
-                       ldaux, alpha, beta, K, 0LL, gr);
+                       ldaux, alpha, beta, K, 0LL, gr, G > 1 ? (int)ST_SC1 : gemm_store_flavour());
   } else {
     int kps = cdiv(cdiv(K, splits), BK) * BK;
     splits = cdiv(K, kps);
@@ -569,7 +564,7 @@
     plan_record(PLAN_LOCK, BM, BN, ST, splits);
     hipLaunchKernelGGL((gemm_kernel<BM, BN, WM, WN, ST, AK, BKc, EPI_NONE, true>),
                        dim3(tiles, 1, splits), dim3(WM * WN * 64), lds, st, A, B, (void*)ws, bias,
-                       aux, M, N, K, lda, ldb, ldc, ldaux, 1.f, 0.f, kps, stride, gr);
+                       aux, M, N, K, lda, ldb, ldc, ldaux, 1.f, 0.f, kps, stride, gr, (int)ST_SC1);
     const long long total = (long long)M * N;
     const int blocks = (int)std::min<long long>(4096, (total + 255) / 256);
     hipLaunchKernelGGL((splitk_reduce_kernel<EPI, F32>), dim3(blocks), dim3(256), 0, st, ws, C,
@@ -612,7 +607,7 @@
     }
     plan_record(PLAN_R256, 256, 256, 2, 1);
     hipLaunchKernelGGL((gemm256_kernel<AK, BKc, EPI, F32>), dim3(tiles), dim3(512), lds, st, args,
-                       bias, aux, K, ldaux, alpha, beta);
+                       bias, aux, K, ldaux, alpha, beta, gemm_store_flavour());
     return 0;
   }
 }
@@ -655,7 +650,7 @@
   hipLaunchKernelGGL((gemm_pipe_kernel<BM, BN, WM, WN, NS, AK, BKc, EPI, F32>), dim3(tiles),
                      dim3(WM * WN * 64), lds,
                      st, A, B, C, bias, aux, M, N, K, lda, ldb, ldc, ldaux, alpha, beta,
-                     (int)(ab * 2), (int)(bb * 2));
+                     (int)(ab * 2), (int)(bb * 2), gemm_store_flavour());
   return true;
   }
 }
diff --git a/csrc/kernels/gemm_pipe.h b/csrc/kernels/gemm_pipe.h
--- a/csrc/kernels/gemm_pipe.h
+++ b/csrc/kernels/gemm_pipe.h
@@ -196,7 +196,7 @@
 __global__ __launch_bounds__(WM * WN * 64) void gemm_pipe_kernel(
     const bf16_t* __restrict__ A, const bf16_t* __restrict__ B, void* __restrict__ Cv,
     const float* __restrict__ bias, const bf16_t* __restrict__ aux, int M, int N, int K, int lda,
-    int ldb, int ldc, int ldaux, float alpha, float beta, int a_bytes, int b_bytes) {
+    int ldb, int ldc, int ldaux, float alpha, float beta, int a_bytes, int b_bytes, int store) {
   using P = Pipe<BM, BN, WM, WN, NS, A_KC, B_KC>;
   constexpr int NW = P::NW, TM = P::TM, TN = P::TN, A_BYTES = P::A_BYTES, SB = P::SB, PT = P::PT;
   constexpr int WTM = BM / WM, WTN = BN / WN;
@@ -209,13 +209,7 @@
   const int tiles_m = cdiv(M, BM), tiles_n = cdiv(N, BN);
   const int t = xcd_remap(blockIdx.x, tiles_m * tiles_n);
   int tm, tn;
-  if (tiles_n <= tiles_m) {
-    tn = t % tiles_n;
-    tm = t / tiles_n;
-  } else {
-    tm = t % tiles_m;
-    tn = t / tiles_m;
-  }
+  tile_raster(t, tiles_m, tiles_n, tm, tn);
   const int m0 = tm * BM, n0 = tn * BN;
   const int nk = K / PK;
 
@@ -277,10 +271,10 @@
     if constexpr (EPI == EPI_DRELU_BITS)
       Epi::run_mask(smem + wid * Epi::BYTES, acc, lane, Cv, ldc, M, N, m0 + wm * WTM, n0 + wn * WTN,
                     alpha, beta, bias, aux, ldaux, epi_vec_ok<EPI, OUT_F32>(Cv, ldc, aux, ldaux),
-                    mask_r);
+                    mask_r, store);
     else
       Epi::run(smem + wid * Epi::BYTES, acc, lane, Cv, ldc, M, N, m0 + wm * WTM, n0 + wn * WTN, alpha,
-               beta, bias, aux, ldaux, epi_vec_ok<EPI, OUT_F32>(Cv, ldc, aux, ldaux));
+               beta, bias, aux, ldaux, epi_vec_ok<EPI, OUT_F32>(Cv, ldc, aux, ldaux), store);
   }
 }
 
diff --git a/csrc/kernels/norm.hip b/csrc/kernels/norm.hip
--- a/csrc/kernels/norm.hip
+++ b/csrc/kernels/norm.hip
@@ -43,16 +43,17 @@
     atomic_amax(amax_word(amax8, blockIdx.x), fmaxf(fmaxf(red8[0], red8[1]), fmaxf(red8[2], red8[3])));
 }
 
-template <int D, int RPW>
+template <int D, int RPW, int ST>
 __global__ __launch_bounds__(256) void ln_fwd_kernel(
     const bf16_t* __restrict__ x, const bf16_t* __restrict__ s, const float* __restrict__ gamma,
     const float* __restrict__ beta, bf16_t* __restrict__ y, bf16_t* __restrict__ hsave,
     float* __restrict__ mean_out, float* __restrict__ rstd_out, int M, float p, uint32_t thresh,
     uint64_t seed, const long long* ctr, uint64_t site, float eps, uint8_t* __restrict__ y8,
-    const float* __restrict__ s8p, unsigned* __restrict__ amax8, uint8_t* __restrict__ kbits) {
+    const float* __restrict__ s8p, unsigned* __restrict__ amax8, uint8_t* __restrict__ kbits,
+    int band) {
   constexpr int VEC = D / 64;
   const int lane = threadIdx.x & 63;
-  const int r0 = (blockIdx.x * 4 + (threadIdx.x >> 6)) * RPW;
+  const int r0 = ln_fwd_row0(ln_block(blockIdx.x, gridDim.x, band), threadIdx.x >> 6, RPW);
   __shared__ float red8[4];
   RowVec<VEC> h[RPW], t[RPW];
 #pragma unroll
@@ -69,13 +70,14 @@
     const size_t rbase = (size_t)row * D;
     RowVec<VEC> o;
     ln_row_fwd<D>(h[k], t[k], s != nullptr, rbase, row, lane, gamma, beta, y, hsave, mean_out,
-                  rstd_out, p, thresh, seed, ctr, site, eps, o, (size_t)M * D * sizeof(bf16_t), kbits);
+                  rstd_out, p, thresh, seed, ctr, site, eps, o, (size_t)M * D * sizeof(bf16_t), kbits,
+                  ST);
     if (y8) ln_row_y8<D>(o, s8p[0], y8, rbase, lane, am, WtBuf(y8, (size_t)M * D));
   }
   if (y8) ln_amax_flush(am, red8, amax8);
 }
 
-template <int D, int RPW, int NWV>
+template <int D, int RPW, int NWV, int ST>
 __global__ __launch_bounds__(NWV * 64) void ln_bwd_kernel(
     const bf16_t* __restrict__ dy, const bf16_t* __restrict__ hsave,
     const float* __restrict__ mean_in, const float* __restrict__ rstd_in,
@@ -84,8 +86,9 @@
     float* __restrict__ part_s, int M, float p, uint32_t thresh, uint64_t seed,
     const long long* ctr, uint64_t site, int iters, uint8_t* __restrict__ ds8,
     const float* __restrict__ s8p, unsigned* __restrict__ amax8,
-    const uint8_t* __restrict__ kbits) {
+    const uint8_t* __restrict__ kbits, int band) {
   constexpr int VEC = D / 64;
+  const int t = ln_block(blockIdx.x, gridDim.x, band);
   __shared__ float red[NWV][D];
   float am8 = 0.f;
   const int lane = threadIdx.x & 63, w = threadIdx.x >> 6;
@@ -96,11 +99,11 @@
 #pragma unroll
   for (int i = 0; i < VEC; ++i) gm[i] = gamma[RowMap<VEC>::col(lane, i)];
   const float sc = p > 0.f ? 1.f / (1.f - p) : 1.f;
-  const WtBuf wdh(dh_out, (size_t)M * D * sizeof(bf16_t));
-  const WtBuf wds(ds_out ? ds_out : dh_out, (size_t)M * D * sizeof(bf16_t));
+  const WtBuf wdh(dh_out, (size_t)M * D * sizeof(bf16_t), ST);
+  const WtBuf wds(ds_out ? ds_out : dh_out, (size_t)M * D * sizeof(bf16_t), ST);
 #pragma unroll 1
   for (int it = 0; it < iters; ++it) {
-  const int r0 = (blockIdx.x * iters + it) * (NWV * RPW) + w * RPW;
+  const int r0 = ln_bwd_row0(t, iters, it, NWV * RPW) + w * RPW;
   if (r0 >= M) break;
   RowVec<VEC> g[RPW], h[RPW], e[RPW];
   float mean[RPW], rstd[RPW];
@@ -173,7 +176,7 @@
       float a = 0.f;
 #pragma unroll
       for (int k = 0; k < NWV; ++k) a += red[k][col];
-      parts[q][(size_t)blockIdx.x * D + col] = a;
+      parts[q][(size_t)t * D + col] = a;
     }
     __syncthreads();
   }
@@ -195,22 +198,22 @@
 using namespace tdg;
 
 namespace {
-template <int D>
+template <int D, int ST>
 void ln_fwd_d(const void* x, const void* s, const float* gamma, const float* beta, void* y,
               void* hsave, float* mean, float* rstd, int M, float p, uint64_t seed,
               const long long* ctr, uint64_t site, float eps, void* y8, const float* s8,
-              unsigned* amax8, void* kbits, hipStream_t st) {
+              unsigned* amax8, void* kbits, int band, hipStream_t st) {
   const uint32_t thresh = dropout_thresh(p);
-  hipLaunchKernelGGL((ln_fwd_kernel<D, 1>), dim3(cdiv(M, 4)), dim3(256), 0, st, (const bf16_t*)x,
+  hipLaunchKernelGGL((ln_fwd_kernel<D, 1, ST>), dim3(cdiv(M, 4)), dim3(256), 0, st, (const bf16_t*)x,
                      (const bf16_t*)s, gamma, beta, (bf16_t*)y, (bf16_t*)hsave, mean, rstd, M, p,
-                     thresh, seed, ctr, site, eps, (uint8_t*)y8, s8, amax8, (uint8_t*)kbits);
-}
-template <int D>
+                     thresh, seed, ctr, site, eps, (uint8_t*)y8, s8, amax8, (uint8_t*)kbits, band);
+}
+template <int D, int ST>
 void ln_bwd_d(const void* dy, const void* hsave, const float* mean, const float* rstd,
               const float* gamma, void* dh, void* ds, const void* dres, float* dgamma,
               float* dbeta, float* dbias, float* ws, int M, float p, uint64_t seed, const long long* ctr, uint64_t site,
               int accumulate, int skip_reduce, int rpb, void* ds8, const float* s8, unsigned* amax8,
-              const void* kbits, hipStream_t st) {
+              const void* kbits, int band, hipStream_t st) {
   const uint32_t thresh = dropout_thresh(p);
   constexpr int RPW = D >= 1024 ? 2 : 4;
   const int nb = cdiv(M, rpb);
@@ -218,15 +221,17 @@
   float* pb = ws + (size_t)nb * D;
   float* ps = dbias ? ws + 2 * (size_t)nb * D : nullptr;
   if (rpb <= 16)
-    hipLaunchKernelGGL((ln_bwd_kernel<D, RPW, 4>), dim3(nb), dim3(256), 0, st, (const bf16_t*)dy,
+    hipLaunchKernelGGL((ln_bwd_kernel<D, RPW, 4, ST>), dim3(nb), dim3(256), 0, st, (const bf16_t*)dy,
                        (const bf16_t*)hsave, mean, rstd, gamma, (bf16_t*)dh, (bf16_t*)ds,
                        (const bf16_t*)dres, pg, pb, ps, M, p, thresh, seed, ctr, site,
-                       max(1, rpb / (RPW * 4)), (uint8_t*)ds8, s8, amax8, (const uint8_t*)kbits);
+                       max(1, rpb / (RPW * 4)), (uint8_t*)ds8, s8, amax8, (const uint8_t*)kbits,
+                       band);
   else
-    hipLaunchKernelGGL((ln_bwd_kernel<D, RPW, 8>), dim3(nb), dim3(512), 0, st, (const bf16_t*)dy,
+    hipLaunchKernelGGL((ln_bwd_kernel<D, RPW, 8, ST>), dim3(nb), dim3(512), 0, st, (const bf16_t*)dy,
                        (const bf16_t*)hsave, mean, rstd, gamma, (bf16_t*)dh, (bf16_t*)ds,
                        (const bf16_t*)dres, pg, pb, ps, M, p, thresh, seed, ctr, site,
-                       max(1, rpb / (RPW * 8)), (uint8_t*)ds8, s8, amax8, (const uint8_t*)kbits);
+                       max(1, rpb / (RPW * 8)), (uint8_t*)ds8, s8, amax8, (const uint8_t*)kbits,
+                       band);
   if (skip_reduce) return;
   const float beta = accumulate ? 1.f : 0.f;
   ReduceSet rs{{pg, pb, ps}, {dgamma, dbeta, dbias}};
@@ -238,10 +243,17 @@
 extern "C" int tdg_ln_fwd(const void* x, const void* s, const float* gamma, const float* beta,
                           void* y, void* hsave, float* mean, float* rstd, int M, int D, float p,
                           uint64_t seed, const long long* ctr, uint64_t site, float eps, void* y8,
-                          const float* s8, unsigned* amax8, void* kbits, hipStream_t st) {
+                          const float* s8, unsigned* amax8, void* kbits, int band_order,
+                          int band_store, hipStream_t st) {
   if (kbits && D < 512) return -3;
-#define TDG_LN_F(DD) \
-  ln_fwd_d<DD>(x, s, gamma, beta, y, hsave, mean, rstd, M, p, seed, ctr, site, eps, y8, s8, amax8, kbits, st); \
+  if (band_store < ST_SC1 || band_store > ST_PLAIN) return -4;
+#define TDG_LN_F1(DD, ST) \
+  ln_fwd_d<DD, ST>(x, s, gamma, beta, y, hsave, mean, rstd, M, p, seed, ctr, site, eps, y8, s8,  \
+                   amax8, kbits, band_order, st)
+#define TDG_LN_F(DD)                                   \
+  if (band_store == ST_NT) TDG_LN_F1(DD, ST_NT);       \
+  else if (band_store == ST_PLAIN) TDG_LN_F1(DD, ST_PLAIN); \
+  else TDG_LN_F1(DD, ST_SC1);                          \
   return 0;
   switch (D) {
     case 128: TDG_LN_F(128)
@@ -251,6 +263,7 @@
     default: return -1;
   }
 #undef TDG_LN_F
+#undef TDG_LN_F1
 }
 
 extern "C" int tdg_ln_bwd(const void* dy, const void* hsave, const float* mean, const float* rstd,
@@ -258,13 +271,19 @@
                           float* dbeta, float* dbias, float* ws, int M, int D, float p,
                           uint64_t seed, const long long* ctr, uint64_t site, int accumulate,
                           int skip_reduce, int rpb, void* ds8, const float* s8, unsigned* amax8,
-                          const void* kbits, hipStream_t st) {
+                          const void* kbits, int band_order, int band_store, hipStream_t st) {
   if (rpb != 16 && rpb != 32 && rpb != 64) return -2;
+  if (band_store < ST_SC1 || band_store > ST_PLAIN) return -4;
   if (ds8 && !s8) return -2;
   if (kbits && D < 512) return -3;
-#define TDG_LN_B(DD)                                                                              \
-  ln_bwd_d<DD>(dy, hsave, mean, rstd, gamma, dh, ds, dres, dgamma, dbeta, dbias, ws, M, p, seed, \
-               ctr, site, accumulate, skip_reduce, rpb, ds8, s8, amax8, kbits, st);              \
+#define TDG_LN_B1(DD, ST)                                                                      \
+  ln_bwd_d<DD, ST>(dy, hsave, mean, rstd, gamma, dh, ds, dres, dgamma, dbeta, dbias, ws, M, p,    \
+                   seed, ctr, site, accumulate, skip_reduce, rpb, ds8, s8, amax8, kbits,          \
+                   band_order, st)
+#define TDG_LN_B(DD)                                        \
+  if (band_store == ST_NT) TDG_LN_B1(DD, ST_NT);            \
+  else if (band_store == ST_PLAIN) TDG_LN_B1(DD, ST_PLAIN); \
+  else TDG_LN_B1(DD, ST_SC1);                               \
   return 0;
   switch (D) {
     case 128: TDG_LN_B(128)
@@ -274,6 +293,7 @@
     default: return -1;
   }
 #undef TDG_LN_B
+#undef TDG_LN_B1
 }
 
 namespace tdg {
diff --git a/tensorflow_distributed_on_gke_amd/ops/kernels.py b/tensorflow_distributed_on_gke_amd/ops/kernels.py
--- a/tensorflow_distributed_on_gke_amd/ops/kernels.py
+++ b/tensorflow_distributed_on_gke_amd/ops/kernels.py
@@ -10,6 +10,32 @@
 
 EPI_NONE, EPI_BIAS, EPI_BIAS_RELU, EPI_DRELU = 0, 1, 2, 3
 NUM_CU = 256
+
+STORE_SC1, STORE_NT, STORE_PLAIN = 0, 1, 2
+_STORES = {"sc1": STORE_SC1, "nt": STORE_NT, "plain": STORE_PLAIN}
+
+
+def _store_id(v) -> int:
+    if isinstance(v, str) and v.strip().lower() in _STORES:
+        return _STORES[v.strip().lower()]
+    if int(v) not in (STORE_SC1, STORE_NT, STORE_PLAIN):
+        raise ValueError(f"store flavour {v!r}: sc1 / nt / plain (0 / 1 / 2)")
+    return int(v)
+
+
+LN_XCD = int(os.environ.get("TDG_LN_XCD", "1") != "0")
+BAND_STORE = _store_id(os.environ.get("TDG_BAND_STORE", "sc1") or "sc1")
+
+
+def set_row_bands(ln_xcd=None, band_store=None) -> Tuple[int, int]:
+    global LN_XCD, BAND_STORE
+    old = (LN_XCD, BAND_STORE)
+    if ln_xcd is not None:
+        LN_XCD = int(bool(ln_xcd))
+    if band_store is not None:
+        BAND_STORE = _store_id(band_store)
+    return old
+
 
 _WS: Dict[Tuple[int, int, str], torch.Tensor] = {}
 _WS_RETIRED: List[torch.Tensor] = []
@@ -139,10 +165,11 @@
         ws = workspace("splitk", splits * M * ldc, A.device) if splits > 1 else None
         if relu_bits is None:
             C().gemm(A, B, out, bias, aux, M, N, K, lda, ldb, ldc, ldaux, a_kc, b_kc, epi, alpha,
-                     beta, tile, splits, ws)
+                     beta, tile, splits, ws, band_store=BAND_STORE)
         else:
             C().gemm(A, B, out, bias, aux, M, N, K, lda, ldb, ldc, ldaux, a_kc, b_kc, epi, alpha,
-                     beta, tile, splits, ws, relu_bits=relu_bits, ldbits=relu_bits.stride(0))
+                     beta, tile, splits, ws, relu_bits=relu_bits, ldbits=relu_bits.stride(0),
+                     band_store=BAND_STORE)
 
     if cfg is None:
         Mk, Kk = (M, _tok_bucket(K)) if (not a_kc and not b_kc) else (_tok_bucket(M), K)
@@ -488,7 +515,8 @@
     h = torch.empty_like(x) if save else None
     mean = torch.empty(M, dtype=torch.float32, device=x.device) if save else None
     rstd = torch.empty(M, dtype=torch.float32, device=x.device) if save else None
-    C().ln_fwd(x, s, gamma, beta, y, h, mean, rstd, p, seed, ctr, site, eps, y8, s8, amax8, kbits)
+    C().ln_fwd(x, s, gamma, beta, y, h, mean, rstd, p, seed, ctr, site, eps, y8, s8, amax8, kbits,
+               bool(LN_XCD), BAND_STORE)
     return y, h, mean, rstd
 
 
@@ -515,7 +543,8 @@
     else:
         ws = workspace(f"ln_bwd_part_{site}", 3 * ln_bwd_nparts(M, D) * D, dy.device)
     C().ln_bwd(dy, h, mean, rstd, gamma, dh, ds, dres, dgamma, dbeta, dbias, ws, p, seed, ctr, site,
-               accumulate, defer is not None, ln_bwd_rpb(D), ds8, s8, amax8, kbits)
+               accumulate, defer is not None, ln_bwd_rpb(D), ds8, s8, amax8, kbits, bool(LN_XCD),
+               BAND_STORE)
     if defer is not None:
         nb = ln_bwd_nparts(M, D)
         outs = [dgamma, dbeta] + ([dbias] if dbias is not None else [])
@@ -541,7 +570,7 @@
     B, L = tok.shape
     D = table.shape[1]
     out = torch.empty(B, L, D, dtype=torch.bfloat16, device=tok.device)
-    C().embed_fwd(tok, table, pe, out, scale, p, seed, ctr, site, kbits)
+    C().embed_fwd(tok, table, pe, out, scale, p, seed, ctr, site, kbits, bool(LN_XCD))
     return out
 
 
```

Result: no change. 3.562 million tokens/s (-0.0%).
